# liangyuanpeng/kwok

Measured on AMD Instinct MI355X. Metric: stage transitions/sec (whole node), 1M nodes/100M pods; achieved HBM GB/s, higher is better.
Workload: dtype u8/i64

## Files before the change

### kwok_amd/csrc/engine.hip

```cpp
#include <hip/hip_runtime.h>

#include <cstdio>
#include <cstdlib>
#include <algorithm>
#include <cmath>
#include <cstring>
#include <mutex>
#include <set>
#include <string>
#include <type_traits>
#include <utility>
#include <vector>

#include "../../include/kwok_engine.h"
#include "id8_compose.hpp"
#include "errscope.hpp"
#include "devmem.hpp"
#include "usage_rows.hpp"

namespace {

constexpr int kBlock = 256;
constexpr int kMinObjPerThread = 8;
constexpr int kMaxObjPerThread = 32;
constexpr int kWavesPerBlock = kBlock / 64;
constexpr int kStatWords = 4 + KWK_MAX_STAGES;
constexpr int kStatLine = 3 + KWK_MAX_STAGES;

__device__ __forceinline__ void philox10(uint32_t& c0, uint32_t& c1, uint32_t& c2, uint32_t& c3, uint32_t k0,
                                         uint32_t k1) {
  k0 = (uint32_t)__builtin_amdgcn_readfirstlane((int)k0);
  k1 = (uint32_t)__builtin_amdgcn_readfirstlane((int)k1);
  asm volatile("" : "+s"(k0), "+s"(k1));
#pragma unroll
  for (int r = 0; r < 10; ++r) {
    const uint64_t p0 = (uint64_t)0xD2511F53u * c0, p1 = (uint64_t)0xCD9E8D57u * c2;
    const uint32_t lo0 = (uint32_t)p0, hi0 = (uint32_t)(p0 >> 32);
    const uint32_t lo1 = (uint32_t)p1, hi1 = (uint32_t)(p1 >> 32);
    const uint32_t n0 = hi1 ^ c1 ^ k0;
    const uint32_t n2 = hi0 ^ c3 ^ k1;
    c0 = n0;
    c1 = lo1;
    c2 = n2;
    c3 = lo0;
    k0 += 0x9E3779B9u;
    k1 += 0xBB67AE85u;
  }
}

__device__ __forceinline__ uint64_t philox_u64(uint64_t gslot, uint64_t step, uint32_t site, uint64_t key) {
  uint32_t c0 = (uint32_t)gslot, c1 = (uint32_t)step, c2 = (uint32_t)(step >> 32), c3 = site;
  philox10(c0, c1, c2, c3, (uint32_t)key, (uint32_t)(key >> 32));
  return (uint64_t)c0 | ((uint64_t)c1 << 32);
}

__device__ __forceinline__ int64_t below_u64(uint64_t u, int64_t n) { return (int64_t)__umul64hi(u, (uint64_t)n); }

__device__ __forceinline__ double rng_float64(uint64_t gslot, uint64_t step, uint32_t site, uint64_t key) {
  return (double)(philox_u64(gslot, step, site, key) >> 11) * 0x1.0p-53;
}

constexpr uint32_t kSitePick = 1, kSiteLeaseJitter = 3, kSiteRetryJitter = 4;

__device__ __forceinline__ int64_t sat_add(int64_t a, int64_t b) {
  int64_t r;
  if (__builtin_add_overflow(a, b, &r)) return b > 0 ? INT64_MAX : INT64_MIN;
  return r;
}

__device__ __forceinline__ int64_t abs_time_sub(int64_t sec, int32_t nsec, int64_t now) {
  int64_t now_sec = now / 1000000000;
  int64_t now_ns = now % 1000000000;
  if (now_ns < 0) { now_ns += 1000000000; now_sec -= 1; }
  int64_t ds = sec - now_sec;
  int64_t dn = (int64_t)nsec - now_ns;
  if (ds == 0) return dn;
  if (ds > 0) { ds -= 1; dn += 1000000000; } else { ds += 1; dn -= 1000000000; }
  if (ds > 9223372036ll || ds < -9223372036ll) return ds > 0 ? INT64_MAX : INT64_MIN;
  const int64_t p = ds * 1000000000ll;
  int64_t d;
  if (__builtin_add_overflow(p, dn, &d)) return dn > 0 ? INT64_MAX : INT64_MIN;
  return d;
}

struct Getter {
  int64_t v;
  bool ok;
};

__device__ __forceinline__ Getter eval_getter(int32_t slot, int64_t def, bool def_ok, uint32_t sched,
                                              const kwk_value* __restrict__ rec, int64_t del_s, int64_t now,
                                              bool is_duration) {
  if (slot == KWK_SLOT_NONE) return {def, def_ok};
  if (slot == KWK_SLOT_DELETION) {
    if (del_s == KWK_DEL_ABSENT) return {def, def_ok};
    return {abs_time_sub(del_s, 0, now), true};
  }
  if (!(sched & KWK_F_HASREC)) return {def, def_ok};
  const kwk_value e = rec[slot];
  switch (e.kind) {
    case KWK_V_OK: return {e.value, true};
    case KWK_V_NOTOK: return {0, false};
    case KWK_V_ABSTIME: return {is_duration ? abs_time_sub(e.value, e.nsec, now) : 0, is_duration};
    default: return {def, def_ok};
  }
}

struct StateFmt {
  uint32_t narrow;
  uint32_t half;
  uint32_t byte;
  uint32_t dw;
  int64_t epoch;
  uint32_t pmask;
  uint32_t cshift, cmask;
  uint32_t sshift, smask, none_code;
  uint32_t fshift;
  const uint16_t* id2w;
  const uint8_t* w2id;
};

__host__ __device__ __forceinline__ uint2 fmt_unpack(uint32_t w, const StateFmt& f) {
  const uint32_t cls = (w >> f.cshift) & f.cmask;
  const uint32_t sc = (w >> f.sshift) & f.smask;
  const uint32_t stage = sc == f.none_code ? KWK_STAGE_NONE : sc;
  const uint32_t fl = (w >> f.fshift) & 0x1Fu;
  return make_uint2(w & f.pmask, stage | (fl << 8) | (cls << KWK_CLASS_SHIFT));
}

__host__ __device__ __forceinline__ uint32_t fmt_pack(uint32_t pred, uint32_t sched, const StateFmt& f) {
  const uint32_t stage = sched & 0xFFu;
  const uint32_t sc = stage == KWK_STAGE_NONE ? f.none_code : stage;
  return (pred & f.pmask) | (((sched >> KWK_CLASS_SHIFT) & f.cmask) << f.cshift) | ((sc & f.smask) << f.sshift) |
         (((sched >> 8) & 0x1Fu) << f.fshift);
}

constexpr uint32_t kDwShift = 28;
constexpr uint32_t kDwWordMask = (1u << kDwShift) - 1u;
constexpr uint64_t kDwFar = (1ull << 36) - 1ull;
constexpr uint64_t kDwRebase = 1ull << 34;
__host__ __device__ __forceinline__ uint64_t dw_get(uint2 r) {
  return ((uint64_t)(r.x >> kDwShift) << 32) | r.y;
}
__host__ __device__ __forceinline__ uint2 dw_put(uint2 r, uint64_t d) {
  return make_uint2((r.x & kDwWordMask) | ((uint32_t)(d >> 32) << kDwShift), (uint32_t)d);
}
__host__ __device__ __forceinline__ uint64_t dw_enc(int64_t due, int64_t epoch) {
  if (due < epoch) return kDwFar;
  const uint64_t d = (uint64_t)due - (uint64_t)epoch;
  return d < kDwFar ? d : kDwFar;
}
__host__ __device__ __forceinline__ int64_t dw_abs(uint64_t d, int64_t epoch) {
  return (int64_t)((uint64_t)epoch + d);
}

__device__ __forceinline__ uint2 load_state(const void* st, uint64_t i, const StateFmt& f) {
  if (f.byte) return fmt_unpack(f.id2w[reinterpret_cast<const uint8_t*>(st)[i]], f);
  if (f.half) return fmt_unpack(reinterpret_cast<const uint16_t*>(st)[i], f);
  if (f.dw) return fmt_unpack(reinterpret_cast<const uint32_t*>(st)[2 * i], f);
  return f.narrow ? fmt_unpack(reinterpret_cast<const uint32_t*>(st)[i], f) : reinterpret_cast<const uint2*>(st)[i];
}
__device__ __forceinline__ void store_state(void* st, uint64_t i, uint2 v, const StateFmt& f) {
  if (f.byte) {
    reinterpret_cast<uint8_t*>(st)[i] = f.w2id[fmt_pack(v.x, v.y, f) & 0xFFFFu];
  } else if (f.half) {
    reinterpret_cast<uint16_t*>(st)[i] = (uint16_t)fmt_pack(v.x, v.y, f);
  } else if (f.dw) {
    uint32_t* p = reinterpret_cast<uint32_t*>(st) + 2 * i;
    *p = (*p & ~kDwWordMask) | fmt_pack(v.x, v.y, f);
  } else if (f.narrow) {
    reinterpret_cast<uint32_t*>(st)[i] = fmt_pack(v.x, v.y, f);
  } else {
    reinterpret_cast<uint2*>(st)[i] = v;
  }
}
__device__ __forceinline__ void store_state_due(void* st, int64_t* due_col, uint64_t i, uint2 v, int64_t due,
                                                const StateFmt& f) {
  if (f.dw) {
    const uint64_t d = dw_enc(due, f.epoch);
    reinterpret_cast<uint2*>(st)[i] = dw_put(make_uint2(fmt_pack(v.x, v.y, f), 0u), d);
    if (d == kDwFar) due_col[i] = due;
  } else {
    store_state(st, i, v, f);
    due_col[i] = due;
  }
}

__device__ __forceinline__ uint2 sw_decode(uint2 w, const StateFmt&) { return w; }
__device__ __forceinline__ uint2 sw_decode(uint32_t w, const StateFmt& f) { return fmt_unpack(w, f); }
__device__ __forceinline__ void sw_encode(uint2& out, uint2 v, const StateFmt&) { out = v; }
__device__ __forceinline__ void sw_encode(uint32_t& out, uint2 v, const StateFmt& f) { out = fmt_pack(v.x, v.y, f); }

struct RawTest {
  uint32_t managed, dirty, alive;
  uint32_t sshift, smask, none_code;
  uint32_t term, del;
};

constexpr uint32_t kMaxFuseSteps = 4;
constexpr uint32_t kHbMin = kMaxFuseSteps;
constexpr uint32_t kHbMax = 64;
struct SweepArgs {
  void* __restrict__ st;
  int64_t* __restrict__ due;
  int64_t* __restrict__ del_s;
  const uint32_t* __restrict__ rec_idx;
  const kwk_value* __restrict__ values;
  const kwk_stage_table* __restrict__ table;
  const kwk_delta* __restrict__ deltas;
  const uint32_t* __restrict__ lut;
  kwk_fired_rec* __restrict__ fired;
  uint32_t* __restrict__ wave_counts;
  unsigned long long* __restrict__ cum;
  uint32_t n;
  uint32_t lut_n;
  uint32_t lut_bytes;
  uint32_t lut_rest;
  uint32_t value_slots;
  uint64_t slot_base;
  uint64_t key;
  uint64_t step;
  int64_t now;
  uint32_t fire;
  StateFmt fmt;
  RawTest raw;
  kwk_harness harness;
  const uint32_t* __restrict__ fsm;
  const int64_t* __restrict__ fsm_due;
  uint32_t fsm_bits;
  const uint4* __restrict__ comp;
  int64_t dw_epoch_old;
  uint32_t dw_rebase;
  kwk_fired_rec* __restrict__ firedx[kMaxFuseSteps - 1];
  uint32_t* __restrict__ countsx[kMaxFuseSteps - 1];
  int64_t nowx[kMaxFuseSteps - 1];
  struct TailHb {
    void* out;
    uint32_t* offsets;
    uint32_t* host_len;
    unsigned long long* status;
    uint32_t seq;
    uint32_t packed;
  } tail;
};

__host__ __device__ __forceinline__ bool stage_matches(const kwk_stage_desc& s, uint32_t pred) {
  bool ok = ((pred ^ s.eq_val) & s.eq_mask) == 0;
  for (uint32_t k = 0; k < s.n_any; ++k) ok &= ((pred & s.any_mask[k]) != 0) == (((s.any_want >> k) & 1u) != 0);
  return ok;
}

__device__ __forceinline__ Getter stage_weight(const kwk_stage_desc& s, uint32_t sched,
                                               const kwk_value* __restrict__ rec) {
  return eval_getter(s.weight_slot, s.weight_default, true, sched, rec, KWK_DEL_ABSENT, 0, false);
}

__device__ __forceinline__ int nth_bit(uint32_t m, int64_t n) {
  for (int64_t i = 0; i < n; ++i) m &= m - 1;
  return __ffs(m) - 1;
}

struct Fire {
  bool fire;
  uint32_t stage;
  uint32_t flags;
  uint32_t bytes;
};

__device__ __forceinline__ uint32_t match_mask(const kwk_stage_table* __restrict__ T, uint32_t n_stages,
                                               uint32_t pred, const uint32_t* lut, uint32_t lut_n,
                                               uint32_t lut_bytes, uint32_t lut_rest) {
  uint32_t m = 0;
  if (lut_n) {
    m = lut[pred & 0xFFu];
    if (lut_bytes > 1) m &= lut[256u | ((pred >> 8) & 0xFFu)];
    if (lut_bytes > 2) m &= lut[512u | ((pred >> 16) & 0xFFu)];
    if (lut_bytes > 3) m &= lut[768u | (pred >> 24)];
    for (uint32_t r = lut_rest; r; r &= r - 1) {
      const uint32_t s = (uint32_t)__ffs(r) - 1u;
      m |= (stage_matches(T->stages[s], pred) ? 1u : 0u) << s;
    }
  } else {
    for (uint32_t s = 0; s < n_stages; ++s) m |= (stage_matches(T->stages[s], pred) ? 1u : 0u) << s;
  }
  return m;
}

template <bool kProbe = false>
__device__ __forceinline__ bool match_object(const SweepArgs& a, const kwk_stage_table* __restrict__ T,
                                             uint32_t n_stages, uint64_t i, uint32_t pred, uint32_t& sched,
                                             int64_t& due, uint32_t& bytes, const uint32_t* lut, uint32_t lut_n,
                                             uint32_t& gen) {
  const uint32_t m = match_mask(T, n_stages, pred, lut, lut_n, a.lut_bytes, a.lut_rest);
  sched &= ~(KWK_F_DIRTY | KWK_F_MATCHERR);
  if (m == 0) return false;
  const kwk_value* __restrict__ rec = nullptr;
  if (sched & KWK_F_HASREC) {
    if constexpr (kProbe) { gen = 1; return false; }
    rec = a.values + (uint64_t)a.rec_idx[i] * a.value_slots;
    bytes += 4 + 16 * 3;
  }
  const uint64_t gslot = a.slot_base + i;
  int pick;
  const int cnt = __popc(m);
  uint64_t u_pick = 0, u_jit = 0;
  if (!kProbe && (cnt > 1 || (m & T->reserved[0]))) {
    uint32_t c0 = (uint32_t)gslot, c1 = (uint32_t)a.step, c2 = (uint32_t)(a.step >> 32), c3 = kSitePick;
    philox10(c0, c1, c2, c3, (uint32_t)a.key, (uint32_t)(a.key >> 32));
    u_pick = (uint64_t)c0 | ((uint64_t)c1 << 32);
    u_jit = (uint64_t)c2 | ((uint64_t)c3 << 32);
  }
  if (cnt == 1) {
    pick = __ffs(m) - 1;
  } else {
    if constexpr (kProbe) { gen = 1; return false; }
    int64_t total = 0;
    int nerr = 0, nge0 = 0;
    for (uint32_t mm = m; mm; mm &= mm - 1) {
      const Getter w = stage_weight(T->stages[__ffs(mm) - 1], sched, rec);
      if (w.ok) {
        total = (int64_t)((uint64_t)total + (uint64_t)w.v);
        nge0 += w.v >= 0;
      } else {
        ++nerr;
      }
    }
    if (nerr == cnt || (total == 0 && nerr == 0)) {
      pick = nth_bit(m, below_u64(u_pick, cnt));
    } else if (total == 0) {
      int64_t want = below_u64(u_pick, nge0);
      pick = -1;
      for (uint32_t mm = m; mm; mm &= mm - 1) {
        const int s = __ffs(mm) - 1;
        const Getter w = stage_weight(T->stages[s], sched, rec);
        if (w.ok && w.v >= 0) {
          if (want == 0) { pick = s; break; }
          --want;
        }
      }
    } else if (total < 0) {
      sched |= KWK_F_MATCHERR;
      return false;
    } else {
      int64_t off = below_u64(u_pick, total);
      pick = 31 - __clz(m);
      for (uint32_t mm = m; mm; mm &= mm - 1) {
        const int s = __ffs(mm) - 1;
        const Getter w = stage_weight(T->stages[s], sched, rec);
        const int64_t wv = w.ok ? w.v : -1;
        if (wv <= 0) continue;
        off -= wv;
        if (off < 0) { pick = s; break; }
      }
    }
  }
  const kwk_stage_desc& S = T->stages[pick];
  int64_t delay = 0;
  if (S.has_delay) {
    const bool need_del = S.delay_slot == KWK_SLOT_DELETION || S.jitter_slot == KWK_SLOT_DELETION;
    if constexpr (kProbe) {
      if (need_del) { gen = 1; return false; }
    }
    const int64_t dels = need_del ? a.del_s[i] : KWK_DEL_ABSENT;
    if (need_del) bytes += 8;
    const Getter d = eval_getter(S.delay_slot, S.delay_default, true, sched, rec, dels, a.now, true);
    if (d.ok) {
      delay = d.v;
      if (S.has_jitter) {
        const Getter j = eval_getter(S.jitter_slot, S.jitter_default, S.jitter_default_ok != 0, sched, rec, dels,
                                     a.now, true);
        if (j.ok) {
          if (j.v < delay) {
            delay = j.v;
          } else {
            const int64_t jit = (int64_t)((uint64_t)j.v - (uint64_t)delay);
            if constexpr (kProbe) {
              if (jit > 0) { gen = 1; return false; }
            }
            if (jit > 0)
              delay = (int64_t)((uint64_t)delay + (uint64_t)below_u64(u_jit, jit));
          }
        }
      }
    }
  }
  sched = (sched & ~0xFFu) | (uint32_t)pick;
  due = sat_add(a.now, delay);
  return true;
}

__device__ __forceinline__ void fire_object(const SweepArgs& a, const kwk_stage_table* __restrict__ T,
                                            const kwk_delta* __restrict__ deltas, uint32_t n_stages,
                                            uint32_t fin_group, uint32_t cls, uint32_t st, uint32_t& pred,
                                            uint32_t& sched, Fire& f) {
  const kwk_stage_desc& S = T->stages[st];
  f.fire = true;
  f.stage = st;
  const uint32_t pre = pred;
  bool rematch = (S.flags & KWK_NEXT_PATCHES) && (!(S.flags & KWK_NEXT_PATCH_STATIC) || !(pre & S.applied_mask));
  if (S.flags & KWK_NEXT_FIN) {
    const uint32_t F = pre & fin_group;
    uint32_t F2;
    if ((S.flags & KWK_NEXT_FIN_EMPTY) || ((S.flags & KWK_NEXT_FIN_REMOVE) && (F & ~S.fin_remove) == 0))
      F2 = S.fin_add;
    else
      F2 = (F & ~S.fin_remove) | (S.fin_add & ~F);
    rematch |= F2 != F;
    pred = (pred & ~fin_group) | F2;
  }
  if (S.flags & KWK_NEXT_DELETE) {
    sched &= ~KWK_F_ALIVE;
    f.flags |= KWK_FIRED_DELETED;
    rematch = false;
  } else if (S.flags & KWK_NEXT_PATCHES) {
    const kwk_delta d = deltas[cls * n_stages + st];
    f.bytes += 2;
    if (d.and_mask == KWK_DELTA_UNKNOWN_AND && d.or_mask == KWK_DELTA_UNKNOWN_OR)
      f.flags |= KWK_FIRED_DELTA_UNKNOWN;
    else
      pred = (((pred & d.and_mask) | d.or_mask) & ~fin_group) | (pred & fin_group);
  }
  if (rematch) {
    sched |= KWK_F_DIRTY;
    f.flags |= KWK_FIRED_REMATCH;
  }
  sched |= KWK_STAGE_NONE;
}

template <bool kHarness, uint32_t kWordBytes, bool kProbe = false, bool kDueOut = false>
__device__ __forceinline__ uint2 process_object(const SweepArgs& a, const kwk_stage_table* __restrict__ T,
                                               const kwk_delta* __restrict__ deltas, uint32_t n_stages,
                                               uint32_t fin_group, uint64_t i, uint32_t pred, uint32_t sched,
                                               int64_t due, Fire& f, uint32_t& n_matched, const uint32_t* lut,
                                               uint32_t lut_n, uint32_t& gen, int64_t& due_w) {
  if (kHarness) {
    if (!(sched & KWK_F_ALIVE)) {
      pred &= a.harness.keep_mask;
      sched = (sched & (KWK_F_MANAGED | KWK_F_HASREC | KWK_CLASS_MASK)) | KWK_F_ALIVE | KWK_F_DIRTY | KWK_STAGE_NONE;
      if (a.harness.track_deletion) {
        if constexpr (kProbe) gen = 1;
        else a.del_s[i] = KWK_DEL_ABSENT;
        f.bytes += 8;
      }
    } else if ((pred & a.harness.terminal_mask) && !(pred & a.harness.deletion_bit)) {
      pred |= a.harness.deletion_bit;
      int64_t sec = a.now / 1000000000;
      if (a.now % 1000000000 < 0) sec -= 1;
      if (a.harness.track_deletion) {
        if constexpr (kProbe) gen = 1;
        else a.del_s[i] = sec;
        f.bytes += 8;
      }
      sched |= KWK_F_DIRTY;
    }
  }
  bool scheduled = false;
  if (sched & KWK_F_ALIVE) {
    if (sched & KWK_F_DIRTY) {
      if (pred & T->disregard_mask) {
        sched &= ~KWK_F_DIRTY;
      } else {
        scheduled = match_object<kProbe>(a, T, n_stages, i, pred, sched, due, f.bytes, lut, lut_n, gen);
        n_matched += scheduled ? 1 : 0;
      }
    }
    const uint32_t st = sched & 0xFFu;
    if (a.fire && st < n_stages && due <= a.now) fire_object(a, T, deltas, n_stages, fin_group, sched >> KWK_CLASS_SHIFT, st,
                                                   pred, sched, f);
  }
  if (scheduled && (sched & 0xFFu) < n_stages) {
    if constexpr (kProbe) {
      due_w = due;
    } else if constexpr (kDueOut) {
      due_w = due;
      gen = 1;
    } else {
      a.due[i] = due;
    }
    if constexpr (!kDueOut) f.bytes += 8;
  }
  f.bytes += kWordBytes;
  return make_uint2(pred, sched);
}

template <bool kPacked = false>
__device__ __forceinline__ void emit_fired(const Fire& f, uint64_t i, uint32_t lane, kwk_fired_rec* __restrict__ seg,
                                           uint32_t& seg_n, unsigned int* s_stat, uint32_t& n_bytes) {
  const unsigned long long bal = __ballot(f.fire);
  if (!bal) return;
  if (f.fire) {
    const uint32_t pos = seg_n + (uint32_t)__popcll(bal & ((1ull << lane) - 1ull));
    if constexpr (kPacked) {
      reinterpret_cast<uint32_t*>(seg)[pos] = (uint32_t)i | f.stage << 13 | f.flags << 18;
      n_bytes += 4;
    } else {
      seg[pos] = kwk_fired_rec{(uint32_t)i, (uint16_t)f.stage, (uint16_t)f.flags};
      n_bytes += 8;
    }
  }
  seg_n += (uint32_t)__popcll(bal);
  unsigned long long rest = bal;
  while (rest) {
    const uint32_t s = __shfl(f.stage, __ffsll((long long)rest) - 1);
    const unsigned long long same = __ballot(f.fire && f.stage == s);
    if (lane == 0) atomicAdd(&s_stat[3 + s], (unsigned)__popcll(same));
    rest &= ~same;
  }
}

constexpr uint32_t kLutMax = 256;
constexpr uint32_t kLutTables = 1024;
constexpr uint32_t kLutLdsW = 512;

constexpr uint32_t kOOB = 0xFFFFFFF0u;
__device__ __forceinline__ __amdgpu_buffer_rsrc_t make_rsrc(const void* p, uint32_t bytes) {
  return __builtin_amdgcn_make_buffer_rsrc(const_cast<void*>(p), (short)0, (int)bytes, 0x00020000);
}
__device__ __forceinline__ int64_t buf_load_i64(__amdgpu_buffer_rsrc_t r, uint32_t off) {
  const auto t = __builtin_amdgcn_raw_buffer_load_b64(r, off, 0, 0);
  return (int64_t)(((uint64_t)t[1] << 32) | t[0]);
}

__device__ __forceinline__ void store_chunk_nt(void* p, const uint4& v) {
  typedef uint32_t u32x4 __attribute__((ext_vector_type(4)));
  __builtin_nontemporal_store(u32x4{v.x, v.y, v.z, v.w}, reinterpret_cast<u32x4*>(p));
}

constexpr uint32_t kFsmDue = 1u << 30, kFsmGeneral = 1u << 31;

template <bool kHarness>
__global__ void fsm_build_kernel(SweepArgs a, uint32_t* __restrict__ tab, int64_t* __restrict__ dtab) {
  const uint32_t bits = a.fsm_bits;
  const uint32_t idx = blockIdx.x * blockDim.x + threadIdx.x;
  if (idx >= (2u << bits)) return;
  const uint32_t w = idx & ((1u << bits) - 1u), rdy = idx >> bits;
  const uint2 s = fmt_unpack(w, a.fmt);
  const kwk_stage_table* __restrict__ T = a.table;
  const int64_t due = ((s.y & 0xFFu) != KWK_STAGE_NONE) ? (rdy ? 0 : 1) : 0;
  Fire f{false, 0, 0, 0};
  uint32_t nm = 0, gen = 0;
  int64_t dw = INT64_MIN;
  const uint2 nv = process_object<kHarness, 2, true>(a, T, a.deltas, T->n_stages, T->fin_group_mask, 0, s.x, s.y, due,
                                                     f, nm, a.lut, a.lut_n, gen, dw);
  uint32_t e = fmt_pack(nv.x, nv.y, a.fmt) & 0xFFFFu;
  e |= (f.stage & 31u) << 16 | (f.fire ? 1u : 0u) << 21 | (f.flags & 7u) << 22 | (nm & 1u) << 25;
  e |= ((f.bytes >> 1) & 15u) << 26;
  if (dw != INT64_MIN) e |= kFsmDue;
  if (gen || f.bytes > 30 || (f.bytes & 1u)) e = kFsmGeneral;
  tab[idx] = e;
  dtab[idx] = dw;
}

constexpr uint32_t kQ16 = 4;
constexpr int kWpe16 = 6;
constexpr int kWpe16Q4 = 4;
constexpr int kLdsDeltas16 = 64;
constexpr uint32_t kStoreLanes = 8;
__device__ __forceinline__ constexpr uint32_t bit_word(const uint32_t b) {
  return ((b & 15u) >> 2) * 512u + 2u * (b & 3u) + (b >> 4);
}
template <int Q>
constexpr uint32_t seg16_words() { return 64u * 8u * Q + 32u; }
#define kSeg16 seg16_words<Q>()
template <bool kHarness, int Q, bool kPersist>
__global__ __launch_bounds__(kBlock) __attribute__((amdgpu_waves_per_eu(Q >= 4 ? kWpe16Q4 : kWpe16))) void sweep16_kernel(SweepArgs a) {
  constexpr int K = 8 * Q;
  constexpr uint32_t kWave = 64u * K;
  constexpr uint32_t kTile = kBlock * K;
  __shared__ unsigned int s_stat[kStatWords];
  __shared__ kwk_delta s_delta[kLdsDeltas16];
  __shared__ uint16_t s_work[kWavesPerBlock][kWave];
  __shared__ uint4 s_tile[kWavesPerBlock][64 * Q];
  __shared__ uint32_t s_lut[kLutMax];
  __shared__ kwk_stage_table s_tab;
  const uint32_t lane = threadIdx.x & 63;
  const uint32_t wave = threadIdx.x >> 6;
  const uint32_t n_tiles = (uint32_t)(((uint64_t)a.n + kTile - 1) / kTile);
  const __amdgpu_buffer_rsrc_t st_rs = make_rsrc(a.st, ((a.n * 2u) + 15u) & ~15u);
  uint4 va[Q];
  auto issue_tile = [&](uint4 (&dst)[Q], const uint32_t t) {
    if (t >= n_tiles) return;
    const uint32_t wb = t * kTile + wave * kWave;
#pragma unroll
    for (int q = 0; q < Q; ++q) {
      const auto c = __builtin_amdgcn_raw_buffer_load_b128(st_rs, (wb + (uint32_t)q * 512u + lane * 8u) * 2u, 0, 0);
      dst[q] = make_uint4(c[0], c[1], c[2], c[3]);
    }
  };
  uint32_t tile = blockIdx.x;
  issue_tile(va, tile);
  {
    const uint32_t nw = (offsetof(kwk_stage_table, stages) + a.table->n_stages * sizeof(kwk_stage_desc)) / 4;
    const uint32_t* src = reinterpret_cast<const uint32_t*>(a.table);
    uint32_t* dst = reinterpret_cast<uint32_t*>(&s_tab);
    for (uint32_t j = threadIdx.x; j < nw; j += kBlock) dst[j] = src[j];
  }
  const kwk_stage_table* __restrict__ T = &s_tab;
  const uint32_t n_stages = a.table->n_stages;
  const uint32_t fin_group = a.table->fin_group_mask;
  const uint32_t n_deltas = a.table->n_classes * n_stages;
  const uint32_t lut_n = a.lut_n;
  const uint32_t* __restrict__ lutp = lut_n <= kLutMax ? s_lut : a.lut;
  if (lut_n <= kLutMax)
    for (uint32_t j = threadIdx.x; j < lut_n; j += kBlock) s_lut[j] = a.lut[j];
  if (threadIdx.x < kStatWords) s_stat[threadIdx.x] = 0;
  const kwk_delta* __restrict__ deltas = a.deltas;
  if (n_deltas <= kLdsDeltas16) {
    for (uint32_t j = threadIdx.x; j < n_deltas; j += kBlock) s_delta[j] = a.deltas[j];
    deltas = s_delta;
  }
  __syncthreads();

  const StateFmt fmt = a.fmt;
  const RawTest R = a.raw;
  struct {
    uint32_t m2, d2, a2, t2, l2, s2, n2;
    uint32_t sm, sd, sa, sl;
  } X;
  X.m2 = R.managed * 0x10001u; X.d2 = R.dirty * 0x10001u; X.a2 = R.alive * 0x10001u;
  X.t2 = R.term * 0x10001u; X.l2 = R.del * 0x10001u;
  X.s2 = (R.smask << R.sshift) * 0x10001u; X.n2 = (R.none_code << R.sshift) * 0x10001u;
  X.sm = (uint32_t)(16 - __ffs(R.managed)) & 31u; X.sd = (uint32_t)(16 - __ffs(R.dirty)) & 31u;
  X.sa = (uint32_t)(16 - __ffs(R.alive)) & 31u; X.sl = (uint32_t)(16 - __ffs(R.del)) & 31u;
  uint32_t n_matched = 0, n_bytes = 0;
  uint32_t n_line = 0;
  uint32_t wave_fired = 0;
  uint16_t* __restrict__ wl = s_work[wave];
  uint4* __restrict__ tq = s_tile[wave];
  uint16_t* __restrict__ tw = reinterpret_cast<uint16_t*>(tq);
  uint4* __restrict__ gq = reinterpret_cast<uint4*>(a.st);

  auto tile_body = [&](uint4 (&v)[Q], const uint32_t tile) {
    const uint32_t wbase = tile * kTile + wave * kWave;
    const bool full = (uint64_t)(tile + 1) * kTile <= a.n;
    uint32_t seg_n = 0;
    const uint64_t seg_id = (uint64_t)tile * kWavesPerBlock + wave;
    uint32_t* __restrict__ seg32 = reinterpret_cast<uint32_t*>(a.fired) + seg_id * kSeg16;
    kwk_fired_rec* __restrict__ seg = reinterpret_cast<kwk_fired_rec*>(seg32 + 1);

    uint4 cur[Q];
#pragma unroll
    for (int q = 0; q < Q; ++q) cur[q] = v[q];
    if (kPersist) issue_tile(v, tile + gridDim.x);
    constexpr uint32_t kHalfMask = (1u << (4 * Q)) - 1u;
    uint32_t in_range = kHalfMask | kHalfMask << 16;
    if (!full) {
      in_range = 0;
#pragma unroll
      for (int t = 0; t < K; ++t) {
        const int b = t < 4 * Q ? t : 16 + t - 4 * Q;
        in_range |= (wbase + bit_word((uint32_t)b) + lane * 8u < a.n ? 1u : 0u) << b;
      }
    }
    uint32_t pend = 0, need = 0, ready = 0;
#pragma unroll
    for (int q = 0; q < Q; ++q) {
      const uint32_t dw[4] = {cur[q].x, cur[q].y, cur[q].z, cur[q].w};
#pragma unroll
      for (int j = 0; j < 4; ++j) {
        const uint32_t d = dw[j];
        const uint32_t mg = (d & X.m2) << X.sm;
        const uint32_t pe = (((d & X.s2) ^ X.n2) + 0x7FFF7FFFu) & 0x80008000u;
        uint32_t nb = (d & X.d2) << X.sd;
        if (kHarness) {
          nb |= (~d & X.a2) << X.sa;
          nb |= (((d & X.t2) + 0x7FFF7FFFu) & 0x80008000u) & ~((d & X.l2) << X.sl);
        }
        const uint32_t n2 = mg & nb, p2 = mg & pe;
        const int jj = q * 4 + j;
        need |= n2 >> (15 - jj);
        pend |= p2 >> (15 - jj);
      }
    }
    pend &= in_range;
    need &= in_range;
    if (__ballot(pend != 0)) {
      const __amdgpu_buffer_rsrc_t due_rs = make_rsrc(a.due, a.n * 8u);
#pragma unroll 8
      for (int t = 0; t < K; ++t) {
        const int k = t < 4 * Q ? t : 16 + t - 4 * Q;
        const uint32_t p = (pend >> k) & 1u;
        const int64_t d = buf_load_i64(due_rs, p ? (wbase + bit_word((uint32_t)k) + lane * 8u) * 8u : kOOB);
        ready |= (p & (uint32_t)(d <= a.now)) << k;
      }
      need |= ready;
    }
    n_bytes += 2u * (uint32_t)__popc(in_range) + 8u * (uint32_t)__popc(pend);
    uint32_t n_work = 0, pos = 0;
    {
      const uint32_t cnt = (uint32_t)__popc(need);
      const unsigned long long lt = (1ull << lane) - 1ull;
#pragma unroll
      for (int b = 0; b < 6; ++b) {
        const unsigned long long bal = __ballot((cnt >> b) & 1u);
        pos += (uint32_t)__popcll(bal & lt) << b;
        n_work += (uint32_t)__popcll(bal) << b;
      }
      for (uint32_t m = need; m; m &= m - 1u) {
        const uint32_t k = (uint32_t)__ffs(m) - 1u;
        wl[pos++] = (uint16_t)(bit_word(k) + lane * 8u + (((ready >> k) & 1u) << 15));
      }
    }

    if (n_work) {
#pragma unroll
      for (int q = 0; q < Q; ++q) tq[q * 64 + lane] = cur[q];
      __builtin_amdgcn_fence(__ATOMIC_SEQ_CST, "wavefront");
      auto fetch = [&](const uint32_t c, uint32_t& we, uint32_t& raw, uint32_t& ent) {
        we = (c + lane < n_work) ? (uint32_t)wl[c + lane] : 0xFFFFFFFFu;
        raw = we != 0xFFFFFFFFu ? (uint32_t)tw[we & 0x7FFFu] : 0u;
        ent = (we != 0xFFFFFFFFu && a.fsm) ? a.fsm[((we >> 15) << a.fsm_bits) | raw] : kFsmGeneral;
      };
      uint32_t we, raw, ent;
      fetch(0, we, raw, ent);
      for (uint32_t c = 0; c < n_work; c += 64u) {
        const uint32_t cwe = we, craw = raw, e = ent;
        if (c + 64u < n_work) fetch(c + 64u, we, raw, ent);
        Fire f{false, 0, 0, 0};
        uint64_t i = 0;
        if (cwe != 0xFFFFFFFFu) {
          const uint32_t w = cwe & 0x7FFFu, rdy = cwe >> 15;
          i = wbase + w;
          if (!(e & kFsmGeneral)) {
            tw[w] = (uint16_t)e;
            if (e & kFsmDue) a.due[i] = sat_add(a.now, a.fsm_due[(rdy << a.fsm_bits) | craw]);
            f.fire = (e >> 21) & 1u;
            f.stage = (e >> 16) & 31u;
            f.flags = (e >> 22) & 7u;
            f.bytes = ((e >> 26) & 15u) * 2u;
            n_matched += (e >> 25) & 1u;
          } else {
            const uint2 s = fmt_unpack(craw, fmt);
            const int64_t due = ((s.y & 0xFFu) != KWK_STAGE_NONE) ? a.due[i] : 0;
            uint32_t gen_unused = 0;
            int64_t due_unused = 0;
            const uint2 nv = process_object<kHarness, 2>(a, T, deltas, n_stages, fin_group, i, s.x, s.y, due, f,
                                                         n_matched, lutp, lut_n, gen_unused, due_unused);
            tw[w] = (uint16_t)fmt_pack(nv.x, nv.y, fmt);
          }
          n_line -= 2u;
        }
        n_bytes += f.bytes;
        emit_fired<true>(f, i - wbase, lane, seg, seg_n, s_stat, n_bytes);
      }
      __builtin_amdgcn_fence(__ATOMIC_SEQ_CST, "wavefront");
#pragma unroll
      for (int q = 0; q < Q; ++q) {
        const uint4 nv = tq[q * 64 + lane];
        const bool ch = (nv.x ^ cur[q].x) | (nv.y ^ cur[q].y) | (nv.z ^ cur[q].z) | (nv.w ^ cur[q].w);
        const unsigned long long bal = __ballot(ch);
        if ((bal >> (lane & ~(kStoreLanes - 1u))) & ((1ull << kStoreLanes) - 1ull)) {
          store_chunk_nt(&gq[(wbase + (uint32_t)q * 512u + lane * 8u) / 8u], nv);
          n_line += 16u;
        }
      }
      __builtin_amdgcn_fence(__ATOMIC_SEQ_CST, "wavefront");
    }
    {
      const uint32_t used = 1u + seg_n, end = (used + 31u) & ~31u;
      for (uint32_t x = used + lane; x < end; x += 64) seg32[x] = 0u;
      if (lane == 0) {
        seg32[0] = seg_n;
        a.wave_counts[seg_id] = seg_n;
      }
      n_line += 4u * (uint32_t)__popc((uint32_t)(lane < end - used));
    }
    wave_fired += seg_n;
    n_bytes += lane == 0 ? 4u : 0u;
  };
  if constexpr (!kPersist) {
    if (tile < n_tiles) tile_body(va, tile);
  } else {
    for (; tile < n_tiles; tile += gridDim.x) tile_body(va, tile);
  }

  for (int off = 32; off > 0; off >>= 1) {
    n_matched += __shfl_xor(n_matched, off);
    n_bytes += __shfl_xor(n_bytes, off);
    n_line += __shfl_xor(n_line, off);
  }
  if (lane == 0) {
    atomicAdd(&s_stat[0], n_matched);
    atomicAdd(&s_stat[1], wave_fired);
    atomicAdd(&s_stat[2], n_bytes);
    atomicAdd(&s_stat[kStatLine], n_bytes + n_line);
  }
  __syncthreads();
  if (threadIdx.x < 3 + n_stages || threadIdx.x == kStatLine) {
    const unsigned int val = s_stat[threadIdx.x];
    if (val) atomicAdd(&a.cum[(uint64_t)blockIdx.x * kStatWords + threadIdx.x], (unsigned long long)val);
  }
}

template <bool kHarness>
__device__ __forceinline__ uint2 general16(uint32_t i, uint32_t raw) {
  uint64_t ka = (uint64_t)__builtin_amdgcn_kernarg_segment_ptr();
  asm volatile("" : "+v"(ka));
  const SweepArgs& a = *reinterpret_cast<const SweepArgs*>(ka);
  uint64_t tp = (uint64_t)a.table;
  asm volatile("" : "+v"(tp));
  const kwk_stage_table* __restrict__ T = reinterpret_cast<const kwk_stage_table*>(tp);
  const uint2 s = fmt_unpack(raw, a.fmt);
  const int64_t due = ((s.y & 0xFFu) != KWK_STAGE_NONE) ? a.due[i] : 0;
  Fire f{false, 0, 0, 0};
  uint32_t nm = 0, gen_unused = 0;
  int64_t due_unused = 0;
  const uint2 nv = process_object<kHarness, 2>(a, T, a.deltas, T->n_stages, T->fin_group_mask, i, s.x, s.y, due, f, nm,
                                               a.lut, a.lut_n, gen_unused, due_unused);
  uint32_t e = fmt_pack(nv.x, nv.y, a.fmt) & 0xFFFFu;
  e |= (f.stage & 31u) << 16 | (f.fire ? 1u : 0u) << 21 | (f.flags & 7u) << 22 | (nm & 1u) << 25;
  return make_uint2(e, f.bytes);
}

__device__ __forceinline__ uint32_t block_prefix(unsigned long long* status, uint32_t stride, uint32_t b, uint32_t bt,
                                                 uint32_t seq, uint32_t lane) {
  if (lane == 0)
    __hip_atomic_store(&status[(uint64_t)b * stride], (unsigned long long)seq << 32 | bt, __ATOMIC_RELAXED,
                       __HIP_MEMORY_SCOPE_AGENT);
  constexpr uint32_t kIn = 16;
  uint32_t pre = 0;
  for (uint32_t j0 = lane; j0 < b; j0 += 64u * kIn) {
    unsigned long long v[kIn];
#pragma unroll
    for (uint32_t k = 0; k < kIn; ++k) {
      const uint32_t j = j0 + 64u * k;
      v[k] = j < b ? __hip_atomic_load(&status[(uint64_t)j * stride], __ATOMIC_RELAXED, __HIP_MEMORY_SCOPE_AGENT)
                   : (unsigned long long)seq << 32;
    }
#pragma unroll
    for (uint32_t k = 0; k < kIn; ++k) {
      const uint32_t j = j0 + 64u * k;
      while ((uint32_t)(v[k] >> 32) != seq) {
        __builtin_amdgcn_s_sleep(2);
        v[k] = __hip_atomic_load(&status[(uint64_t)j * stride], __ATOMIC_RELAXED, __HIP_MEMORY_SCOPE_AGENT);
      }
      pre += (uint32_t)v[k];
    }
  }
  for (int o = 32; o > 0; o >>= 1) pre += __shfl_xor(pre, o);
  return pre;
}

template <uint32_t kWaveSlots, uint32_t kSegWords>
__device__ __forceinline__ void tail_handback(const SweepArgs& a, uint32_t wave_n, uint32_t lane, uint32_t wave) {
  __shared__ uint32_t s_wn[kWavesPerBlock];
  __shared__ uint32_t s_pre;
  const SweepArgs::TailHb& t = a.tail;
  __builtin_amdgcn_fence(__ATOMIC_RELEASE, "workgroup");
  if (lane == 0) s_wn[wave] = wave_n;
  __syncthreads();
  const uint32_t bt = s_wn[0] + s_wn[1] + s_wn[2] + s_wn[3];
  if (wave == 0) {
    const uint32_t pre = block_prefix(t.status, 1u, blockIdx.x, bt, t.seq, lane);
    if (lane == 0) s_pre = pre;
  }
  __syncthreads();
  uint32_t off = s_pre;
  for (uint32_t w = 0; w < wave; ++w) off += s_wn[w];
  const uint64_t seg_id = (uint64_t)blockIdx.x * kWavesPerBlock + wave;
  const uint32_t* __restrict__ sp = reinterpret_cast<const uint32_t*>(a.fired) + seg_id * kSegWords;
  const uint32_t base = (uint32_t)seg_id * kWaveSlots;
  for (uint32_t j = lane; j < wave_n; j += 64u) {
    const uint32_t x = sp[1u + j];
    const uint32_t slot = base + (x & 0x1FFFu);
    if (t.packed) {
      __builtin_nontemporal_store(((x >> 13) & 31u) << 27 | slot, reinterpret_cast<uint32_t*>(t.out) + off + j);
    } else {
      typedef uint32_t u32x2 __attribute__((ext_vector_type(2)));
      __builtin_nontemporal_store(u32x2{slot, ((x >> 13) & 31u) | ((x >> 18) & 7u) << 16},
                                  reinterpret_cast<u32x2*>(reinterpret_cast<kwk_fired_rec*>(t.out) + off + j));
    }
  }
  if (blockIdx.x == gridDim.x - 1 && threadIdx.x == 0) {
    t.offsets[0] = s_pre + bt;
    if (t.host_len) t.host_len[0] = s_pre + bt;
  }
}

constexpr int kFsmBatch = 4;
constexpr uint32_t kFsmKernelDefault = 2;
template <bool kHarness, int Q, bool kPersist, int kDepth>
__global__ __launch_bounds__(kBlock) __attribute__((amdgpu_waves_per_eu(Q >= 4 ? 4 : 5))) void sweep16_fsm_kernel(SweepArgs a) {
  constexpr int K = 8 * Q;
  constexpr uint32_t kWave = 64u * K;
  constexpr uint32_t kTile = kBlock * K;
  constexpr int B = kFsmBatch;
  static_assert(kDepth >= 1 && kDepth <= 2 && (kPersist || kDepth == 1), "prefetch depth");
  __shared__ unsigned int s_stat[kStatWords];
  __shared__ uint16_t s_work[kWavesPerBlock][kWave];
  __shared__ uint4 s_tile[kWavesPerBlock][64 * Q];
  const uint32_t lane = threadIdx.x & 63;
  const uint32_t wave = __builtin_amdgcn_readfirstlane(threadIdx.x >> 6);
  const uint32_t n_tiles = (uint32_t)(((uint64_t)a.n + kTile - 1) / kTile);
  const __amdgpu_buffer_rsrc_t st_rs = make_rsrc(a.st, ((a.n * 2u) + 15u) & ~15u);
  const __amdgpu_buffer_rsrc_t due_rs = make_rsrc(a.due, a.n * 8u);
  const uint32_t fbits = a.fsm_bits;
  const __amdgpu_buffer_rsrc_t fsm_rs = make_rsrc(a.fsm, 4u << (fbits + 1));
  const __amdgpu_buffer_rsrc_t fdue_rs = make_rsrc(a.fsm_due, 8u << (fbits + 1));
  uint4 va[kDepth][Q];
  auto issue_tile = [&](uint4 (&dst)[Q], const uint32_t t) __attribute__((always_inline)) {
    const uint32_t off = t < n_tiles ? (t * kTile + wave * kWave + lane * 8u) * 2u : kOOB - 4u * 1024u;
#pragma unroll
    for (int q = 0; q < Q; ++q) {
      const auto c = __builtin_amdgcn_raw_buffer_load_b128(st_rs, off + (uint32_t)q * 1024u, 0, 0);
      dst[q] = make_uint4(c[0], c[1], c[2], c[3]);
    }
  };
  uint32_t tile = blockIdx.x;
  issue_tile(va[0], tile);
  if (kDepth > 1) issue_tile(va[1], tile + gridDim.x);
  const uint32_t n_stages = a.table->n_stages;
  if (threadIdx.x < kStatWords) s_stat[threadIdx.x] = 0;
  __syncthreads();

  const RawTest R = a.raw;
  struct {
    uint32_t m2, d2, a2, t2, l2, s2, n2;
    uint32_t sm, sd, sa, sl;
  } X;
  X.m2 = R.managed * 0x10001u; X.d2 = R.dirty * 0x10001u; X.a2 = R.alive * 0x10001u;
  X.t2 = R.term * 0x10001u; X.l2 = R.del * 0x10001u;
  X.s2 = (R.smask << R.sshift) * 0x10001u; X.n2 = (R.none_code << R.sshift) * 0x10001u;
  X.sm = (uint32_t)(16 - __ffs(R.managed)) & 31u; X.sd = (uint32_t)(16 - __ffs(R.dirty)) & 31u;
  X.sa = (uint32_t)(16 - __ffs(R.alive)) & 31u; X.sl = (uint32_t)(16 - __ffs(R.del)) & 31u;
  uint32_t stc01 = 0, stc23 = 0;
  uint32_t n_matched = 0, n_bytes = 0;
  uint32_t n_lline = 0;
  uint32_t w_bytes = 0, w_line = 0;
  uint32_t wave_fired = 0;
  uint16_t* __restrict__ wl = s_work[wave];
  uint4* __restrict__ tq = s_tile[wave];
  uint16_t* __restrict__ tw = reinterpret_cast<uint16_t*>(tq);
  uint4* __restrict__ gq = reinterpret_cast<uint4*>(a.st);

  auto tile_body = [&](uint4 (&v)[Q], const uint32_t tile) __attribute__((always_inline)) {
    const uint32_t wbase = tile * kTile + wave * kWave;
    const bool full = (uint64_t)(tile + 1) * kTile <= a.n;
    uint32_t seg_n = 0;
    const uint64_t seg_id = (uint64_t)tile * kWavesPerBlock + wave;
    uint32_t* __restrict__ seg32 = reinterpret_cast<uint32_t*>(a.fired) + seg_id * kSeg16;
    const __amdgpu_buffer_rsrc_t seg_rs = make_rsrc(seg32, kSeg16 * 4u);
    uint4 cur_copy[Q];
    if (kDepth == 1) {
#pragma unroll
      for (int q = 0; q < Q; ++q) cur_copy[q] = v[q];
    }
    uint4 (&cur)[Q] = kDepth == 1 ? cur_copy : v;
    constexpr uint32_t kHalfMask = (1u << (4 * Q)) - 1u;
    uint32_t in_range = kHalfMask | kHalfMask << 16;
    if (!full) {
      in_range = 0;
#pragma unroll
      for (int q = 0; q < Q; ++q) {
        const int64_t left = (int64_t)a.n - (int64_t)(wbase + (uint32_t)q * 512u + lane * 8u);
        const uint32_t c = left <= 0 ? 0u : left >= 8 ? 8u : (uint32_t)left;
        in_range |= (((1u << ((c + 1u) >> 1)) - 1u) << (4 * q)) | (((1u << (c >> 1)) - 1u) << (16 + 4 * q));
      }
    }
    uint32_t pend = 0, need = 0, ready = 0;
#pragma unroll
    for (int q = 0; q < Q; ++q) {
      const uint32_t dw[4] = {cur[q].x, cur[q].y, cur[q].z, cur[q].w};
#pragma unroll
      for (int j = 0; j < 4; ++j) {
        const uint32_t d = dw[j];
        const uint32_t mg = (d & X.m2) << X.sm;
        const uint32_t pe = (((d & X.s2) ^ X.n2) + 0x7FFF7FFFu) & 0x80008000u;
        uint32_t nb = (d & X.d2) << X.sd;
        if (kHarness) {
          nb |= (~d & X.a2) << X.sa;
          nb |= (((d & X.t2) + 0x7FFF7FFFu) & 0x80008000u) & ~((d & X.l2) << X.sl);
        }
        const uint32_t n2 = mg & nb, p2 = mg & pe;
        const int jj = q * 4 + j;
        need |= n2 >> (15 - jj);
        pend |= p2 >> (15 - jj);
      }
    }
    pend &= in_range;
    need &= in_range;
    if (__ballot(pend != 0)) {
#pragma unroll 8
      for (int t = 0; t < K; ++t) {
        const int k = t < 4 * Q ? t : 16 + t - 4 * Q;
        const uint32_t p = (pend >> k) & 1u;
        const int64_t d = buf_load_i64(due_rs, p ? (wbase + bit_word((uint32_t)k) + lane * 8u) * 8u : kOOB);
        ready |= (p & (uint32_t)(d <= a.now)) << k;
      }
      need |= ready;
    }
    n_bytes += 2u * (uint32_t)__popc(in_range) + 8u * (uint32_t)__popc(pend);
    uint32_t n_work = 0, pos = 0;
    {
      const uint32_t cnt = (uint32_t)__popc(need);
      const unsigned long long lt = (1ull << lane) - 1ull;
#pragma unroll
      for (int b = 0; b < 6; ++b) {
        const unsigned long long bal = __ballot((cnt >> b) & 1u);
        pos += (uint32_t)__popcll(bal & lt) << b;
        n_work += (uint32_t)__popcll(bal) << b;
      }
      for (uint32_t m = need; m; m &= m - 1u) {
        const uint32_t k = (uint32_t)__ffs(m) - 1u;
        wl[pos++] = (uint16_t)(bit_word(k) + lane * 8u + (((ready >> k) & 1u) << 15));
      }
    }
    uint32_t we[B], raw[B], ent[B];
    auto fetch = [&](const uint32_t c0) __attribute__((always_inline)) {
#pragma unroll
      for (int b = 0; b < B; ++b) {
        const uint32_t c = c0 + 64u * b + lane;
        const bool in = c < n_work;
        const uint32_t x0 = (uint32_t)wl[c & (kWave - 1u)];
        const uint32_t x = in ? x0 : 0u;
        we[b] = in ? x : 0xFFFFFFFFu;
        raw[b] = (uint32_t)tw[x & 0x7FFFu];
        ent[b] = __builtin_amdgcn_raw_buffer_load_b32(fsm_rs, in ? ((((x >> 15) << fbits) | raw[b]) * 4u) : kOOB, 0, 0);
      }
    };
    auto emit = [&](const bool fire, const uint32_t w, const uint32_t e) __attribute__((always_inline)) {
      const unsigned long long bal = __ballot(fire);
      if (bal) {
        const uint32_t pos = seg_n + __builtin_amdgcn_mbcnt_hi((uint32_t)(bal >> 32), __builtin_amdgcn_mbcnt_lo((uint32_t)bal, 0u));
        const uint32_t rec = w | ((e >> 16) & 31u) << 13 | ((e >> 22) & 7u) << 18;
        __builtin_amdgcn_raw_buffer_store_b32(rec, seg_rs, fire ? (1u + pos) * 4u : kOOB, 0, 0);
        const uint32_t nf = (uint32_t)__popcll(bal);
        seg_n += nf;
        w_bytes += 4u * nf;
        const uint32_t code = fire ? ((e >> 16) & 31u) : 31u;
        if (n_stages <= 4) {
          const uint32_t inc = 1u << (16u * (code & 1u));
          stc01 += code < 2u ? inc : 0u;
          stc23 += (code - 2u) < 2u ? inc : 0u;
        } else {
          for (uint32_t st = 0; st < n_stages; ++st) {
            const unsigned long long same = __ballot(code == st);
            if (same && lane == 0) atomicAdd(&s_stat[3 + st], (unsigned)__popcll(same));
          }
        }
      }
    };
    uint32_t n_gen = 0;
    auto pass = [&](const int b) __attribute__((always_inline)) {
      const uint32_t cwe = we[b], e = ent[b];
      const bool act = cwe != 0xFFFFFFFFu;
      const uint32_t w = cwe & 0x7FFFu;
      const bool gen = act && (e & kFsmGeneral);
      const unsigned long long gb = __ballot(gen);
      if (gb) {
        if (gen) wl[n_gen + __builtin_amdgcn_mbcnt_hi((uint32_t)(gb >> 32), __builtin_amdgcn_mbcnt_lo((uint32_t)gb, 0u))] = (uint16_t)w;
        n_gen += (uint32_t)__popcll(gb);
      }
      const bool tab = act && !gen;
      if (tab) {
        tw[w] = (uint16_t)e;
        n_matched += (e >> 25) & 1u;
        n_bytes += ((e >> 26) & 15u) * 2u;
      }
      const bool dw = tab && (e & kFsmDue);
      if (__ballot(dw)) {
        const int64_t dd = buf_load_i64(fdue_rs, dw ? ((((cwe >> 15) << fbits) | raw[b]) * 8u) : kOOB);
        const int64_t v = sat_add(a.now, dd);
        const uint32_t off = dw ? (wbase + w) * 8u : kOOB;
        __builtin_amdgcn_raw_buffer_store_b32((uint32_t)v, due_rs, off, 0, 0);
        __builtin_amdgcn_raw_buffer_store_b32((uint32_t)((uint64_t)v >> 32), due_rs, off + 4u, 0, 0);
      }
      emit(tab && ((e >> 21) & 1u), w, e);
    };
    if (n_work) {
#pragma unroll
      for (int q = 0; q < Q; ++q) tq[q * 64 + lane] = cur[q];
      __builtin_amdgcn_fence(__ATOMIC_SEQ_CST, "wavefront");
      fetch(0);
    }
    if (kPersist && kDepth == 1) issue_tile(v, tile + gridDim.x);
    if (n_work) {
#pragma unroll
      for (int b = 0; b < B; ++b)
        if (64u * b < n_work) pass(b);
      for (uint32_t c0 = 64u * B; c0 < n_work; c0 += 64u * B) {
        fetch(c0);
#pragma unroll
        for (int b = 0; b < B; ++b)
          if (c0 + 64u * b < n_work) pass(b);
      }
      for (uint32_t j = 0; j < n_gen; j += 64u) {
        const bool in = j + lane < n_gen;
        const uint32_t w = in ? (uint32_t)wl[j + lane] : 0u;
        uint32_t e = 0;
        if (in) {
          const uint2 r = general16<kHarness>(wbase + w, (uint32_t)tw[w]);
          e = r.x;
          tw[w] = (uint16_t)e;
          n_matched += (e >> 25) & 1u;
          n_bytes += r.y;
        }
        emit(in && ((e >> 21) & 1u), w, e);
      }
      w_line -= 2u * n_work;
      __builtin_amdgcn_fence(__ATOMIC_SEQ_CST, "wavefront");
#pragma unroll
      for (int q = 0; q < Q; ++q) {
        const uint4 nv = tq[q * 64 + lane];
        const bool ch = (nv.x ^ cur[q].x) | (nv.y ^ cur[q].y) | (nv.z ^ cur[q].z) | (nv.w ^ cur[q].w);
        const unsigned long long bal = __ballot(ch);
        if ((bal >> (lane & ~(kStoreLanes - 1u))) & ((1ull << kStoreLanes) - 1ull)) {
          store_chunk_nt(&gq[(wbase + (uint32_t)q * 512u + lane * 8u) / 8u], nv);
          n_lline += 16u;
        }
      }
      __builtin_amdgcn_fence(__ATOMIC_SEQ_CST, "wavefront");
    }
    {
      const uint32_t used = 1u + seg_n, end = (used + 31u) & ~31u;
      for (uint32_t x = used + lane; x < end; x += 64) seg32[x] = 0u;
      if (lane == 0) {
        seg32[0] = seg_n;
        a.wave_counts[seg_id] = seg_n;
      }
      w_line += 4u * (end - used);
    }
    wave_fired += seg_n;
    w_bytes += 4u;
    if (kPersist && kDepth == 2) issue_tile(v, tile + 2u * gridDim.x);
  };
  if constexpr (!kPersist) {
    if (tile < n_tiles) tile_body(va[0], tile);
  } else if constexpr (kDepth == 1) {
    for (; tile < n_tiles; tile += gridDim.x) tile_body(va[0], tile);
  } else {
    for (; tile < n_tiles; tile += 2u * gridDim.x) {
      tile_body(va[0], tile);
      if (tile + gridDim.x >= n_tiles) break;
      tile_body(va[1], tile + gridDim.x);
    }
  }

  for (int off = 32; off > 0; off >>= 1) {
    n_matched += __shfl_xor(n_matched, off);
    n_bytes += __shfl_xor(n_bytes, off);
    n_lline += __shfl_xor(n_lline, off);
  }
  uint32_t stn[4] = {stc01 & 0xFFFFu, stc01 >> 16, stc23 & 0xFFFFu, stc23 >> 16};
#pragma unroll
  for (int st = 0; st < 4; ++st)
    for (int off = 32; off > 0; off >>= 1) stn[st] += __shfl_xor(stn[st], off);
  if (lane == 0) {
#pragma unroll
    for (int st = 0; st < 4; ++st)
      if (stn[st]) atomicAdd(&s_stat[3 + st], stn[st]);
    atomicAdd(&s_stat[0], n_matched);
    atomicAdd(&s_stat[1], wave_fired);
    atomicAdd(&s_stat[2], n_bytes + w_bytes);
    atomicAdd(&s_stat[kStatLine], n_bytes + w_bytes + n_lline + w_line);
  }
  __syncthreads();
  if (threadIdx.x < 3 + n_stages || threadIdx.x == kStatLine) {
    const unsigned int val = s_stat[threadIdx.x];
    if (val) atomicAdd(&a.cum[(uint64_t)blockIdx.x * kStatWords + threadIdx.x], (unsigned long long)val);
  }
  if constexpr (!kPersist) {
    if (a.tail.out) tail_handback<kWave, kSeg16>(a, tile < n_tiles ? wave_fired : 0u, lane, wave);
  }
}

constexpr int kQ8 = 2;
constexpr uint32_t kId8AnyDue = 1u;
constexpr uint32_t kRec16Header = 16;

__device__ __forceinline__ uint32_t lds_id8(const uint32_t k, const uint32_t lane4) {
  const uint32_t jj = k & 7u;
  return jj << 8 | (lane4 ^ jj << 2) | k >> 3;
}
__device__ __forceinline__ uint32_t lds_col8(const uint32_t jj, const uint32_t lane) { return jj * 64u + (lane ^ jj); }
__host__ __device__ __forceinline__ uint32_t id8_slot(const uint32_t x) {
  const uint32_t jj = x >> 8, lane = ((x >> 2) & 63u) ^ jj, b = x & 3u;
  return (jj >> 2) * 1024u + lane * 16u + (jj & 3u) * 4u + b;
}
__device__ __forceinline__ unsigned long long ballot(const bool b) { return __builtin_amdgcn_ballot_w64(b); }

template <int C, int RM>
__device__ __forceinline__ uint32_t dpp_u32(uint32_t v) {
  return (uint32_t)__builtin_amdgcn_update_dpp(0, (int)v, C, RM, 0xF, false);
}
__device__ __forceinline__ uint32_t wave_incl_scan(uint32_t v) {
  v += dpp_u32<0x111, 0xF>(v);
  v += dpp_u32<0x112, 0xF>(v);
  v += dpp_u32<0x114, 0xF>(v);
  v += dpp_u32<0x118, 0xF>(v);
  v += dpp_u32<0x142, 0xA>(v);
  v += dpp_u32<0x143, 0xC>(v);
  return v;
}

typedef __attribute__((address_space(3))) uint8_t lds_u8;
typedef __attribute__((address_space(3))) uint16_t lds_u16;
__device__ __forceinline__ uint32_t lds_addr(const void* p) {
  return (uint32_t)(size_t)(const __attribute__((address_space(3))) uint8_t*)p;
}

template <bool kStages4>
__device__ __forceinline__ void id8_fire(const uint32_t addr, const uint32_t e, uint16_t* __restrict__ wl,
                                         const __amdgpu_buffer_rsrc_t seg_rs, uint32_t& seg_n, uint32_t (&stc)[4],
                                         unsigned int* s_stat, uint32_t n_stages, uint32_t lane);

template <bool kSlow, bool kStages4>
__device__ __forceinline__ void id8_pass(const uint32_t we, const uint32_t* __restrict__ s_fsm, uint16_t* __restrict__ wl,
                                         const __amdgpu_buffer_rsrc_t seg_rs, uint32_t& seg_n, uint32_t& n_bytes,
                                         uint32_t& n_matched, uint32_t (&stc)[4], unsigned int* s_stat, uint32_t n_stages,
                                         uint32_t lane, bool any_due, const __amdgpu_buffer_rsrc_t fdue_rs,
                                         const __amdgpu_buffer_rsrc_t due_rs, uint32_t wbase, int64_t now) {
  const uint32_t addr = kSlow ? (we & 0x7FFFu) : we;
  const uint32_t r = kSlow ? (we >> 7) & 0x100u : 0u;
  lds_u8* p = (lds_u8*)(size_t)addr;
  const uint32_t key = r | (uint32_t)*p;
  const uint32_t e = s_fsm[key];
  *p = (uint8_t)e;
  n_bytes += (e >> 24) & 31u;
  n_matched += (e >> 30) & 1u;
  if (kSlow && any_due && (e & kId8Due)) {
    const int64_t dd = buf_load_i64(fdue_rs, key * 8u);
    const int64_t t = sat_add(now, dd);
    const uint32_t off = (wbase + id8_slot(addr & 0x7FFu)) * 8u;
    __builtin_amdgcn_raw_buffer_store_b32((uint32_t)t, due_rs, off, 0, 0);
    __builtin_amdgcn_raw_buffer_store_b32((uint32_t)((uint64_t)t >> 32), due_rs, off + 4u, 0, 0);
  }
  id8_fire<kStages4>(addr, e, wl, seg_rs, seg_n, stc, s_stat, n_stages, lane);
}

constexpr uint32_t kId8Batch = 4;
template <bool kStages4, uint32_t kN>
__device__ __forceinline__ void id8_passn(const uint32_t (&we)[kN], const uint32_t* __restrict__ s_fsm,
                                          uint16_t* __restrict__ wl, const __amdgpu_buffer_rsrc_t seg_rs, uint32_t& seg_n,
                                          uint32_t& n_bytes, uint32_t& n_matched, uint32_t (&stc)[4],
                                          unsigned int* s_stat, uint32_t n_stages, uint32_t lane) {
  uint32_t k[kN], e[kN];
#pragma unroll
  for (uint32_t j = 0; j < kN; ++j) k[j] = (uint32_t)*(lds_u8*)(size_t)we[j];
#pragma unroll
  for (uint32_t j = 0; j < kN; ++j) e[j] = s_fsm[k[j]];
#pragma unroll
  for (uint32_t j = 0; j < kN; ++j) *(lds_u8*)(size_t)we[j] = (uint8_t)e[j];
#pragma unroll
  for (uint32_t j = 0; j < kN; ++j) {
    n_bytes += (e[j] >> 24) & 31u;
    n_matched += (e[j] >> 30) & 1u;
    id8_fire<kStages4>(we[j], e[j], wl, seg_rs, seg_n, stc, s_stat, n_stages, lane);
  }
}

template <int kSteps, uint32_t kN>
__device__ __forceinline__ void id8_carryn(const uint32_t (&we)[kN], const uint32_t* __restrict__ s_fsm,
                                           uint16_t* __restrict__ wl, const __amdgpu_buffer_rsrc_t seg_rs,
                                           uint32_t (&segs)[kSteps], uint32_t& n_bytes, uint32_t& n_matched,
                                           uint32_t (&stc)[4], uint32_t& live, unsigned int* s_stat, uint32_t n_stages,
                                           uint32_t lane) {
  constexpr uint32_t kRegion = 2048u / (uint32_t)kSteps;
  uint32_t key[kN], fin[kN], e[kN];
#pragma unroll
  for (uint32_t j = 0; j < kN; ++j) {
    key[j] = (uint32_t)*(lds_u8*)(size_t)we[j];
    fin[j] = kIdInvalid;
  }
#pragma unroll
  for (int s = 0; s < kSteps; ++s) {
    if (s > 0) {
#pragma unroll
      for (uint32_t j = 0; j < kN; ++j) live += (uint32_t)__popcll(ballot(key[j] != kIdInvalid));
    }
#pragma unroll
    for (uint32_t j = 0; j < kN; ++j) e[j] = s_fsm[key[j]];
#pragma unroll
    for (uint32_t j = 0; j < kN; ++j) {
      n_bytes += (e[j] >> 24) & 31u;
      n_matched += (e[j] >> 30) & 1u;
      id8_fire<true>(we[j], e[j], wl + (uint32_t)s * kRegion, seg_rs, segs[s], stc, s_stat, n_stages, lane);
    }
#pragma unroll
    for (uint32_t j = 0; j < kN; ++j) {
      const uint32_t nid = e[j] & 0xFFu;
      if (s + 1 < kSteps) {
        const bool on = (nid & kIdNeed) != 0;
        key[j] = on ? nid : kIdInvalid;
        fin[j] = on ? fin[j] : nid;
      } else {
        fin[j] &= nid;
      }
    }
  }
#pragma unroll
  for (uint32_t j = 0; j < kN; ++j) *(lds_u8*)(size_t)we[j] = (uint8_t)fin[j];
}

template <int kSteps, uint32_t kN>
__device__ __forceinline__ void id8_carryc(const uint32_t (&we)[kN], const uint4* __restrict__ s_comp,
                                           uint16_t* __restrict__ wl, uint32_t (&segs)[kSteps], uint32_t& stat,
                                           uint32_t& n_lline, uint32_t (&stc)[4]) {
  constexpr uint32_t kRegion = 2048u / (uint32_t)kSteps;
  static_assert(kSteps <= kId8cMaxSteps && 2048u / (uint32_t)kSteps / 64u <= 16u, "row words, statistics fields");
  uint32_t key[kN];
  uint4 r[kN];
#pragma unroll
  for (uint32_t j = 0; j < kN; ++j) key[j] = (uint32_t)*(lds_u8*)(size_t)we[j];
#pragma unroll
  for (uint32_t j = 0; j < kN; ++j) r[j] = s_comp[key[j]];
#pragma unroll
  for (uint32_t j = 0; j < kN; ++j) *(lds_u8*)(size_t)we[j] = (uint8_t)r[j].x;
#pragma unroll
  for (uint32_t j = 0; j < kN; ++j) {
    stat += r[j].y & kId8cStat;
    n_lline -= r[j].z & kId8cLive;
    stc[0] += r[j].w & kId8cStages;
  }
#pragma unroll
  for (int s = 0; s < kSteps; ++s) {
#pragma unroll
    for (uint32_t j = 0; j < kN; ++j) {
      const uint32_t w = s == 0 ? r[j].x : s == 1 ? r[j].y : s == 2 ? r[j].z : r[j].w;
      const bool fire = (int32_t)w < 0;
      const unsigned long long bal = ballot(fire);
      if (bal) {
        const uint32_t pos =
            __builtin_amdgcn_mbcnt_hi((uint32_t)(bal >> 32), __builtin_amdgcn_mbcnt_lo((uint32_t)bal, segs[s]));
        if (fire) wl[(uint32_t)s * kRegion + pos] = (uint16_t)((we[j] & 0x7FFu) | (w & kId8Rec16));
        segs[s] += (uint32_t)__popcll(bal);
      }
    }
  }
}

template <bool kStages4>
__device__ __forceinline__ void id8_fire(const uint32_t addr, const uint32_t e, uint16_t* __restrict__ wl,
                                         const __amdgpu_buffer_rsrc_t seg_rs, uint32_t& seg_n, uint32_t (&stc)[4],
                                         unsigned int* s_stat, uint32_t n_stages, uint32_t lane) {
  const bool fire = (int32_t)e < 0;
  const unsigned long long bal = ballot(fire);
  if (bal) {
    const uint32_t pos = __builtin_amdgcn_mbcnt_hi((uint32_t)(bal >> 32), __builtin_amdgcn_mbcnt_lo((uint32_t)bal, seg_n));
    if constexpr (kStages4) {
      if (fire) wl[pos] = (uint16_t)((addr & 0x7FFu) | (e & kId8Rec16));
      stc[0] += (e >> 31) << ((e >> 8) & 0x18u);
    } else {
      __builtin_amdgcn_raw_buffer_store_b32((addr & 0x7FFu) | ((e >> 3) & 0x1FE000u), seg_rs, fire ? (1u + pos) * 4u : kOOB,
                                            0, 0);
      const uint32_t code = (e >> 16) & 31u;
      for (uint32_t st = 0; st < n_stages; ++st) {
        const unsigned long long same = ballot(code == st) & bal;
        if (same && lane == 0) atomicAdd(&s_stat[3 + st], (unsigned)__popcll(same));
      }
    }
    seg_n += (uint32_t)__popcll(bal);
  }
}

template <bool kPersist, int kDepth, bool kStages4, int kSteps = 1>
__global__ __launch_bounds__(kBlock) __attribute__((amdgpu_waves_per_eu(kPersist ? 1 : 6))) void sweep8_kernel(SweepArgs a) {
  constexpr int Q = kQ8;
  constexpr int K = 16 * Q;
  constexpr uint32_t kWave = 64u * K;
  constexpr uint32_t kTile = kBlock * K;
  constexpr uint32_t kSeg8 = 64u * K + 32u;
  static_assert(kDepth >= 1 && kDepth <= 2 && (kPersist || kDepth == 1), "prefetch depth");
  static_assert(kWave == 2048 && K == 32, "11-bit record offsets, 32-bit lane masks");
  static_assert((kSteps == 1 || kStages4) && kSteps >= 1 && kSteps <= (int)kMaxFuseSteps,
                "fused steps hand back 2-byte records");
  __shared__ __attribute__((aligned(2048))) uint32_t s_tile[kWavesPerBlock][4 * Q][64];
  __shared__ __attribute__((aligned(16))) uint16_t s_work[kWavesPerBlock][kWave];
  __shared__ uint32_t s_inv[64];
  __shared__ uint32_t s_fsm[512];
  constexpr bool kCompose = kSteps > 1 && kPersist;
  __shared__ __attribute__((aligned(16))) uint4 s_comp[kCompose ? 256 : 1];
  __shared__ unsigned int s_stat[kStatWords];
  const uint32_t lane = threadIdx.x & 63;
  const uint32_t wave = __builtin_amdgcn_readfirstlane(threadIdx.x >> 6);
  const uint32_t n_tiles = (uint32_t)(((uint64_t)a.n + kTile - 1) / kTile);
  const __amdgpu_buffer_rsrc_t st_rs = make_rsrc(a.st, (a.n + 15u) & ~15u);
  const __amdgpu_buffer_rsrc_t due_rs = make_rsrc(a.due, a.n * 8u);
  const __amdgpu_buffer_rsrc_t fdue_rs = make_rsrc(a.fsm_due, 8u * 512u);
  const __amdgpu_buffer_rsrc_t cnt_rs = make_rsrc(a.wave_counts, n_tiles * kWavesPerBlock * 4u);
  uint4 va[kDepth][Q];
  auto issue_tile = [&](uint4 (&dst)[Q], const uint32_t t) __attribute__((always_inline)) {
    const uint32_t off = t < n_tiles ? t * kTile + wave * kWave + lane * 16u : kOOB - 2048u;
#pragma unroll
    for (int q = 0; q < Q; ++q) {
      const auto c = __builtin_amdgcn_raw_buffer_load_b128(st_rs, off + (uint32_t)q * 1024u, 0, 0);
      dst[q] = make_uint4(c[0], c[1], c[2], c[3]);
    }
  };
  uint32_t tile = blockIdx.x;
  issue_tile(va[0], tile);
  if (kDepth > 1) issue_tile(va[kDepth - 1], tile + gridDim.x);
  const uint32_t n_stages = a.table->n_stages;
  const bool any_due = (a.fsm_bits & kId8AnyDue) != 0;
  static_assert(kBlock * 2 == 512, "id table staging");
  {
    const uint32_t t0 = a.fsm[threadIdx.x], t1 = a.fsm[threadIdx.x + kBlock];
    s_fsm[threadIdx.x] = t0;
    s_fsm[threadIdx.x + kBlock] = t1;
  }
  if constexpr (kCompose) {
    static_assert(kBlock == 256, "composite table staging");
    s_comp[threadIdx.x] = a.comp[threadIdx.x];
  }
  if (threadIdx.x < kStatWords) s_stat[threadIdx.x] = 0;
  if (wave == 0) s_inv[lane] = 0xFFFFFFFFu;
  __syncthreads();

  uint32_t stc[4] = {0u, 0u, 0u, 0u};
  uint32_t n_matched = 0, n_bytes = 0;
  uint32_t n_lline = 0;
  uint32_t w_bytes = 0, w_line = 0;
  uint32_t wave_fired = 0;
  uint32_t* __restrict__ tw = &s_tile[wave][0][0];
  uint16_t* __restrict__ wl = s_work[wave];
  const __amdgpu_buffer_rsrc_t gq_rs = make_rsrc(a.st, (a.n + 2047u) & ~2047u);
  const uint32_t tile_lds = lds_addr(tw);
  const uint32_t lane4 = lane * 4u;
  const uint32_t inv_ent = lds_addr(&s_inv[lane]);

  auto tile_body = [&](uint4 (&v)[Q], const uint32_t tile) __attribute__((always_inline)) {
    const bool real = tile < n_tiles;
    const uint32_t wbase = tile * kTile + wave * kWave;
    const bool full = (uint64_t)(tile + 1) * kTile <= a.n;
    const uint32_t seg_id = tile * kWavesPerBlock + wave;
    uint32_t* __restrict__ seg32 = reinterpret_cast<uint32_t*>(a.fired) + (uint64_t)seg_id * kSeg8;
    const __amdgpu_buffer_rsrc_t seg_rs = make_rsrc(seg32, kSeg8 * 4u);
    uint4 cur_copy[Q];
    if (kDepth == 1) {
#pragma unroll
      for (int q = 0; q < Q; ++q) cur_copy[q] = v[q];
    }
    uint4 (&cur)[Q] = kDepth == 1 ? cur_copy : v;
    if (kPersist && kDepth == 1) issue_tile(v, tile + gridDim.x);
    uint32_t in_range = 0xFFFFFFFFu;
    if (!full) {
      in_range = 0;
#pragma unroll
      for (int q = 0; q < Q; ++q) {
        const int64_t left = (int64_t)a.n - (int64_t)(wbase + (uint32_t)q * 1024u + lane * 16u);
        const uint32_t c = left <= 0 ? 0u : left >= 16 ? 16u : (uint32_t)left;
#pragma unroll
        for (uint32_t j = 0; j < 4; ++j)
#pragma unroll
          for (uint32_t b = 0; b < 4; ++b) in_range |= (j * 4u + b < c ? 1u : 0u) << (b * 8u + (uint32_t)q * 4u + j);
      }
    }
    constexpr uint32_t kCarry = kWave / (uint32_t)kSteps;
    uint32_t segs[kSteps] = {};
    bool carry = false;
    uint32_t cstat = 0;
    auto phase12 = [&](const uint4 (&ids)[Q], const int64_t now, const auto first_t, const bool in_lds, uint32_t& seg_n)
                       __attribute__((always_inline)) -> uint32_t {
      constexpr bool first = decltype(first_t)::value;
      uint32_t need = 0, pend = 0, ready = 0;
  #pragma unroll
      for (int q = 0; q < Q; ++q) {
        const uint32_t dw[4] = {ids[q].x, ids[q].y, ids[q].z, ids[q].w};
  #pragma unroll
        for (int j = 0; j < 4; ++j) {
          const uint32_t jj = (uint32_t)(q * 4 + j);
          need |= (dw[j] & 0x80808080u) >> (7u - jj);
          pend |= ((dw[j] << 1) & 0x80808080u) >> (7u - jj);
        }
      }
// ... 637 lines not shown
}

constexpr uint32_t kCompactSpw = 4;
constexpr uint32_t kCompact16Spw = 8;
template <int kRec, bool kPacked = false, uint32_t kSpw = 1>
__global__ __launch_bounds__(kBlock) void compact_kernel(CompactArgs a) {
  constexpr int kPre = 4;
  static_assert(kScanGroup % (kSpw * kWavesPerBlock) == 0, "a wave's segments lie in one scan group");
  const uint32_t lane = threadIdx.x & 63, wave = threadIdx.x >> 6;
  const uint32_t seg0 = (blockIdx.x * kWavesPerBlock + wave) * kSpw;
  if (seg0 >= a.n_segs) return;
  uint2 r[kSpw][kPre];
  uint32_t c[kSpw], o1[kSpw];
#pragma unroll
  for (uint32_t s = 0; s < kSpw; ++s) {
    const uint32_t seg = seg0 + s < a.n_segs ? seg0 + s : seg0;
    const uint32_t* __restrict__ sp = a.fired32 + (uint64_t)seg * a.stride;
#pragma unroll
    for (int k = 0; k < kPre; ++k) r[s][k] = rec_at<kRec>(sp, lane + 64u * k);
    c[s] = seg0 + s < a.n_segs ? a.counts[seg] : 0u;
    o1[s] = a.offsets[1 + seg];
  }
  uint32_t gp = 0;
  for (uint32_t g = lane; g < seg0 / kScanGroup; g += 64) gp += a.group_tot[g];
  for (int o = 32; o > 0; o >>= 1) gp += __shfl_xor(gp, o);
#pragma unroll
  for (uint32_t s = 0; s < kSpw; ++s) {
    const uint32_t seg = seg0 + s;
    if (seg >= a.n_segs) break;
    const uint32_t off = gp + o1[s];
    if (seg == a.n_segs - 1 && lane == 0) {
      a.offsets[0] = off + c[s];
      if (a.host_len) a.host_len[0] = off + c[s];
    }
    const uint32_t base = (seg >> a.seg_region_shift) * a.region_slots;
#pragma unroll
    for (int k = 0; k < kPre; ++k) {
      const uint32_t j = lane + 64u * k;
      if (j < c[s]) store_out<kPacked>(a, off + j, base + r[s][k].x, r[s][k].y);
    }
    const uint32_t* __restrict__ sp = a.fired32 + (uint64_t)seg * a.stride;
    for (uint32_t j = lane + 64u * kPre; j < c[s]; j += 64) {
      const uint2 x = rec_at<kRec>(sp, j);
      store_out<kPacked>(a, off + j, base + x.x, x.y);
    }
  }
}

template <uint32_t kSpw>
__device__ __forceinline__ void compact16_block(const CompactArgs& a, const uint32_t block) {
  static_assert(kScanGroup % (kSpw * kWavesPerBlock) == 0, "a wave's segments lie in one scan group");
  const uint32_t lane = threadIdx.x & 63, wave = threadIdx.x >> 6;
  const uint32_t seg0 = (block * kWavesPerBlock + wave) * kSpw;
  if (seg0 >= a.n_segs) return;
  uint32_t c[kSpw], o1[kSpw];
  uint16_t r[kSpw][4];
#pragma unroll
  for (uint32_t s = 0; s < kSpw; ++s) {
    const uint32_t seg = seg0 + s < a.n_segs ? seg0 + s : seg0;
    const uint16_t* sp = reinterpret_cast<const uint16_t*>(a.fired32 + (uint64_t)seg * a.stride + kRec16Header / 4u);
#pragma unroll
    for (uint32_t k = 0; k < 4; ++k) r[s][k] = sp[lane + 64u * k];
    c[s] = seg0 + s < a.n_segs ? a.counts[seg] : 0u;
    o1[s] = a.offsets[1 + seg];
  }
  if (a.counts_out) {
#pragma unroll
    for (uint32_t s = 0; s < kSpw; ++s)
      if (lane == s && seg0 + s < a.n_segs) a.counts_out[seg0 + s] = c[s];
  }
  uint32_t gp = 0;
  for (uint32_t g = lane; g < seg0 / kScanGroup; g += 64) gp += a.group_tot[g];
  for (int o = 32; o > 0; o >>= 1) gp += __shfl_xor(gp, o);
  uint16_t* out = reinterpret_cast<uint16_t*>(a.out);
#pragma unroll
  for (uint32_t s = 0; s < kSpw; ++s) {
    const uint32_t seg = seg0 + s;
    if (seg >= a.n_segs) break;
    const uint32_t off = gp + o1[s];
    if (seg == a.n_segs - 1 && lane == 0) {
      a.offsets[0] = off + c[s];
      if (a.host_len) a.host_len[0] = off + c[s];
    }
#pragma unroll
    for (uint32_t k = 0; k < 4; ++k)
      if (lane + 64u * k < c[s]) __builtin_nontemporal_store(r[s][k], out + off + lane + 64u * k);
    const uint16_t* sp = reinterpret_cast<const uint16_t*>(a.fired32 + (uint64_t)seg * a.stride + kRec16Header / 4u);
    for (uint32_t j = lane + 256u; j < c[s]; j += 64) __builtin_nontemporal_store(sp[j], out + off + j);
  }
}
template <uint32_t kSpw>
__global__ __launch_bounds__(kBlock) void compact16_kernel(CompactArgs a) {
  compact16_block<kSpw>(a, blockIdx.x);
}
template <uint32_t kSpw>
__global__ __launch_bounds__(kBlock) void compact16_multi_kernel(CompactArgs4 m) {
  compact16_block<kSpw>(m.a[blockIdx.y], blockIdx.x);
}

constexpr uint32_t kSmall16Spw = 4;
constexpr uint32_t kSmall16Spb = kSmall16Spw * kWavesPerBlock;
template <uint32_t kSpw>
__device__ __forceinline__ void compact16_small_block(const CompactArgs& a, const uint32_t block) {
  constexpr uint32_t kSpb = kSpw * kWavesPerBlock;
  static_assert(kSpb % 4 == 0, "prefix loads assume whole uint4s before the block");
  __shared__ uint32_t s_part[kWavesPerBlock];
  __shared__ uint32_t s_seg[kSpb];
  const uint32_t lane = threadIdx.x & 63, wave = threadIdx.x >> 6;
  const uint32_t first = block * kSpb;
  const uint4* __restrict__ c4 = reinterpret_cast<const uint4*>(a.counts);
  uint32_t sum = 0;
#pragma unroll 8
  for (uint32_t q = threadIdx.x; q < first / 4u; q += kBlock) {
    const uint4 v = c4[q];
    sum += (v.x + v.y) + (v.z + v.w);
  }
  for (int o = 32; o > 0; o >>= 1) sum += __shfl_xor(sum, o);
  if (lane == 0) s_part[wave] = sum;
  if (threadIdx.x < kSpb) {
    const uint32_t c = first + threadIdx.x < a.n_segs ? a.counts[first + threadIdx.x] : 0u;
    s_seg[threadIdx.x] = c;
    if (a.counts_out && first + threadIdx.x < a.n_segs) a.counts_out[first + threadIdx.x] = c;
  }
  __syncthreads();
  const uint32_t seg0 = first + wave * kSpw;
  if (seg0 >= a.n_segs) return;
  uint32_t off = s_part[0] + s_part[1] + s_part[2] + s_part[3];
  for (uint32_t w = 0; w < wave * kSpw; ++w) off += s_seg[w];
  uint32_t c[kSpw];
  uint16_t r[kSpw][4];
#pragma unroll
  for (uint32_t s = 0; s < kSpw; ++s) {
    const uint32_t seg = seg0 + s < a.n_segs ? seg0 + s : seg0;
    const uint16_t* sp = reinterpret_cast<const uint16_t*>(a.fired32 + (uint64_t)seg * a.stride + kRec16Header / 4u);
#pragma unroll
    for (uint32_t k = 0; k < 4; ++k) r[s][k] = sp[lane + 64u * k];
    c[s] = seg0 + s < a.n_segs ? s_seg[wave * kSpw + s] : 0u;
  }
  uint16_t* out = reinterpret_cast<uint16_t*>(a.out);
#pragma unroll
  for (uint32_t s = 0; s < kSpw; ++s) {
    const uint32_t seg = seg0 + s;
    if (seg >= a.n_segs) break;
    if (seg == a.n_segs - 1 && lane == 0) {
      a.offsets[0] = off + c[s];
      if (a.host_len) a.host_len[0] = off + c[s];
    }
#pragma unroll
    for (uint32_t k = 0; k < 4; ++k)
      if (lane + 64u * k < c[s]) __builtin_nontemporal_store(r[s][k], out + off + lane + 64u * k);
    const uint16_t* sp = reinterpret_cast<const uint16_t*>(a.fired32 + (uint64_t)seg * a.stride + kRec16Header / 4u);
    for (uint32_t j = lane + 256u; j < c[s]; j += 64) __builtin_nontemporal_store(sp[j], out + off + j);
    off += c[s];
  }
}
__global__ __launch_bounds__(kBlock) void compact16_small_kernel(CompactArgs a) {
  compact16_small_block<kSmall16Spw>(a, blockIdx.x);
}
__global__ __launch_bounds__(kBlock) void compact16_small_multi_kernel(CompactArgs4 m) {
  compact16_small_block<kSmall16Spw>(m.a[blockIdx.y], blockIdx.x);
}

__device__ __forceinline__ void bits_map(const CompactArgs& a, uint32_t seg, uint32_t c, uint32_t* __restrict__ map,
                                         uint32_t lane) {
  const uint16_t* __restrict__ rp =
      reinterpret_cast<const uint16_t*>(a.fired32 + (uint64_t)seg * a.stride + kRec16Header / 4u);
  map[lane] = 0u;
  __builtin_amdgcn_fence(__ATOMIC_SEQ_CST, "wavefront");
  __builtin_amdgcn_wave_barrier();
  for (uint32_t j = lane; j < c; j += 64u) {
    const uint32_t x = rp[j] & 0x7FFu, jj = x >> 8;
    atomicOr(&map[((x >> 2) & 63u) ^ jj], 1u << ((x & 3u) * 8u + jj));
  }
  __builtin_amdgcn_fence(__ATOMIC_SEQ_CST, "wavefront");
  __builtin_amdgcn_wave_barrier();
}

__device__ __forceinline__ uint32_t nz_bytes(uint32_t d) {
  return (uint32_t)((d & 0xFFu) != 0) + (uint32_t)((d & 0xFF00u) != 0) + (uint32_t)((d & 0xFF0000u) != 0) +
         (uint32_t)((d >> 24) != 0);
}

__global__ __launch_bounds__(kBlock) void bits_size_kernel(CompactArgs a, uint32_t* __restrict__ wc,
                                                           uint32_t* __restrict__ bsum) {
  __shared__ uint32_t s_map[kWavesPerBlock][64];
  __shared__ uint32_t s_c[kWavesPerBlock];
  const uint32_t lane = threadIdx.x & 63, wave = threadIdx.x >> 6;
  const uint32_t seg = blockIdx.x * kSegsPerBlock + wave;
  uint32_t c = 0;
  if (seg < a.n_segs) {
    c = a.counts[seg];
    bits_map(a, seg, c, s_map[wave], lane);
    uint32_t z = nz_bytes(s_map[wave][lane]);
    for (int o = 32; o > 0; o >>= 1) z += __shfl_xor(z, o);
    if (lane == 0) {
      reinterpret_cast<uint32_t*>(a.out)[seg] = c | z << 16;
      wc[seg] = 8u + ((z + 3u) >> 2) + ((c + 15u) >> 4);
    }
  }
  if (lane == 0) s_c[wave] = c;
  __syncthreads();
  if (threadIdx.x == 0) bsum[blockIdx.x] = s_c[0] + s_c[1] + s_c[2] + s_c[3];
}

template <bool kSmall>
__global__ __launch_bounds__(kBlock) void bits_write_kernel(CompactArgs a, const uint32_t* __restrict__ wc,
                                                            const uint32_t* __restrict__ bsum, uint32_t* __restrict__ tot) {
  __shared__ uint32_t s_map[kWavesPerBlock][64];
  __shared__ uint32_t s_stage[kWavesPerBlock][64];
  __shared__ uint32_t s_sum[kWavesPerBlock][8];
  __shared__ uint32_t s_part[kWavesPerBlock];
  __shared__ uint32_t s_seg[kWavesPerBlock];
  const uint32_t lane = threadIdx.x & 63, wave = threadIdx.x >> 6;
  const uint32_t first = blockIdx.x * kSegsPerBlock;
  const uint32_t seg = first + wave;
  const uint32_t n = a.n_segs;
  uint32_t pre = 0;
  if constexpr (kSmall) {
    const uint4* __restrict__ w4 = reinterpret_cast<const uint4*>(wc);
    uint32_t ws = 0;
#pragma unroll 8
    for (uint32_t q = threadIdx.x; q < first / 4u; q += kBlock) {
      const uint4 v = w4[q];
      ws += (v.x + v.y) + (v.z + v.w);
    }
    for (int o = 32; o > 0; o >>= 1) ws += __shfl_xor(ws, o);
    if (lane == 0) s_part[wave] = ws;
    if (threadIdx.x < kSegsPerBlock) s_seg[threadIdx.x] = first + threadIdx.x < n ? wc[first + threadIdx.x] : 0u;
    __syncthreads();
    if (seg >= n) return;
    pre = s_part[0] + s_part[1] + s_part[2] + s_part[3];
    for (uint32_t w = 0; w < wave; ++w) pre += s_seg[w];
  } else {
    if (seg >= n) return;
    for (uint32_t x = lane; x < seg / kScanGroup; x += 64) pre += a.group_tot[x];
    for (int o = 32; o > 0; o >>= 1) pre += __shfl_xor(pre, o);
    pre += a.offsets[1 + seg];
  }
  uint32_t* __restrict__ out = reinterpret_cast<uint32_t*>(a.out);
  const uint32_t cz = out[seg];
  const uint32_t c = cz & 0xFFFFu, z = cz >> 16;
  uint32_t* __restrict__ map = s_map[wave];
  bits_map(a, seg, c, map, lane);
  uint32_t* __restrict__ dst = out + n + pre;
  const uint32_t d = map[lane];
  const uint32_t f4 = (uint32_t)((d & 0xFFu) != 0) | (uint32_t)((d & 0xFF00u) != 0) << 1 |
                      (uint32_t)((d & 0xFF0000u) != 0) << 2 | (uint32_t)((d >> 24) != 0) << 3;
  uint32_t* __restrict__ sm = s_sum[wave];
  uint32_t* __restrict__ st = s_stage[wave];
  if (lane < 8) sm[lane] = 0u;
  st[lane] = 0u;
  __builtin_amdgcn_fence(__ATOMIC_SEQ_CST, "wavefront");
  __builtin_amdgcn_wave_barrier();
  if (f4) atomicOr(&sm[lane >> 3], f4 << (4u * (lane & 7u)));
  const uint32_t cnt = (uint32_t)__popc(f4);
  const uint32_t incl = wave_incl_scan(cnt);
  uint32_t pb = incl - cnt;
  uint8_t* __restrict__ sb = reinterpret_cast<uint8_t*>(st);
#pragma unroll
  for (uint32_t j = 0; j < 4; ++j)
    if ((f4 >> j) & 1u) sb[pb++] = (uint8_t)(d >> (8u * j));
  __builtin_amdgcn_fence(__ATOMIC_SEQ_CST, "wavefront");
  __builtin_amdgcn_wave_barrier();
  if (lane < 8) __builtin_nontemporal_store(sm[lane], dst + lane);
  const uint32_t zw = (z + 3u) >> 2;
  if (lane < zw) __builtin_nontemporal_store(st[lane], dst + 8u + lane);
  uint32_t* __restrict__ codes = dst + 8u + zw;
  const uint16_t* __restrict__ rp =
      reinterpret_cast<const uint16_t*>(a.fired32 + (uint64_t)seg * a.stride + kRec16Header / 4u);
  for (uint32_t base = 0; base < c; base += 1024u) {
    const uint32_t i = base + 16u * lane;
    if (i < c) {
      const uint4* q = reinterpret_cast<const uint4*>(rp + i);
      const uint4 r0 = q[0], r1 = q[1];
      const uint32_t dd[8] = {r0.x, r0.y, r0.z, r0.w, r1.x, r1.y, r1.z, r1.w};
      uint32_t w = 0;
#pragma unroll
      for (uint32_t t = 0; t < 8; ++t) {
        w |= ((dd[t] >> 11) & 3u) << (4u * t);
        w |= ((dd[t] >> 27) & 3u) << (4u * t + 2u);
      }
      const uint32_t left = c - i;
      if (left < 16u) w &= (1u << (2u * left)) - 1u;
      __builtin_nontemporal_store(w, codes + i / 16u);
    }
  }
  if (seg == n - 1) {
    const uint32_t nb = (n + kSegsPerBlock - 1) / kSegsPerBlock;
    uint32_t r = 0;
    for (uint32_t x = lane; x < nb; x += 64) r += bsum[x];
    for (int o = 32; o > 0; o >>= 1) r += __shfl_xor(r, o);
    if (lane == 0) {
      tot[0] = n + pre + 8u + zw + ((c + 15u) >> 4);
      tot[1] = r;
      a.offsets[0] = tot[0];
      if (a.host_len) {
        a.host_len[0] = tot[0];
        a.host_len[1] = r;
      }
    }
  }
}

template <int kRec, bool kPacked = false>
__global__ __launch_bounds__(kBlock) void compact_small_kernel(CompactArgs a) {
  __shared__ uint32_t s_part[kWavesPerBlock];
  __shared__ uint32_t s_seg[kWavesPerBlock];
  const uint32_t lane = threadIdx.x & 63, wave = threadIdx.x >> 6;
  const uint32_t first = blockIdx.x * kSegsPerBlock;
  static_assert(kSegsPerBlock % 4 == 0, "prefix loads assume whole uint4s before the block");
  const uint4* __restrict__ c4 = reinterpret_cast<const uint4*>(a.counts);
  const uint32_t nq = first / 4u;
  uint32_t sum = 0;
#pragma unroll 8
  for (uint32_t q = threadIdx.x; q < nq; q += kBlock) {
    const uint4 v = c4[q];
    sum += (v.x + v.y) + (v.z + v.w);
  }
  for (int o = 32; o > 0; o >>= 1) sum += __shfl_xor(sum, o);
  if (lane == 0) s_part[wave] = sum;
  if (threadIdx.x < kSegsPerBlock) s_seg[threadIdx.x] = first + threadIdx.x < a.n_segs ? a.counts[first + threadIdx.x] : 0u;
  __syncthreads();
  const uint32_t seg = first + wave;
  if (seg >= a.n_segs) return;
  uint32_t off = s_part[0] + s_part[1] + s_part[2] + s_part[3];
  for (uint32_t w = 0; w < wave; ++w) off += s_seg[w];
  const uint32_t c = s_seg[wave];
  if (seg == a.n_segs - 1 && lane == 0) {
    a.offsets[0] = off + c;
    if (a.host_len) a.host_len[0] = off + c;
  }
  const uint32_t* __restrict__ sp = a.fired32 + (uint64_t)seg * a.stride;
  const uint32_t base = (seg >> a.seg_region_shift) * a.region_slots;
  for (uint32_t j = lane; j < c; j += 64) {
    const uint2 x = rec_at<kRec>(sp, j);
    store_out<kPacked>(a, off + j, base + x.x, x.y);
  }
}

__global__ void reduce_stats_kernel(const unsigned long long* __restrict__ cum, uint32_t n_blocks,
                                    unsigned long long* __restrict__ out) {
  const uint32_t word = blockIdx.x;
  unsigned long long s = 0;
  for (uint32_t b = threadIdx.x; b < n_blocks; b += blockDim.x) s += cum[(uint64_t)b * kStatWords + word];
  for (int off = 32; off > 0; off >>= 1) s += __shfl_xor(s, off);
  __shared__ unsigned long long part[kBlock / 64];
  if ((threadIdx.x & 63) == 0) part[threadIdx.x >> 6] = s;
  __syncthreads();
  if (threadIdx.x == 0) {
    unsigned long long t = 0;
    for (int i = 0; i < kBlock / 64; ++i) t += part[i];
    out[word] = t;
  }
}

struct ScatterArgs {
  void* st;
  StateFmt fmt;
  int64_t* due;
  int64_t* del_s;
  uint32_t* rec_idx;
  const uint32_t* slots;
  const kwk_hot* s_hot;
  const int64_t* s_del;
  const uint32_t* s_rec;
  const uint16_t* s_cls;
  uint32_t n;
  uint32_t mark_dirty;
};

__global__ void scatter_kernel(ScatterArgs a) {
  const uint32_t j = blockIdx.x * blockDim.x + threadIdx.x;
  if (j >= a.n) return;
  const uint32_t i = a.slots[j];
  kwk_hot h = a.s_hot[j];
  h.sched = (h.sched & ~KWK_CLASS_MASK) | ((uint32_t)a.s_cls[j] << KWK_CLASS_SHIFT);
  if (a.mark_dirty) h.sched |= KWK_F_DIRTY;
  store_state_due(a.st, a.due, i, make_uint2(h.pred, h.sched), h.due, a.fmt);
  a.del_s[i] = a.s_del[j];
  a.rec_idx[i] = a.s_rec[j];
}

__device__ __forceinline__ double go_pow_int(double x, uint64_t n) {
  if (n == 0 || x == 1.0) return 1.0;
  if (n == 1) return x;
  if (x == 0.0 || isinf(x) || isnan(x)) return pow(x, (double)n);
  double a1 = 1.0;
  int ae = 0;
  int xe;
  double x1 = frexp(x, &xe);
  for (uint64_t i = n; i != 0; i >>= 1) {
    if (xe < -(1 << 12) || (1 << 12) < xe) {
      ae += xe;
      break;
    }
    if (i & 1) {
      a1 *= x1;
      ae += xe;
    }
    x1 *= x1;
    xe <<= 1;
    if (x1 < 0.5) {
      x1 += x1;
      xe--;
    }
  }
  return ldexp(a1, ae);
}

__device__ __forceinline__ int64_t go_duration(double d) {
  if (!(d > -9223372036854775808.0 && d < 9223372036854775808.0)) return INT64_MIN;
  return (int64_t)d;
}

struct RetryArgs {
  void* st;
  StateFmt fmt;
  int64_t* due;
  const uint32_t* slots;
  const kwk_hot* hot;
  const uint16_t* cls;
  const uint16_t* stages;
  const uint32_t* retry_count;
  kwk_backoff b;
  uint32_t n;
  uint64_t slot_base;
  uint64_t key;
  uint64_t step;
  int64_t now;
};

__global__ void retry_kernel(RetryArgs a) {
  const uint32_t j = blockIdx.x * blockDim.x + threadIdx.x;
  if (j >= a.n) return;
  const uint32_t i = a.slots[j];
  const double d = fmin((double)a.b.duration_ns * go_pow_int(a.b.factor, a.retry_count[j]), (double)a.b.cap_ns);
  const int64_t base = go_duration(d);
  const double mf = a.b.jitter <= 0.0 ? 1.0 : a.b.jitter;
  const double u = rng_float64(a.slot_base + i, a.step, kSiteRetryJitter, a.key);
  const int64_t delay = base + go_duration(u * mf * (double)base);
  const uint32_t sched = (a.hot[j].sched & ~(KWK_CLASS_MASK | 0xFFu | KWK_F_DIRTY)) |
                         ((uint32_t)a.cls[j] << KWK_CLASS_SHIFT) | (uint32_t)a.stages[j];
  store_state_due(a.st, a.due, i, make_uint2(a.hot[j].pred, sched), sat_add(a.now, delay), a.fmt);
}

__global__ void delete_kernel(void* st, StateFmt fmt, const uint32_t* slots, uint32_t n) {
  const uint32_t j = blockIdx.x * blockDim.x + threadIdx.x;
  if (j >= n) return;
  const uint32_t i = slots[j];
  uint2 v = load_state(st, i, fmt);
  v.y = (v.y & ~(KWK_F_ALIVE | KWK_F_DIRTY | 0xFFu)) | KWK_STAGE_NONE;
  store_state(st, i, v, fmt);
}

__global__ void dw_fold_kernel(uint2* __restrict__ st, const int64_t* __restrict__ due, uint32_t first, uint32_t n,
                               int64_t epoch) {
  for (uint32_t j = blockIdx.x * blockDim.x + threadIdx.x; j < n; j += gridDim.x * blockDim.x) {
    const uint32_t i = first + j;
    st[i] = dw_put(st[i], dw_enc(due[i], epoch));
  }
}
__global__ void dw_unfold_kernel(const uint2* __restrict__ st, int64_t* __restrict__ due, uint32_t first, uint32_t n,
                                 int64_t epoch) {
  for (uint32_t j = blockIdx.x * blockDim.x + threadIdx.x; j < n; j += gridDim.x * blockDim.x) {
    const uint32_t i = first + j;
    const uint64_t d = dw_get(st[i]);
    if (d != kDwFar) due[i] = dw_abs(d, epoch);
  }
}

constexpr uint32_t kURun = 16;
constexpr uint32_t kURow = 64u * kURun;
constexpr uint32_t kUChunkRows = 4;
constexpr uint32_t kUChunkPods = kURow - 8u;
constexpr uint32_t kUChunkNodes = 128;
constexpr uint32_t kULdsValues = 512;
constexpr int kMaxCountMasks = 16;
struct UsageArgs {
  const void* __restrict__ st;
  StateFmt fmt;
  const uint32_t* __restrict__ node_ptr;
  const uint32_t* __restrict__ ukey;
  const double* __restrict__ cpu_v;
  const double* __restrict__ mem_v;
  uint32_t n_cpu, n_mem;
  const uint4* __restrict__ chunks;
  uint32_t n_chunks;
  uint32_t n_pods;
  double* __restrict__ node_out;
  double* __restrict__ cum;
  int64_t* __restrict__ last_t;
  int64_t now;
  double* __restrict__ block_part;
  double* __restrict__ pod_out;
  double* __restrict__ pod_cum;
  int64_t* __restrict__ pod_last;
  const uint2* __restrict__ mixed;
  const uint32_t* __restrict__ ckeys;
  const uint32_t* __restrict__ mbase;
  double* __restrict__ ccum;
  const double* __restrict__ podv;
  uint32_t podv_n;
  const uint8_t* __restrict__ ukey8;
  const double2* __restrict__ kv;
  uint32_t kv_n;
  const uint32_t* __restrict__ cmasks;
  uint32_t n_cmasks;
  uint32_t* __restrict__ cpart;
};
struct UsageDynArgs {
  const uint2* __restrict__ progs;
  uint32_t n_cpu_progs, n_mem_progs;
  const kwk_metric_op* __restrict__ uops;
  uint32_t n_uops;
  const int64_t* __restrict__ pod_created;
  const int64_t* __restrict__ node_created;
  double zero_time_unix_s;
  double* __restrict__ unit_val;
  double* __restrict__ cval;
};
constexpr uint32_t kUKeyDict = 256;
constexpr uint32_t kUKeyZero = 255;
constexpr uint32_t kUSeqKeys = 16;

constexpr uint32_t kUKeyMixedIndex = 0x0FFFFFFFu;

__device__ __forceinline__ double dur_seconds(int64_t d) {
  return (double)(d / 1000000000) + (double)(d % 1000000000) / 1e9;
}

__device__ __forceinline__ double since_seconds(int64_t now, int64_t created) {
  if (created == INT64_MIN) return 9223372036.854775807;
  int64_t d;
  if (__builtin_sub_overflow(now, created, &d)) d = now > created ? INT64_MAX : INT64_MIN;
  return dur_seconds(d);
}

constexpr uint32_t kULdsOps = 256;
constexpr uint32_t kULdsProgs = 256;
constexpr uint32_t kUStack = 8;

__device__ __forceinline__ double qfloat_approx(double v) {
  const double x = v * 10e9;
  const int64_t n = (x >= -9223372036854775808.0 && x < 9223372036854775808.0) ? (int64_t)x : INT64_MIN;
  return (double)n * 1e-9;
}

__device__ __noinline__ double run_usage_program(const kwk_metric_op* ops, uint32_t n_ops, int64_t now,
                                                 int64_t pod_created, int64_t node_created, double zero_time_unix_s) {
  double s[kUStack] = {0.0, 0.0, 0.0, 0.0, 0.0, 0.0, 0.0, 0.0};
  auto push = [&](double v) {
#pragma unroll
    for (int i = kUStack - 1; i > 0; --i) s[i] = s[i - 1];
    s[0] = v;
  };
  auto drop = [&](int from) {
#pragma unroll
    for (int i = 1; i < (int)kUStack - 1; ++i)
      if (i >= from) s[i] = s[i + 1];
  };
  for (uint32_t i = 0; i < n_ops; ++i) {
    const kwk_metric_op op = ops[i];
    switch (op.op) {
      case KWK_MOP_CONST: push(op.value); break;
      case KWK_MOP_LOAD: {
        double v;
        if (op.arg == KWK_MIN_NOW_S) v = (double)now / 1e9;
        else if (op.arg == KWK_MIN_POD_SINCE) v = since_seconds(now, pod_created);
        else if (op.arg == KWK_MIN_NODE_SINCE) v = since_seconds(now, node_created);
        else {
          const int64_t c = op.arg == KWK_MIN_POD_CREATED ? pod_created : node_created;
          v = c == INT64_MIN ? zero_time_unix_s : (double)c / 1e9;
        }
        push(v);
        break;
      }
      case KWK_MOP_ADD: s[0] = s[1] + s[0]; drop(1); break;
      case KWK_MOP_SUB: s[0] = s[1] - s[0]; drop(1); break;
      case KWK_MOP_MUL: s[0] = s[1] * s[0]; drop(1); break;
      case KWK_MOP_DIV: s[0] = s[1] / s[0]; drop(1); break;
      case KWK_MOP_NEG: s[0] = -s[0]; break;
      case KWK_MOP_QFLOAT: s[0] = qfloat_approx(s[0]); break;
      case KWK_MOP_LT: s[0] = s[1] < s[0] ? 1.0 : 0.0; drop(1); break;
      case KWK_MOP_LE: s[0] = s[1] <= s[0] ? 1.0 : 0.0; drop(1); break;
      case KWK_MOP_GT: s[0] = s[1] > s[0] ? 1.0 : 0.0; drop(1); break;
      case KWK_MOP_GE: s[0] = s[1] >= s[0] ? 1.0 : 0.0; drop(1); break;
      case KWK_MOP_SELECT: s[0] = s[2] != 0.0 ? s[1] : s[0]; drop(1); drop(1); break;
      default: break;
    }
  }
  return s[0];
}

template <uint32_t WB>
__device__ __forceinline__ bool run_alive(const uint4 (&sv)[WB], int j, uint32_t abit, bool px) {
  if constexpr (WB == 1) {
    const uint4 c = sv[0];
    const int d = j >> 2;
    const uint32_t w = d == 0 ? c.x : d == 1 ? c.y : d == 2 ? c.z : c.w;
    return ((w >> (8 * (j & 3))) & abit) != 0;
  } else if constexpr (WB == 2) {
    const uint4 c = sv[j >> 3];
    const int d = (j >> 1) & 3;
    const uint32_t w = d == 0 ? c.x : d == 1 ? c.y : d == 2 ? c.z : c.w;
    return ((w >> (16 * (j & 1))) & abit) != 0;
  } else if constexpr (WB == 4) {
    const uint4 c = sv[j >> 2];
    const int d = j & 3;
    return ((d == 0 ? c.x : d == 1 ? c.y : d == 2 ? c.z : c.w) & abit) != 0;
  } else {
    const uint4 c = sv[j >> 1];
    return ((px ? ((j & 1) ? c.z : c.x) : ((j & 1) ? c.w : c.y)) & abit) != 0;
  }
}

__device__ __forceinline__ uint32_t alive16_ids(const uint4 c) {
  const uint32_t dw[4] = {c.x, c.y, c.z, c.w};
  uint32_t m = 0;
#pragma unroll
  for (int d = 0; d < 4; ++d) {
    const uint32_t a = (dw[d] >> 5) & 0x01010101u;
    m |= (((a * 0x204081u) >> 21) & 15u) << (4 * d);
  }
  return m;
}

template <int C, int RM>
__device__ __forceinline__ double dpp_f64(double v) {
  const uint64_t b = (uint64_t)__double_as_longlong(v);
  const uint32_t lo = (uint32_t)__builtin_amdgcn_update_dpp(0, (int)(uint32_t)b, C, RM, 0xF, false);
  const uint32_t hi = (uint32_t)__builtin_amdgcn_update_dpp(0, (int)(uint32_t)(b >> 32), C, RM, 0xF, false);
  return __longlong_as_double((long long)(((uint64_t)hi << 32) | lo));
}
template <int C, int RM>
__device__ __forceinline__ uint32_t dpp_key(uint32_t v) {
  return (uint32_t)__builtin_amdgcn_update_dpp((int)0xFFFFFFFFu, (int)v, C, RM, 0xF, false);
}
template <int C, int RM>
__device__ __forceinline__ void dpp_seg_step(double& sc, double& sm, const uint32_t key) {
  const double uc = dpp_f64<C, RM>(sc), um = dpp_f64<C, RM>(sm);
// ... 2186 lines not shown

kwk_status kwk_load(kwk_engine* e, uint32_t n, const kwk_hot* hot, const int64_t* del, const uint32_t* rec,
                    const uint16_t* cls, uint32_t n_records, const kwk_value* records) {
  ErrScope es_(e ? &e->err : nullptr);
  if (!e || (n && (!hot || !del || !rec || !cls))) return fail(KWK_EINVAL, "null argument");
  if (n > e->capacity) return fail(KWK_ECAP, "n exceeds capacity");
  if (n_records > e->max_records) return fail(KWK_ECAP, "n_records exceeds max_records");
  for (uint32_t i = 0; i < n; ++i) {
    if ((hot[i].sched & KWK_F_HASREC) && rec[i] >= n_records)
      return fail(KWK_EINVAL, "object " + std::to_string(i) + ": record index out of range");
    if (e->loaded_table && cls[i] >= e->n_classes)
      return fail(KWK_EINVAL, "object " + std::to_string(i) + ": class out of range");
  }
  if (kwk_status st = set_dev(e)) return st;
  HIP_TRY(hipStreamSynchronize(e->stream));
  {
    std::vector<uint2> st(n);
    std::vector<int64_t> due(n);
    for (uint32_t i = 0; i < n; ++i) {
      st[i] = make_uint2(hot[i].pred, (hot[i].sched & ~KWK_CLASS_MASK) | ((uint32_t)cls[i] << KWK_CLASS_SHIFT));
      if (!fits_fmt(e->fmt, e->n_stages, st[i].x, st[i].y))
        return fail(KWK_EINVAL, "object " + std::to_string(i) + ": pred bits / stage beyond the loaded stage table");
      due[i] = hot[i].due;
    }
    StateFmt nf;
    if (kwk_status s2 = pick_format(e, st, nf)) return s2;
    e->fmt = nf;
    const std::vector<uint8_t> raw = pack_words(e, st, e->fmt);
    HIP_TRY(hipMemcpyAsync(e->d_st, raw.data(), raw.size(), hipMemcpyHostToDevice, e->stream));
    HIP_TRY(hipMemcpyAsync(e->d_due, due.data(), sizeof(int64_t) * n, hipMemcpyHostToDevice, e->stream));
    if (kwk_status s2 = dw_fold(e, 0, n)) return s2;
    HIP_TRY(hipStreamSynchronize(e->stream));
  }
  HIP_TRY(upload(e, e->d_del, del, sizeof(int64_t) * n));
  HIP_TRY(upload(e, e->d_rec, rec, sizeof(uint32_t) * n));
  if (n_records)
    HIP_TRY(upload(e, e->d_values, records, sizeof(kwk_value) * (size_t)n_records * e->value_slots));
  if (n < e->n_active)
    HIP_TRY(hipMemsetAsync((char*)e->d_st.get() + word_bytes(e->fmt) * n, 0, word_bytes(e->fmt) * (size_t)(e->n_active - n), e->stream));
  e->n_active = n;
  return KWK_OK;
}

kwk_status kwk_set_records(kwk_engine* e, uint32_t first, uint32_t n, const kwk_value* records) {
  ErrScope es_(e ? &e->err : nullptr);
  if (!e || (n && !records)) return fail(KWK_EINVAL, "null argument");
  if ((uint64_t)first + n > e->max_records) return fail(KWK_ECAP, "records exceed max_records");
  if (kwk_status st = set_dev(e)) return st;
  HIP_TRY(upload(e, e->d_values + (size_t)first * e->value_slots, records, sizeof(kwk_value) * (size_t)n * e->value_slots));
  return KWK_OK;
}

static kwk_status scatter_rows(kwk_engine* e, uint32_t n, const uint32_t* slots, const kwk_hot* hot, const int64_t* del,
                               const uint32_t* rec, const uint16_t* cls, uint32_t mark_dirty);

kwk_status kwk_upsert(kwk_engine* e, uint32_t n, const uint32_t* slots, const kwk_hot* hot, const int64_t* del,
                      const uint32_t* rec, const uint16_t* cls) {
  ErrScope es_(e ? &e->err : nullptr);
  return scatter_rows(e, n, slots, hot, del, rec, cls, 1u);
}

kwk_status kwk_replace(kwk_engine* e, uint32_t n, const uint32_t* slots, const kwk_hot* hot, const int64_t* del,
                       const uint32_t* rec, const uint16_t* cls) {
  ErrScope es_(e ? &e->err : nullptr);
  return scatter_rows(e, n, slots, hot, del, rec, cls, 0u);
}

static kwk_status scatter_rows(kwk_engine* e, uint32_t n, const uint32_t* slots, const kwk_hot* hot, const int64_t* del,
                               const uint32_t* rec, const uint16_t* cls, uint32_t mark_dirty) {
  if (!e || (n && (!slots || !hot || !del || !rec || !cls))) return fail(KWK_EINVAL, "null argument");
  if (n == 0) return KWK_OK;
  uint32_t max_slot = 0;
  for (uint32_t j = 0; j < n; ++j) {
    if (slots[j] >= e->capacity) return fail(KWK_ECAP, "slot beyond capacity");
    if (e->loaded_table && cls[j] >= e->n_classes) return fail(KWK_EINVAL, "class out of range");
    if ((hot[j].sched & KWK_F_HASREC) && rec[j] >= e->max_records) return fail(KWK_EINVAL, "record out of range");
    if (!fits_fmt(e->fmt, e->n_stages, hot[j].pred, hot[j].sched))
      return fail(KWK_EINVAL, "pred bits / stage beyond the loaded stage table");
    max_slot = slots[j] > max_slot ? slots[j] : max_slot;
  }
  if (kwk_status st = set_dev(e)) return st;
  {
    std::vector<uint2> rows(n);
    for (uint32_t j = 0; j < n; ++j)
      rows[j] = make_uint2(hot[j].pred, (hot[j].sched & ~KWK_CLASS_MASK) | ((uint32_t)cls[j] << KWK_CLASS_SHIFT) |
                                            (mark_dirty ? KWK_F_DIRTY : 0u));
    if (kwk_status st = admit_rows(e, rows)) return st;
  }
  const size_t bytes = (size_t)n * (4 + sizeof(kwk_hot) + 8 + 4 + 2) + 64;
  if (kwk_status st = ensure_stage_buf(e, bytes)) return st;
  HIP_TRY(hipStreamSynchronize(e->stream));
  char* p = (char*)e->d_stage_buf.get();
  kwk_hot* s_hot = (kwk_hot*)p; p += sizeof(kwk_hot) * n;
  int64_t* s_del = (int64_t*)p; p += 8 * (size_t)n;
  uint32_t* s_slots = (uint32_t*)p; p += 4 * (size_t)n;
  uint32_t* s_rec = (uint32_t*)p; p += 4 * (size_t)n;
  uint16_t* s_cls = (uint16_t*)p;
  HIP_TRY(upload(e, s_hot, hot, sizeof(kwk_hot) * n));
  HIP_TRY(upload(e, s_del, del, 8 * (size_t)n));
  HIP_TRY(upload(e, s_slots, slots, 4 * (size_t)n));
  HIP_TRY(upload(e, s_rec, rec, 4 * (size_t)n));
  HIP_TRY(upload(e, s_cls, cls, 2 * (size_t)n));
  if (max_slot + 1 > e->n_active) {
    HIP_TRY(hipMemsetAsync((char*)e->d_st.get() + word_bytes(e->fmt) * e->n_active, 0,
                           word_bytes(e->fmt) * (size_t)(max_slot + 1 - e->n_active), e->stream));
    e->n_active = max_slot + 1;
  }
  ScatterArgs a{e->d_st, e->fmt, e->d_due, e->d_del, e->d_rec, s_slots, s_hot, s_del, s_rec, s_cls, n, mark_dirty};
  hipLaunchKernelGGL(scatter_kernel, dim3((n + kBlock - 1) / kBlock), dim3(kBlock), 0, e->stream, a);
  HIP_TRY(hipGetLastError());
  HIP_TRY(hipStreamSynchronize(e->stream));
  return KWK_OK;
}

kwk_status kwk_delete(kwk_engine* e, uint32_t n, const uint32_t* slots) {
  ErrScope es_(e ? &e->err : nullptr);
  if (!e || (n && !slots)) return fail(KWK_EINVAL, "null argument");
  if (n == 0) return KWK_OK;
  for (uint32_t j = 0; j < n; ++j)
    if (slots[j] >= e->n_active) return fail(KWK_EINVAL, "slot not active");
  if (kwk_status st = set_dev(e)) return st;
  if (kwk_status st = ensure_stage_buf(e, 4 * (size_t)n)) return st;
  HIP_TRY(hipStreamSynchronize(e->stream));
  HIP_TRY(upload(e, e->d_stage_buf, slots, 4 * (size_t)n));
  hipLaunchKernelGGL(delete_kernel, dim3((n + kBlock - 1) / kBlock), dim3(kBlock), 0, e->stream, e->d_st,
                     e->fmt, (const uint32_t*)e->d_stage_buf.get(), n);
  HIP_TRY(hipGetLastError());
  HIP_TRY(hipStreamSynchronize(e->stream));
  return KWK_OK;
}

kwk_status kwk_retry(kwk_engine* e, int64_t now_ns, uint64_t seed, uint64_t step, uint32_t n, const uint32_t* slots,
                     const kwk_hot* hot, const uint16_t* cls, const uint16_t* stages, const uint32_t* retry_count,
                     const kwk_backoff* backoff) {
  ErrScope es_(e ? &e->err : nullptr);
  if (!e || !backoff || (n && (!slots || !hot || !cls || !stages || !retry_count)))
    return fail(KWK_EINVAL, "null argument");
  if (n == 0) return KWK_OK;
  for (uint32_t j = 0; j < n; ++j) {
    if (slots[j] >= e->n_active) return fail(KWK_EINVAL, "slot not active");
    if (stages[j] >= e->n_stages) return fail(KWK_EINVAL, "stage out of range");
    if (e->loaded_table && cls[j] >= e->n_classes) return fail(KWK_EINVAL, "class out of range");
    if (!(hot[j].sched & KWK_F_ALIVE)) return fail(KWK_EINVAL, "retried object must be alive");
    if (!fits_fmt(e->fmt, e->n_stages, hot[j].pred, stages[j])) return fail(KWK_EINVAL, "pred bits beyond the stage table");
  }
  if (kwk_status st = set_dev(e)) return st;
  {
    std::vector<uint2> rows(n);
    for (uint32_t j = 0; j < n; ++j)
      rows[j] = make_uint2(hot[j].pred, (hot[j].sched & ~(KWK_CLASS_MASK | 0xFFu | KWK_F_DIRTY)) |
                                            ((uint32_t)cls[j] << KWK_CLASS_SHIFT) | (uint32_t)stages[j]);
    if (kwk_status st = admit_rows(e, rows)) return st;
  }
  const size_t bytes = (size_t)n * (4 + sizeof(kwk_hot) + 2 + 2 + 4) + 64;
  if (kwk_status st = ensure_stage_buf(e, bytes)) return st;
  HIP_TRY(hipStreamSynchronize(e->stream));
  char* p = (char*)e->d_stage_buf.get();
  kwk_hot* s_hot = (kwk_hot*)p; p += sizeof(kwk_hot) * n;
  uint32_t* s_slots = (uint32_t*)p; p += 4 * (size_t)n;
  uint32_t* s_rc = (uint32_t*)p; p += 4 * (size_t)n;
  uint16_t* s_cls = (uint16_t*)p; p += 2 * (size_t)n;
  uint16_t* s_stg = (uint16_t*)p;
  HIP_TRY(upload(e, s_hot, hot, sizeof(kwk_hot) * n));
  HIP_TRY(upload(e, s_slots, slots, 4 * (size_t)n));
  HIP_TRY(upload(e, s_rc, retry_count, 4 * (size_t)n));
  HIP_TRY(upload(e, s_cls, cls, 2 * (size_t)n));
  HIP_TRY(upload(e, s_stg, stages, 2 * (size_t)n));
  RetryArgs a{e->d_st, e->fmt, e->d_due, s_slots, s_hot, s_cls, s_stg, s_rc, *backoff, n, e->slot_base,
              seed ^ ((uint64_t)e->kind_salt << 32), step, now_ns};
  hipLaunchKernelGGL(retry_kernel, dim3((n + kBlock - 1) / kBlock), dim3(kBlock), 0, e->stream, a);
  HIP_TRY(hipGetLastError());
  HIP_TRY(hipStreamSynchronize(e->stream));
  return KWK_OK;
}

static uint32_t persist_grid(kwk_engine* e, const void* kernel, uint32_t tiles) {
  int per_cu = 0;
  for (const auto& kv : e->occupancy)
    if (kv.first == kernel) per_cu = kv.second;
  if (per_cu == 0) {
    if (hipOccupancyMaxActiveBlocksPerMultiprocessor(&per_cu, kernel, kBlock, 0) != hipSuccess || per_cu <= 0) per_cu = 1;
    e->occupancy.emplace_back(kernel, per_cu);
  }
  const uint32_t g = (uint32_t)e->n_cus * (uint32_t)per_cu;
  return tiles < g ? tiles : g;
}

static SweepArgs sweep_args(kwk_engine* e, int64_t now_ns, uint64_t seed, uint64_t step, bool fire) {
  SweepArgs a;
  a.st = e->d_st;
  a.due = e->d_due;
  a.del_s = e->d_del;
  a.rec_idx = e->d_rec;
  a.values = e->d_values;
  a.table = e->d_table;
  a.deltas = e->d_deltas;
  a.lut = e->d_lut;
  a.lut_n = e->lut_n;
  a.lut_bytes = e->lut_bytes;
  a.lut_rest = e->lut_rest;
  a.fired = e->d_fired;
  a.wave_counts = e->d_wave_counts;
  a.cum = e->d_cum;
  a.n = e->n_active;
  a.value_slots = e->value_slots;
  a.slot_base = e->slot_base;
  a.key = seed ^ ((uint64_t)e->kind_salt << 32);
  a.step = step;
  a.now = now_ns;
  a.fire = fire ? 1u : 0u;
  a.fmt = e->fmt;
  if (e->fmt.narrow) {
    const uint32_t fs = e->fmt.fshift;
    a.raw = RawTest{(KWK_F_MANAGED >> 8) << fs, (KWK_F_DIRTY >> 8) << fs, (KWK_F_ALIVE >> 8) << fs, e->fmt.sshift,
                    e->fmt.smask, e->fmt.none_code, e->harness.terminal_mask & e->fmt.pmask,
                    e->harness.deletion_bit & e->fmt.pmask};
  } else {
    a.raw = RawTest{KWK_F_MANAGED, KWK_F_DIRTY, KWK_F_ALIVE, 0, 0xFFu, KWK_STAGE_NONE, e->harness.terminal_mask,
                    e->harness.deletion_bit};
  }
  a.harness = e->harness;
  if (!fire) a.harness.enable = 0;
  a.fsm = nullptr;
  a.fsm_due = nullptr;
  a.fsm_bits = 0;
  a.comp = nullptr;
  a.dw_epoch_old = e->fmt.epoch;
  a.dw_rebase = 0;
  a.tail = SweepArgs::TailHb{nullptr, nullptr, nullptr, nullptr, 0u, 0u};
  return a;
}

static kwk_status build_fsm(kwk_engine* e) {
  e->fsm_harness = -1;
  e->byte_ok = false;
  if (!e->fmt.half || !e->loaded_table || !e->use_fsm) return KWK_OK;
  const uint32_t bits = e->fmt.fshift + 5;
  if (bits > 16) return KWK_OK;
  if (e->fsm_bits != bits || !e->d_fsm) {
    e->d_fsm.reset();
    HIP_TRY(e->d_fsm_due.alloc(2u << bits));
    HIP_TRY(e->d_fsm.alloc(2u << bits));
    e->fsm_bits = bits;
  }
  SweepArgs a = sweep_args(e, 0, 0, 0, true);
  a.fsm_bits = bits;
  const uint32_t n = 2u << bits;
  if (a.harness.enable)
    hipLaunchKernelGGL(fsm_build_kernel<true>, dim3((n + kBlock - 1) / kBlock), dim3(kBlock), 0, e->stream, a, e->d_fsm,
                       e->d_fsm_due);
  else
    hipLaunchKernelGGL(fsm_build_kernel<false>, dim3((n + kBlock - 1) / kBlock), dim3(kBlock), 0, e->stream, a, e->d_fsm,
                       e->d_fsm_due);
  HIP_TRY(hipGetLastError());
  HIP_TRY(hipStreamSynchronize(e->stream));
  e->fsm_harness = a.harness.enable ? 1 : 0;
  e->h_fsm.resize(n);
  e->h_fsm_due.resize(n);
  HIP_TRY(hipMemcpy(e->h_fsm.data(), e->d_fsm, sizeof(uint32_t) * n, hipMemcpyDeviceToHost));
  HIP_TRY(hipMemcpy(e->h_fsm_due.data(), e->d_fsm_due, sizeof(int64_t) * n, hipMemcpyDeviceToHost));
  e->byte_ok = true;
  return KWK_OK;
}

struct TailReq {
  uint32_t slot;
  HbFmt mode;
  bool done;
};
static void hb_tail_args(kwk_engine* e, const TailReq& t, SweepArgs& a);


using SweepKernel = void (*)(SweepArgs);

static const void* sweep8_pick(bool persistent, uint32_t depth, bool stages4, uint32_t steps) {
  static const SweepKernel k[3][4] = {
      {sweep8_kernel<true, 2, true, 4>, sweep8_kernel<true, 2, true, 2>, sweep8_kernel<true, 2, true>,
       sweep8_kernel<true, 2, false>},
      {sweep8_kernel<true, 1, true, 4>, sweep8_kernel<true, 1, true, 2>, sweep8_kernel<true, 1, true>,
       sweep8_kernel<true, 1, false>},
      {sweep8_kernel<false, 1, true, 4>, sweep8_kernel<false, 1, true, 2>, sweep8_kernel<false, 1, true>,
       sweep8_kernel<false, 1, false>}};
  return (const void*)k[persistent ? (depth == 2 ? 0 : 1) : 2][steps == 4 ? 0 : steps == 2 ? 1 : stages4 ? 2 : 3];
}

static const void* sweep16_pick(bool harness, uint32_t q, bool lean, bool persistent, uint32_t depth) {
  static const SweepKernel k[3][2][5] = {
      {{sweep16_fsm_kernel<true, 4, true, 2>, sweep16_fsm_kernel<true, 4, true, 1>, sweep16_kernel<true, 4, true>,
        sweep16_fsm_kernel<true, 4, false, 1>, sweep16_kernel<true, 4, false>},
       {sweep16_fsm_kernel<false, 4, true, 2>, sweep16_fsm_kernel<false, 4, true, 1>, sweep16_kernel<false, 4, true>,
        sweep16_fsm_kernel<false, 4, false, 1>, sweep16_kernel<false, 4, false>}},
      {{sweep16_fsm_kernel<true, 1, true, 2>, sweep16_fsm_kernel<true, 1, true, 1>, sweep16_kernel<true, 1, true>,
        sweep16_fsm_kernel<true, 1, false, 1>, sweep16_kernel<true, 1, false>},
       {sweep16_fsm_kernel<false, 1, true, 2>, sweep16_fsm_kernel<false, 1, true, 1>, sweep16_kernel<false, 1, true>,
        sweep16_fsm_kernel<false, 1, false, 1>, sweep16_kernel<false, 1, false>}},
      {{sweep16_fsm_kernel<true, 2, true, 2>, sweep16_fsm_kernel<true, 2, true, 1>, sweep16_kernel<true, 2, true>,
        sweep16_fsm_kernel<true, 2, false, 1>, sweep16_kernel<true, 2, false>},
       {sweep16_fsm_kernel<false, 2, true, 2>, sweep16_fsm_kernel<false, 2, true, 1>, sweep16_kernel<false, 2, true>,
        sweep16_fsm_kernel<false, 2, false, 1>, sweep16_kernel<false, 2, false>}}};
  const int v = persistent ? (lean ? (depth == 2 ? 0 : 1) : 2) : (lean ? 3 : 4);
  return (const void*)k[q == 4 ? 0 : q == 1 ? 1 : 2][harness ? 0 : 1][v];
}

static const void* sweepw_pick(bool harness, bool dw, bool narrow) {
  static const SweepKernel k[3][2] = {{sweepw_kernel<true, 8, true>, sweepw_kernel<false, 8, true>},
                                      {sweepw_kernel<true, 4>, sweepw_kernel<false, 4>},
                                      {sweepw_kernel<true, 8>, sweepw_kernel<false, 8>}};
  return (const void*)k[dw ? 0 : narrow ? 1 : 2][harness ? 0 : 1];
}

static kwk_status launch_sweep(kwk_engine* e, int64_t now_ns, uint64_t seed, uint64_t step, bool fire,
                               uint32_t steps = 1, int64_t dt_ns = 0, TailReq* tail = nullptr) {
  const bool fuse = steps > 1;
  if (!e) return fail(KWK_EINVAL, "null engine");
  if (!e->loaded_table) return fail(KWK_ESTATE, "kwk_load_stages must be called before kwk_step");
  e->compacted = false;
  e->last_sweep = kwk_sweep_info{};
  e->last_step_no = step + (steps ? steps - 1 : 0);
  if (e->n_active == 0) { e->last_blocks = 0; e->steps += steps; return KWK_OK; }
  SweepArgs a = sweep_args(e, now_ns, seed, step, fire);
  const bool nar = e->fmt.narrow != 0, dw = e->fmt.dw != 0;
  const bool h = a.harness.enable != 0;
  if (e->fmt.half && fire && e->fsm_harness == (h ? 1 : 0)) {
    a.fsm = e->d_fsm;
    a.fsm_due = e->d_fsm_due;
    a.fsm_bits = e->fsm_bits;
  }

  uint32_t K, region_shift = 0;
  int rec = kRecSlot;
  uint32_t q16 = e->q16;
  bool lean = false, s4 = false;
  if (e->fmt.byte) {
    if (!fire) return fail(KWK_ESTATE, "the 1-byte format sweeps with fire only");
    a.fsm = e->d_fsm8;
    a.fsm_due = e->d_fsm8_due;
    a.fsm_bits = e->fsm8_due_any ? kId8AnyDue : 0u;
    s4 = e->n_stages <= 4;
    if (fuse) {
      if (!s4 || (steps != 2 && steps != 4)) return fail(KWK_ESTATE, "fused steps: 2 or 4, 1-byte sweep with <= 4 stages");
      for (uint32_t i = 0; i + 1 < steps; ++i) {
        if (!e->d_firedx[i]) return fail(KWK_ESTATE, "fused steps: buffers not allocated");
        a.firedx[i] = e->d_firedx[i];
        a.countsx[i] = e->d_countsx[i];
        a.nowx[i] = now_ns + (int64_t)(i + 1) * dt_ns;
      }
      a.comp = e->d_comp8 + (steps == 4 ? 256 : 0);
    }
    K = 16 * kQ8;
    rec = s4 ? kRecId8Half : kRecId8;
  } else if (e->fmt.half) {
    if (q16 > 1 && (e->n_active + kBlock * 8 * q16 - 1) / (kBlock * 8 * q16) < 4u * (uint32_t)e->n_cus) q16 = 1;
    K = 8 * q16;
    lean = a.fsm && e->fsm_kernel;
  } else {
    K = dw ? (uint32_t)kQWD * 2u : (uint32_t)kQW * (nar ? 4u : 2u);
    region_shift = 2;
    static_assert(kWavesPerBlock == 4, "region shift");
  }
  const uint32_t tile = kBlock * K;
  const uint32_t tiles = (e->n_active + tile - 1) / tile;

  const void* kern;
  uint32_t blocks = tiles;
  if (e->fmt.byte || e->fmt.half) {
    const uint32_t depth = e->fmt.byte ? e->fsm_kernel : lean ? e->fsm_kernel : 1;
    const void* pk = e->fmt.byte ? sweep8_pick(true, depth, s4, steps) : sweep16_pick(h, q16, lean, true, depth);
    const uint32_t pg = e->persist16 ? persist_grid(e, pk, tiles) : tiles;
    const uint32_t kind = e->fmt.byte ? KWK_SWEEP_8 : lean ? KWK_SWEEP_16_FSM : KWK_SWEEP_16;
    e->last_sweep = kwk_sweep_info{kind, e->fmt.byte ? (uint32_t)kQ8 : q16, 0, 1, tiles, tiles, h ? 1u : 0u, 0};
    if (2 * pg <= tiles) {
      blocks = pg;
      e->last_sweep.persistent = 1;
      e->last_sweep.grid = pg;
      e->last_sweep.depth = depth;
      kern = pk;
    } else if (e->fmt.byte) {
      kern = sweep8_pick(false, 1, s4, steps);
    } else {
      if (lean && tail && tiles * 4u <= (uint32_t)e->n_cus && tiles * kWavesPerBlock <= e->compact_small) {
        hb_tail_args(e, *tail, a);
        tail->done = true;
      }
      kern = sweep16_pick(h, q16, lean, false, 1);
    }
    if (e->fmt.byte) e->last_sweep.steps = steps;
  } else {
    const uint32_t tpb = e->word_tpb ? e->word_tpb : dw ? 8u : 4u;
    blocks = e->word_tpb ? (tiles + tpb - 1) / tpb
                         : std::min(tiles, std::max((tiles + tpb - 1) / tpb, (uint32_t)e->n_cus * 5u));
    if (dw) {
      const int64_t e0 = e->fmt.epoch;
      if (now_ns < e0 || (uint64_t)now_ns - (uint64_t)e0 > kDwRebase) {
        a.fmt.epoch = now_ns;
        a.dw_rebase = 1;
      }
    }
    kern = sweepw_pick(h, dw, nar);
    e->last_sweep = kwk_sweep_info{dw ? (uint32_t)KWK_SWEEP_WD : nar ? (uint32_t)KWK_SWEEP_W4 : (uint32_t)KWK_SWEEP_W8,
                                   (uint32_t)(dw ? kQWD : kQW), blocks < tiles ? 1u : 0u,
                                   blocks < tiles ? 2u : 1u , blocks, tiles, h ? 1u : 0u, 0};
  }

  void* args[] = {&a};
  HIP_TRY(hipLaunchKernel(kern, dim3(blocks), dim3(kBlock), args, 0, e->stream));
  HIP_TRY(hipGetLastError());

  if (dw) e->fmt.epoch = a.fmt.epoch;
  e->last_objs = K;
  e->last_region_shift = region_shift;
  e->last_rec = rec;
  e->last_blocks = tiles;
  e->last_grid = blocks;
  e->cum_rows = blocks > e->cum_rows ? blocks : e->cum_rows;
  e->steps += steps;
  return KWK_OK;
}

kwk_status kwk_step(kwk_engine* e, int64_t now_ns, uint64_t seed, uint64_t step) {
  ErrScope es_(e ? &e->err : nullptr);
  return launch_sweep(e, now_ns, seed, step, true);
}

kwk_status kwk_match(kwk_engine* e, int64_t now_ns, uint64_t seed, uint64_t step) {
  ErrScope es_(e ? &e->err : nullptr);
  if (!e) return fail(KWK_EINVAL, "null engine");
  if (kwk_status st = set_dev(e)) return st;
  if (kwk_status st = leave_byte(e)) return st;
  return launch_sweep(e, now_ns, seed, step, false);
}

kwk_status kwk_sync(kwk_engine* e) {
  ErrScope es_(e ? &e->err : nullptr);
  if (!e) return fail(KWK_EINVAL, "null engine");
  if (kwk_status st = set_dev(e)) return st;
  HIP_TRY(hipStreamSynchronize(e->stream));
  return KWK_OK;
}


static bool hb_fmt_of(uint32_t code, HbFmt* f) {
  switch (code) {
    case KWK_COMPACT_REC: *f = HbFmt::Rec; return true;
    case KWK_COMPACT_PACKED: *f = HbFmt::Packed; return true;
    case KWK_COMPACT_PACKED16: *f = HbFmt::Packed16; return true;
    case KWK_COMPACT_BITS: *f = HbFmt::Bits; return true;
  }
  return false;
}
static uint32_t hb_code(HbFmt f) {
  switch (f) {
    case HbFmt::Packed: return KWK_COMPACT_PACKED;
    case HbFmt::Packed16: return KWK_COMPACT_PACKED16;
    case HbFmt::Bits: return KWK_COMPACT_BITS;
    case HbFmt::Rec: break;
  }
  return KWK_COMPACT_REC;
}
static HbFmt hb_fmt_of_compact(uint32_t compact) {
  HbFmt f = HbFmt::Rec;
  hb_fmt_of(compact, &f);
  return f;
}
static uint32_t hb_record_bytes(HbFmt f) {
  return f == HbFmt::Packed16 ? 2u : f == HbFmt::Rec ? (uint32_t)sizeof(kwk_fired_rec) : 4u;
}
static bool hb_segmented(HbFmt f) { return f == HbFmt::Packed16 || f == HbFmt::Bits; }
static HbFmt current_fmt(const kwk_engine* e) { return e->hb[e->hb_cur].mode; }

static uint32_t hb_next(const kwk_engine* e, uint32_t k = 1) { return (e->hb_cur + k) % (uint32_t)e->hb.size(); }

static size_t hb_list_bytes(const kwk_engine* e, HbFmt mode) {
  if (mode == HbFmt::Bits) return 4u * ((size_t)e->n_blocks_cap * kWavesPerBlock * 201u + 64u);
  return (size_t)hb_record_bytes(mode) * (size_t)e->capacity + 64u;
}

static kwk_status hb_prepare(kwk_engine* e, uint32_t i, HbFmt mode, hipStream_t stream) {
  kwk_engine::HbSlot& h = e->hb[i];
  if (h.copy_pending) {
    HIP_TRY(hipStreamWaitEvent(stream, h.ev_copied, 0));
    h.copy_pending = false;
  }
  const size_t need = hb_list_bytes(e, mode);
  HIP_TRY(h.list.grow(need));
  if (!h.offsets) {
    const size_t n_waves = (size_t)e->n_blocks_cap * kWavesPerBlock;
    HIP_TRY(h.offsets.alloc(n_waves + 4));
    HIP_TRY(h.groups.alloc(n_waves / kScanGroup + 4));
    HIP_TRY(h.tot.alloc(16));
    HIP_TRY(h.counts.alloc(n_waves + 4));
  }
  if (e->hb_track) HIP_TRY(h.ev_done.create(hipEventDisableTiming));
  return KWK_OK;
}

static kwk_status hb_commit(kwk_engine* e, uint32_t i, uint64_t step, HbFmt mode, uint32_t n_segs, int done_slot,
                            hipStream_t stream, bool record) {
  kwk_engine::HbSlot& h = e->hb[i];
  h.valid = true;
  h.step = step;
  h.mode = mode;
  h.n_segs = n_segs;
  h.region_slots = n_segs ? 64u * e->last_objs << e->last_region_shift : 0u;
  h.done_slot = done_slot;
  e->hb_cur = i;
  e->compacted = true;
  if (e->hb_track && record) HIP_TRY(hipEventRecord(h.ev_done, stream));
  return KWK_OK;
}

static void hb_args(const kwk_engine* e, uint32_t i, HbFmt mode, CompactArgs& a) {
  const kwk_engine::HbSlot& h = e->hb[i];
  a.out = reinterpret_cast<kwk_fired_rec*>(h.list.get());
  a.offsets = h.offsets;
  a.group_tot = h.groups;
  a.counts_out = mode == HbFmt::Packed16 ? h.counts : nullptr;
  a.host_len = e->hb_track ? e->h_len_dev + 2u * i : nullptr;
  a.n_segs = e->last_blocks * kWavesPerBlock;
  a.seg_region_shift = e->last_region_shift;
  a.region_slots = 64u * e->last_objs << e->last_region_shift;
  a.stride = 64u * e->last_objs + 32u;
}

static void hb_tail_args(kwk_engine* e, const TailReq& t, SweepArgs& a) {
  const kwk_engine::HbSlot& h = e->hb[t.slot];
  if (++e->tail_seq == 0) e->tail_seq = 1;
  a.tail = SweepArgs::TailHb{h.list, h.offsets, e->hb_track ? e->h_len_dev + 2u * t.slot : nullptr, e->d_tail_status,
                             e->tail_seq, t.mode == HbFmt::Packed ? 1u : 0u};
}

using BitsWriteKernel = void (*)(CompactArgs, const uint32_t*, const uint32_t*, uint32_t*);
static const void* compact_pick(HbFmt mode, int rec, bool small) {
  constexpr uint32_t W = kCompactSpw;
  static_assert(std::is_same<decltype(&bits_write_kernel<true>), BitsWriteKernel>::value &&
                    std::is_same<decltype(&bits_write_kernel<false>), BitsWriteKernel>::value &&
                    std::is_same<decltype(&compact16_small_kernel), void (*)(CompactArgs)>::value &&
                    std::is_same<decltype(&compact16_kernel<kCompact16Spw>), void (*)(CompactArgs)>::value &&
                    std::is_same<decltype(&compact_small_kernel<kRecSlot>), void (*)(CompactArgs)>::value &&
                    std::is_same<decltype(&compact_kernel<kRecSlot, false, W>), void (*)(CompactArgs)>::value,
                "enqueue_compact's argument array");
  static const void* const k[2][8] = {
      {(const void*)bits_write_kernel<true>, (const void*)compact16_small_kernel,
       (const void*)compact_small_kernel<kRecId8Half, true>, (const void*)compact_small_kernel<kRecId8, true>,
       (const void*)compact_small_kernel<kRecSlot, true>, (const void*)compact_small_kernel<kRecId8Half>,
       (const void*)compact_small_kernel<kRecId8>, (const void*)compact_small_kernel<kRecSlot>},
      {(const void*)bits_write_kernel<false>, (const void*)compact16_kernel<kCompact16Spw>,
       (const void*)compact_kernel<kRecId8Half, true, W>, (const void*)compact_kernel<kRecId8, true, W>,
       (const void*)compact_kernel<kRecSlot, true, W>, (const void*)compact_kernel<kRecId8Half, false, W>,
       (const void*)compact_kernel<kRecId8, false, W>, (const void*)compact_kernel<kRecSlot, false, W>}};
  const int r = rec == kRecId8Half ? 0 : rec == kRecId8 ? 1 : 2;
  const int col = mode == HbFmt::Bits ? 0 : mode == HbFmt::Packed16 ? 1 : mode == HbFmt::Packed ? 2 + r : 5 + r;
  return k[small ? 0 : 1][col];
}

static kwk_status launch_compact16(const kwk_engine* e, hipStream_t stream, uint32_t n_waves, CompactArgs4& c4,
                                   uint32_t m) {
  constexpr uint32_t W16 = kCompact16Spw;
  const bool small = n_waves <= e->compact_small;
  const uint32_t spb = small ? kSmall16Spb : W16 * kWavesPerBlock;
  const dim3 grid((n_waves + spb - 1) / spb, m);
  const dim3 scan_grid((n_waves + kScanGroup - 1) / kScanGroup, m);
  CompactArgs& a = c4.a[0];
  if (m > 1) {
    if (small) {
      hipLaunchKernelGGL(compact16_small_multi_kernel, grid, dim3(kBlock), 0, stream, c4);
    } else {
      hipLaunchKernelGGL(seg_scan_multi_kernel, scan_grid, dim3(kBlock), 0, stream, c4);
      hipLaunchKernelGGL(compact16_multi_kernel<W16>, grid, dim3(kBlock), 0, stream, c4);
    }
  } else {
    if (!small)
      hipLaunchKernelGGL(seg_scan_kernel, scan_grid, dim3(kBlock), 0, stream, a.counts, n_waves, a.offsets,
                         const_cast<uint32_t*>(a.group_tot));
    void* args[] = {&a};
    HIP_TRY(hipLaunchKernel(compact_pick(HbFmt::Packed16, e->last_rec, small), grid, dim3(kBlock), args, 0, stream));
  }
  HIP_TRY(hipGetLastError());
  return KWK_OK;
}

static kwk_status enqueue_compact(kwk_engine* e, HbFmt mode) {
  const hipStream_t stream = e->stream;
  const uint32_t n_waves = e->last_blocks * kWavesPerBlock;
  if (hb_segmented(mode) && e->last_rec != kRecId8Half) mode = HbFmt::Packed;
  const uint32_t i = hb_next(e);
  if (kwk_status st = hb_prepare(e, i, mode, stream)) return st;
  kwk_engine::HbSlot& h = e->hb[i];
  if (n_waves == 0) {
    HIP_TRY(hipMemsetAsync(h.offsets, 0, sizeof(uint32_t), stream));
    HIP_TRY(hipMemsetAsync(h.tot, 0, 2 * sizeof(uint32_t), stream));
    if (e->hb_track) HIP_TRY(hipMemsetAsync(e->h_len_dev + 2u * i, 0, 2 * sizeof(uint32_t), stream));
    return hb_commit(e, i, e->last_step_no, mode, 0, (int)i, stream, true);
  }
  CompactArgs4 c4;
  CompactArgs& a = c4.a[0];
  a.fired32 = reinterpret_cast<const uint32_t*>(e->d_fired.get());
  a.counts = e->d_wave_counts;
  hb_args(e, i, mode, a);
  if (mode == HbFmt::Packed16) {
    if (kwk_status st = launch_compact16(e, stream, n_waves, c4, 1)) return st;
  } else {
    const bool bits = mode == HbFmt::Bits, small = n_waves <= e->compact_small;
    const uint32_t blocks = (n_waves + kSegsPerBlock - 1) / kSegsPerBlock;
    const uint32_t eblocks = (n_waves + kCompactSpw * kWavesPerBlock - 1) / (kCompactSpw * kWavesPerBlock);
    if (bits)
      hipLaunchKernelGGL(bits_size_kernel, dim3(blocks), dim3(kBlock), 0, stream, a, e->d_bits_wc, e->d_bits_bsum);
    if (!small)
      hipLaunchKernelGGL(seg_scan_kernel, dim3((n_waves + kScanGroup - 1) / kScanGroup), dim3(kBlock), 0, stream,
                         bits ? e->d_bits_wc : e->d_wave_counts, n_waves, h.offsets, h.groups);
    const uint32_t* wc = e->d_bits_wc;
    const uint32_t* bsum = e->d_bits_bsum;
    uint32_t* tot = h.tot;
    void* args[] = {&a, &wc, &bsum, &tot};
    HIP_TRY(hipLaunchKernel(compact_pick(mode, e->last_rec, small), dim3(bits || small ? blocks : eblocks), dim3(kBlock),
                            args, 0, stream));
    HIP_TRY(hipGetLastError());
  }
  return hb_commit(e, i, e->last_step_no, mode, n_waves, (int)i, stream, true);
}

static kwk_status packed_ok(const kwk_engine* e) {
  if (e->capacity > kPackedSlots) return fail(KWK_ECAP, "packed fired records hold 27-bit slots: engine capacity > 2^27");
  return KWK_OK;
}

static kwk_status sweep_compact(kwk_engine* e, int64_t now, uint64_t seed, uint64_t step, bool compact, HbFmt mode,
                                int ev_a = -1) {
  TailReq tr{0u, mode == HbFmt::Rec ? HbFmt::Rec : HbFmt::Packed, false};
  const bool try_tail = compact && e->tail_hb && e->fmt.half && !e->fmt.byte && e->loaded_table;
  if (try_tail) {
    tr.slot = hb_next(e);
    if (kwk_status st = hb_prepare(e, tr.slot, tr.mode, e->stream)) return st;
  }
  if (ev_a >= 0)
    if (kwk_status st = kwk_event_record(e, (uint32_t)ev_a)) return st;
  if (kwk_status st = launch_sweep(e, now, seed, step, true, 1, 0, try_tail ? &tr : nullptr)) return st;
  if (ev_a >= 0)
    if (kwk_status st = kwk_event_record(e, (uint32_t)ev_a + 1u)) return st;
  if (!compact) return KWK_OK;
  if (tr.done)
    return hb_commit(e, tr.slot, e->last_step_no, tr.mode, e->last_blocks * kWavesPerBlock, (int)tr.slot, e->stream,
                     true);
  return enqueue_compact(e, mode);
}

static kwk_status step_one(kwk_engine* e, int64_t now, uint64_t seed, uint64_t step, uint32_t compact, int ev_a = -1) {
  return sweep_compact(e, now, seed, step, compact != 0, hb_fmt_of_compact(compact), ev_a);
}

static uint32_t fuse_group(const kwk_engine* e, uint32_t left, uint32_t ev_every) {
  if (e->fuse_steps < 2 || !e->fmt.byte || e->n_stages > 4 || e->fsm8_due_any || !e->loaded_table || ev_every == 1)
    return 1;
  uint32_t m = e->fuse_steps;
  while (ev_every && m > 2 && m > ev_every) m >>= 1;
  while (m > left) m >>= 1;
  return m ? m : 1;
}

static kwk_status step_group(kwk_engine* e, uint32_t m, int64_t now, int64_t dt, uint64_t seed, uint64_t step,
                             uint32_t compact, int ev_a) {
  for (uint32_t i = 0; i + 1 < m; ++i) {
    if (e->d_firedx[i]) continue;
    const size_t n_waves = (size_t)e->n_blocks_cap * kWavesPerBlock;
    HIP_TRY(e->d_firedx[i].alloc((size_t)e->n_blocks_cap * kBlock * kMinObjPerThread + (size_t)kBlock * kMaxObjPerThread));
    HIP_TRY(e->d_countsx[i].alloc(n_waves + 4));
  }
  if (ev_a >= 0)
    if (kwk_status st = kwk_event_record(e, (uint32_t)ev_a)) return st;
  if (kwk_status st = launch_sweep(e, now, seed, step, true, m, dt)) return st;
  if (ev_a >= 0)
    if (kwk_status st = kwk_event_record(e, (uint32_t)ev_a + 1u)) return st;
  const uint32_t n_waves = e->last_blocks * kWavesPerBlock;
  if (compact == KWK_COMPACT_PACKED16 && e->last_rec == kRecId8Half && n_waves) {
    CompactArgs4 c4;
    for (uint32_t i = 0; i < m; ++i)
      if (kwk_status st = hb_prepare(e, hb_next(e, i + 1), HbFmt::Packed16, e->stream)) return st;
    for (uint32_t i = 0; i < m; ++i) {
      CompactArgs& a = c4.a[i];
      a.fired32 = reinterpret_cast<const uint32_t*>((i ? e->d_firedx[i - 1] : e->d_fired).get());
      a.counts = i ? e->d_countsx[i - 1] : e->d_wave_counts;
      hb_args(e, hb_next(e, i + 1), HbFmt::Packed16, a);
    }
    if (kwk_status st = launch_compact16(e, e->stream, n_waves, c4, m)) return st;
    for (uint32_t i = 1; i < m; ++i) {
      std::swap(e->d_fired, e->d_firedx[i - 1]);
      std::swap(e->d_wave_counts, e->d_countsx[i - 1]);
    }
    const uint32_t last = hb_next(e, m);
    for (uint32_t i = 0; i < m; ++i) {
      const uint32_t slot = hb_next(e, 1);
      if (kwk_status st = hb_commit(e, slot, step + i, HbFmt::Packed16, n_waves, (int)last, e->stream, i + 1 == m))
        return st;
    }
    return KWK_OK;
  }
  for (uint32_t i = 0; i < m; ++i) {
    if (i) {
      std::swap(e->d_fired, e->d_firedx[i - 1]);
      std::swap(e->d_wave_counts, e->d_countsx[i - 1]);
      e->compacted = false;
    }
    if (compact) {
      e->last_step_no = step + i;
      if (kwk_status st = enqueue_compact(e, hb_fmt_of_compact(compact))) return st;
    }
  }
  e->last_step_no = step + m - 1;
  return KWK_OK;
}

static int ev_of(uint32_t ev_every, uint32_t j) {
  return ev_every && j % ev_every == 0 ? (int)(2u * (j / ev_every)) : -1;
}
static int ev_of_group(uint32_t ev_every, uint32_t j, uint32_t m) {
  for (uint32_t i = 0; i < m; ++i)
    if (ev_of(ev_every, j + i) >= 0) return ev_of(ev_every, j + i);
  return -1;
}

kwk_status kwk_step_n(kwk_engine* e, uint32_t n, int64_t now0_ns, int64_t dt_ns, uint64_t seed, uint64_t step0,
                      uint32_t compact, uint32_t ev_every, uint32_t ev_j0) {
  ErrScope es_(e ? &e->err : nullptr);
  if (!e) return fail(KWK_EINVAL, "null engine");
  if (compact == KWK_COMPACT_PACKED || compact == KWK_COMPACT_PACKED16)
    if (kwk_status st = packed_ok(e)) return st;
  if (kwk_status st = set_dev(e)) return st;
  for (uint32_t k = 0; k < n;) {
    const uint32_t j = ev_j0 + k;
    const uint32_t m = fuse_group(e, n - k, ev_every);
    if (m > 1) {
      if (kwk_status st = step_group(e, m, now0_ns + (int64_t)k * dt_ns, dt_ns, seed, step0 + k, compact,
                                     ev_of_group(ev_every, j, m)))
        return st;
      k += m;
      continue;
    }
    if (kwk_status st = step_one(e, now0_ns + (int64_t)k * dt_ns, seed, step0 + k, compact, ev_of(ev_every, j)))
      return st;
    ++k;
  }
  return KWK_OK;
}

kwk_status kwk_step_n_pair(kwk_engine* e, kwk_engine* other, uint32_t n, int64_t now0_ns, int64_t dt_ns, uint64_t seed,
                           uint64_t step0, uint32_t compact, uint32_t ev_every, uint32_t ev_j0) {
  ErrScope es_(e ? &e->err : nullptr);
  if (!e || !other) return fail(KWK_EINVAL, "null engine");
  if (e == other) return fail(KWK_EINVAL, "the two engines must differ");
  if (e->device != other->device) return fail(KWK_EINVAL, "the two engines are on different devices");
  if (compact == KWK_COMPACT_PACKED || compact == KWK_COMPACT_PACKED16) {
    if (kwk_status st = packed_ok(e)) return st;
    if (other->capacity > kPackedSlots) return fail(KWK_ECAP, "packed fired records hold 27-bit slots: other engine > 2^27");
  }
  if (kwk_status st = set_dev(e)) return st;
  for (uint32_t k = 0; k < n;) {
    const uint32_t j = ev_j0 + k;
    const int64_t now = now0_ns + (int64_t)k * dt_ns;
    const uint32_t m = fuse_group(e, n - k, ev_every);
    if (m > 1) {
      if (kwk_status st = step_group(e, m, now, dt_ns, seed, step0 + k, compact, ev_of_group(ev_every, j, m))) return st;
    } else if (kwk_status st = step_one(e, now, seed, step0 + k, compact, ev_of(ev_every, j))) {
      return st;
    }
    for (uint32_t i = 0; i < m; ++i)
      if (kwk_status st = step_one(other, now + (int64_t)i * dt_ns, seed, step0 + k + i, compact, -1)) return st;
    k += m;
  }
  return KWK_OK;
}

kwk_status kwk_fired_keep(kwk_engine* e, uint32_t depth) {
  ErrScope es_(e ? &e->err : nullptr);
  if (!e) return fail(KWK_EINVAL, "null engine");
  if (depth > kHbMax) return fail(KWK_EINVAL, "kwk_fired_keep: depth 0.." + std::to_string(kHbMax));
  if (kwk_status st = set_dev(e)) return st;
  HIP_TRY(hipStreamSynchronize(e->stream));
  if (e->copy_stream) HIP_TRY(hipStreamSynchronize(e->copy_stream));
  const uint32_t slots = depth > kHbMin ? depth : kHbMin;
  kwk_engine::HbSlot cur = std::move(e->hb[e->hb_cur]);
  e->hb.clear();
  e->hb.resize(slots);
  cur.copy_pending = false;
  e->hb[0] = std::move(cur);
  e->hb_cur = 0;
  e->hb_track = depth > 0;
  if (e->hb_track && !e->h_len) {
    HIP_TRY(e->h_len.alloc(2 * kHbMax));
    memset(e->h_len, 0, 2 * sizeof(uint32_t) * kHbMax);
    void* dev = nullptr;
    HIP_TRY(hipHostGetDevicePointer(&dev, e->h_len, 0));
    e->h_len_dev = static_cast<uint32_t*>(dev);
  }
  e->hb[0].done_slot = 0;
  if (e->hb_track && e->hb[0].offsets) {
    HIP_TRY(e->hb[0].ev_done.create(hipEventDisableTiming));
    const bool bits = e->hb[0].mode == HbFmt::Bits;
    e->h_len[1] = 0u;
    HIP_TRY(hipMemcpy(e->h_len, bits ? e->hb[0].tot : e->hb[0].offsets, (bits ? 2 : 1) * sizeof(uint32_t),
                      hipMemcpyDeviceToHost));
    HIP_TRY(hipEventRecord(e->hb[0].ev_done, e->stream));
  }
  return KWK_OK;
}

static kwk_status hb_fetch(kwk_engine* e, uint32_t i, void* out, uint64_t cap_bytes, uint32_t* seg_counts,
                           uint32_t seg_cap, kwk_fetch_info* info) {
  kwk_engine::HbSlot& h = e->hb[i];
  if (!e->copy_stream) {
    int prio = 0;
    HIP_TRY(hipStreamGetPriority(e->stream, &prio));
    HIP_TRY(hipStreamCreateWithPriority(&e->copy_stream, hipStreamNonBlocking, prio));
    HIP_TRY(e->ev_count.create(hipEventDisableTiming));
    HIP_TRY(e->h_count.alloc(16));
  }
  HIP_TRY(h.ev_copied.create(hipEventDisableTiming));
  const bool bits = h.mode == HbFmt::Bits, b16 = h.mode == HbFmt::Packed16;
  const uint32_t rb = hb_record_bytes(h.mode);
  const bool segs = b16 && seg_counts && h.n_segs;
  if (segs && h.n_segs > seg_cap) return fail(KWK_ECAP, "segment buffer too small: need " + std::to_string(h.n_segs));
  uint32_t t[2] = {0u, 0u};
  hipEvent_t done = nullptr;
  if (e->hb_track && h.done_slot >= 0 && e->hb[h.done_slot].ev_done) {
    done = e->hb[h.done_slot].ev_done;
    HIP_TRY(hipEventSynchronize(done));
    t[0] = e->h_len[2u * i];
    t[1] = e->h_len[2u * i + 1u];
  } else {
    HIP_TRY(hipMemcpyAsync(e->h_count, bits ? h.tot : h.offsets, 2 * sizeof(uint32_t), hipMemcpyDeviceToHost, e->stream));
    HIP_TRY(hipEventRecord(e->ev_count, e->stream));
    HIP_TRY(hipEventSynchronize(e->ev_count));
    done = e->ev_count;
    t[0] = e->h_count[0];
    t[1] = e->h_count[1];
  }
  if (!h.n_segs) t[0] = t[1] = 0u;
  const uint32_t total = t[0];
  info->n_records = bits ? t[1] : total;
  info->record_bytes = bits ? 0u : rb;
  info->format = hb_code(h.mode);
  info->bytes = (uint64_t)total * rb;
  info->step = h.step;
  if (b16 || bits) {
    info->n_segs = h.n_segs;
    info->region_slots = h.region_slots;
  }
  if (out && (uint64_t)total * rb > cap_bytes)
    return fail(KWK_ECAP, "fired buffer too small: need " + std::to_string((uint64_t)total * rb) + " bytes");
  HIP_TRY(hipStreamWaitEvent(e->copy_stream, done, 0));
  if (out && total) HIP_TRY(hipMemcpyAsync(out, h.list, (size_t)total * rb, hipMemcpyDeviceToHost, e->copy_stream));
  if (segs)
    HIP_TRY(hipMemcpyAsync(seg_counts, h.counts, sizeof(uint32_t) * h.n_segs, hipMemcpyDeviceToHost, e->copy_stream));
  HIP_TRY(hipEventRecord(h.ev_copied, e->copy_stream));
  h.copy_pending = true;
  e->copy_recorded = true;
  return KWK_OK;
}

static kwk_status fired_prologue(kwk_engine* e, uint32_t format, HbFmt* f) {
  if (!hb_fmt_of(format, f)) return fail(KWK_EINVAL, "format: KWK_COMPACT_REC, _PACKED, _PACKED16 or _BITS");
  if (*f == HbFmt::Packed)
    if (kwk_status st = packed_ok(e)) return st;
  return set_dev(e);
}

kwk_status kwk_fired_compact(kwk_engine* e, uint32_t format) {
  ErrScope es_(e ? &e->err : nullptr);
  if (!e) return fail(KWK_EINVAL, "null engine");
  HbFmt f;
  if (kwk_status st = fired_prologue(e, format, &f)) return st;
  return enqueue_compact(e, f);
}

kwk_status kwk_fired_device(kwk_engine* e, uint32_t format, const void** list, const uint32_t** count) {
  ErrScope es_(e ? &e->err : nullptr);
  if (!e || !list || !count) return fail(KWK_EINVAL, "null argument");
  HbFmt f;
  if (!hb_fmt_of(format, &f)) return fail(KWK_EINVAL, "format: KWK_COMPACT_REC, _PACKED, _PACKED16 or _BITS");
  if (!e->compacted || current_fmt(e) != f)
    return fail(KWK_ESTATE, "kwk_fired_compact in this format must follow kwk_step");
  *list = e->hb[e->hb_cur].list;
  *count = f == HbFmt::Bits ? e->hb[e->hb_cur].tot : e->hb[e->hb_cur].offsets;
  return KWK_OK;
}

kwk_status kwk_fired_read(kwk_engine* e, uint32_t format, void* out, uint64_t cap_bytes, uint32_t* seg_counts,
                          uint32_t seg_cap, kwk_fetch_info* info) {
  ErrScope es_(e ? &e->err : nullptr);
  if (!e || !info) return fail(KWK_EINVAL, "null argument");
  HbFmt f;
  if (kwk_status st = fired_prologue(e, format, &f)) return st;
  const bool bits = f == HbFmt::Bits;
  const uint32_t rb = hb_record_bytes(f);
  const uint32_t n_waves = e->last_blocks * kWavesPerBlock;
  memset(info, 0, sizeof(*info));
  info->format = format;
  info->record_bytes = bits ? 0u : rb;
  info->step = e->last_step_no;
  if (hb_segmented(f)) {
    info->n_segs = n_waves;
    info->region_slots = 64u * e->last_objs << e->last_region_shift;
  }
  if (n_waves == 0) return KWK_OK;
  if (!e->compacted || current_fmt(e) != f) {
    if (hb_segmented(f) && e->last_rec != kRecId8Half)
      return fail(KWK_ESTATE, std::string(bits ? "the bitmap hand-back is" : "2-byte records are") +
                                  " the 1-byte sweep's with at most 4 stages: use KWK_COMPACT_PACKED");
    if (kwk_status st = enqueue_compact(e, f)) return st;
  }
  const kwk_engine::HbSlot& h = e->hb[e->hb_cur];
  uint32_t t[2] = {0u, 0u};
  HIP_TRY(hipMemcpyAsync(t, bits ? h.tot : h.offsets, (bits ? 2 : 1) * sizeof(uint32_t), hipMemcpyDeviceToHost,
                         e->stream));
  HIP_TRY(hipStreamSynchronize(e->stream));
  const uint32_t total = t[0];
  info->n_records = bits ? t[1] : total;
  info->bytes = (uint64_t)total * rb;
  const bool segs = f == HbFmt::Packed16 && seg_counts;
  if (!out && !segs) return KWK_OK;
  if (out && info->bytes > cap_bytes)
    return fail(KWK_ECAP, "fired buffer too small: need " + std::to_string(total) + (bits ? " words" : ""));
  if (segs && n_waves > seg_cap) return fail(KWK_ECAP, "segment buffer too small: need " + std::to_string(n_waves));
  if (out && total) HIP_TRY(hipMemcpyAsync(out, h.list, (size_t)total * rb, hipMemcpyDeviceToHost, e->stream));
  if (segs) HIP_TRY(hipMemcpyAsync(seg_counts, h.counts, sizeof(uint32_t) * n_waves, hipMemcpyDeviceToHost, e->stream));
  HIP_TRY(hipStreamSynchronize(e->stream));
  return KWK_OK;
}

kwk_status kwk_fired_fetch(kwk_engine* e, uint64_t step, void* out, uint64_t cap_bytes, uint32_t* seg_counts,
                           uint32_t seg_cap, kwk_fetch_info* info) {
  ErrScope es_(e ? &e->err : nullptr);
  if (!e || !info) return fail(KWK_EINVAL, "null argument");
  if (kwk_status st = set_dev(e)) return st;
  memset(info, 0, sizeof(*info));
  const uint32_t n = (uint32_t)e->hb.size();
  if (step == KWK_STEP_LAST) {
    if (e->last_blocks == 0) return KWK_OK;
    if (!e->compacted) return fail(KWK_ESTATE, "kwk_fired_fetch needs the step's list compacted (kwk_fired_compact)");
    return hb_fetch(e, e->hb_cur, out, cap_bytes, seg_counts, seg_cap, info);
  }
  for (uint32_t k = 0; k < n; ++k) {
    const uint32_t i = (e->hb_cur + n - k) % n;
    if (e->hb[i].valid && e->hb[i].step == step) return hb_fetch(e, i, out, cap_bytes, seg_counts, seg_cap, info);
  }
  return fail(KWK_ESTATE, "no kept list of step " + std::to_string(step) + " (the ring holds the last " +
                              std::to_string(n) + " compactions: kwk_fired_keep)");
}

static kwk_status hb_view(const kwk_engine* e, uint32_t i, kwk_fired_view* out) {
  const kwk_engine::HbSlot& h = e->hb[i];
  if (!h.list || !h.offsets) return fail(KWK_ESTATE, "the ring slot of step " + std::to_string(h.step) + " holds no list");
  out->list = h.list;
  out->count = h.mode == HbFmt::Bits ? h.tot : h.offsets;
  out->seg_counts = h.mode == HbFmt::Packed16 ? h.counts : nullptr;
  out->format = hb_code(h.mode);
  out->n_segs = h.n_segs;
  out->region_slots = h.region_slots;
  out->step = h.step;
  return KWK_OK;
}

kwk_status kwk_ring_view(kwk_engine* e, uint64_t step, kwk_fired_view* out) {
  ErrScope es_(e ? &e->err : nullptr);
  if (!e || !out) return fail(KWK_EINVAL, "null argument");
  memset(out, 0, sizeof(*out));
  const uint32_t n = (uint32_t)e->hb.size();
  if (step == KWK_STEP_LAST) {
    if (!e->compacted) return fail(KWK_ESTATE, "kwk_ring_view needs the step's list compacted (kwk_fired_compact)");
    return hb_view(e, e->hb_cur, out);
  }
  for (uint32_t k = 0; k < n; ++k) {
    const uint32_t i = (e->hb_cur + n - k) % n;
    if (e->hb[i].valid && e->hb[i].step == step) return hb_view(e, i, out);
  }
  return fail(KWK_ESTATE, "no kept list of step " + std::to_string(step) + " (the ring holds the last " +
                              std::to_string(n) + " compactions: kwk_fired_keep)");
}

kwk_status kwk_fired_fetch_wait(kwk_engine* e) {
  ErrScope es_(e ? &e->err : nullptr);
  if (!e) return fail(KWK_EINVAL, "null engine");
  if (kwk_status st = set_dev(e)) return st;
  if (e->copy_recorded) HIP_TRY(hipStreamSynchronize(e->copy_stream));
  return KWK_OK;
}

kwk_status kwk_alloc_host(uint64_t bytes, void** out) {
  if (!out) return fail(KWK_EINVAL, "null argument");
  *out = nullptr;
  if (bytes == 0) return KWK_OK;
  HIP_TRY(hipHostMalloc(out, bytes, hipHostMallocDefault));
  return KWK_OK;
}

kwk_status kwk_free_host(void* p) {
  if (p) HIP_TRY(hipHostFree(p));
  return KWK_OK;
}

kwk_status kwk_stats(kwk_engine* e, kwk_step_stats* out) {
  ErrScope es_(e ? &e->err : nullptr);
  if (!e || !out) return fail(KWK_EINVAL, "null argument");
  if (kwk_status st = set_dev(e)) return st;
  hipLaunchKernelGGL(reduce_stats_kernel, dim3(kStatWords), dim3(kBlock), 0, e->stream, e->d_cum, e->cum_rows,
                     e->d_stats);
  HIP_TRY(hipGetLastError());
  unsigned long long h[kStatWords];
  HIP_TRY(hipMemcpyAsync(h, e->d_stats, sizeof(h), hipMemcpyDeviceToHost, e->stream));
  HIP_TRY(hipStreamSynchronize(e->stream));
  memset(out, 0, sizeof(*out));
  out->steps = e->steps;
  out->matched = h[0];
  out->fired = h[1];
  out->bytes = h[2];
  for (int s = 0; s < KWK_MAX_STAGES; ++s) out->fired_per_stage[s] = h[3 + s];
  out->line_bytes = h[kStatLine];
  out->state_bytes = word_bytes(e->fmt);
  return KWK_OK;
}

kwk_status kwk_read(kwk_engine* e, uint32_t first, uint32_t n, kwk_hot* hot, int64_t* del) {
  ErrScope es_(e ? &e->err : nullptr);
  if (!e) return fail(KWK_EINVAL, "null engine");
  if ((uint64_t)first + n > e->capacity) return fail(KWK_EINVAL, "range beyond capacity");
  if (kwk_status st = set_dev(e)) return st;
  HIP_TRY(hipStreamSynchronize(e->stream));
  if (hot) {
    std::vector<uint8_t> raw(word_bytes(e->fmt) * (size_t)n);
    std::vector<int64_t> due(n);
    HIP_TRY(hipMemcpy(raw.data(), (const char*)e->d_st.get() + word_bytes(e->fmt) * first, raw.size(), hipMemcpyDeviceToHost));
    HIP_TRY(hipMemcpy(due.data(), e->d_due + first, sizeof(int64_t) * n, hipMemcpyDeviceToHost));
    const std::vector<uint2> st = unpack_words(e, raw, e->fmt, n);
    if (e->fmt.dw) {
      const uint2* r = reinterpret_cast<const uint2*>(raw.data());
      for (uint32_t i = 0; i < n; ++i) {
        const uint64_t d = dw_get(r[i]);
        if (d != kDwFar) due[i] = dw_abs(d, e->fmt.epoch);
      }
    }
    for (uint32_t i = 0; i < n; ++i) hot[i] = kwk_hot{st[i].x, st[i].y, due[i]};
  }
  if (del) HIP_TRY(hipMemcpy(del, e->d_del + first, sizeof(int64_t) * n, hipMemcpyDeviceToHost));
  return KWK_OK;
}

static kwk_status check_usage_program(const kwk_metric_op* ops, kwk_usage_prog pr, uint32_t n_ops) {
  if (pr.n_ops == 0 || pr.n_ops > 64 || (uint64_t)pr.first_op + pr.n_ops > n_ops) return fail(KWK_EINVAL, "usage program ops range");
  int depth = 0;
  for (uint32_t i = pr.first_op; i < pr.first_op + pr.n_ops; ++i) {
    const kwk_metric_op& op = ops[i];
    const std::string at = " (op " + std::to_string(i) + ": " + std::to_string(op.op) + ")";
    if (op.op == KWK_MOP_CONST || op.op == KWK_MOP_LOAD) {
      if (++depth > (int)kUStack) return fail(KWK_EINVAL, "usage program deeper than 8" + at);
      if (op.op == KWK_MOP_LOAD && op.arg != KWK_MIN_NOW_S && op.arg != KWK_MIN_POD_SINCE && op.arg != KWK_MIN_NODE_SINCE &&
          op.arg != KWK_MIN_POD_CREATED && op.arg != KWK_MIN_NODE_CREATED)
        return fail(KWK_EINVAL, "usage program loads input " + std::to_string(op.arg) + at);
    } else if (op.op == KWK_MOP_NEG || op.op == KWK_MOP_QFLOAT) {
      if (depth < 1) return fail(KWK_EINVAL, "usage program underflow" + at);
    } else if ((op.op >= KWK_MOP_ADD && op.op <= KWK_MOP_DIV) || (op.op >= KWK_MOP_LT && op.op <= KWK_MOP_GE)) {
      if (depth < 2) return fail(KWK_EINVAL, "usage program underflow" + at);
      --depth;
    } else if (op.op == KWK_MOP_SELECT) {
      if (depth < 3) return fail(KWK_EINVAL, "usage program underflow" + at);
      depth -= 2;
    } else {
      return fail(KWK_EINVAL, "usage program op" + at);
    }
  }
  if (depth != 1) return fail(KWK_EINVAL, "a usage program leaves one value");
// ... 1426 lines not shown
```

Baseline: 222.0 billion.

## Fuse multiple steps into one 2-byte FSM sweep kernel with multi-step compaction

Extends the 2-byte FSM sweep kernel so one launch can run 2 or 4 simulation steps over a tile kept in registers. Each step writes to its own fired buffer and uses its own timestamp. A multi-step small compaction kernel is added, and the paired-engine loop now groups the other engine's steps too. The aim is to avoid re-reading and re-writing the state words from HBM and to cut per-step launch overhead. In exchange the code gains more template instantiations, higher register pressure, and coherent due loads between fused steps.

```diff
diff --git a/kwok_amd/csrc/engine.hip b/kwok_amd/csrc/engine.hip
--- a/kwok_amd/csrc/engine.hip
+++ b/kwok_amd/csrc/engine.hip
@@ -286,11 +286,23 @@
   return m;
 }
 
-template <bool kProbe = false>
+struct ClockOfArgs {
+  const SweepArgs& a;
+  __device__ __forceinline__ int64_t now() const { return a.now; }
+  __device__ __forceinline__ uint64_t step() const { return a.step; }
+};
+struct ClockAt {
+  int64_t now_ns;
+  uint64_t step_no;
+  __device__ __forceinline__ int64_t now() const { return now_ns; }
+  __device__ __forceinline__ uint64_t step() const { return step_no; }
+};
+
+template <bool kProbe = false, class Clock>
 __device__ __forceinline__ bool match_object(const SweepArgs& a, const kwk_stage_table* __restrict__ T,
                                              uint32_t n_stages, uint64_t i, uint32_t pred, uint32_t& sched,
                                              int64_t& due, uint32_t& bytes, const uint32_t* lut, uint32_t lut_n,
-                                             uint32_t& gen) {
+                                             uint32_t& gen, const Clock& clk) {
   const uint32_t m = match_mask(T, n_stages, pred, lut, lut_n, a.lut_bytes, a.lut_rest);
   sched &= ~(KWK_F_DIRTY | KWK_F_MATCHERR);
   if (m == 0) return false;
@@ -305,7 +317,7 @@
   const int cnt = __popc(m);
   uint64_t u_pick = 0, u_jit = 0;
   if (!kProbe && (cnt > 1 || (m & T->reserved[0]))) {
-    uint32_t c0 = (uint32_t)gslot, c1 = (uint32_t)a.step, c2 = (uint32_t)(a.step >> 32), c3 = kSitePick;
+    uint32_t c0 = (uint32_t)gslot, c1 = (uint32_t)clk.step(), c2 = (uint32_t)(clk.step() >> 32), c3 = kSitePick;
     philox10(c0, c1, c2, c3, (uint32_t)a.key, (uint32_t)(a.key >> 32));
     u_pick = (uint64_t)c0 | ((uint64_t)c1 << 32);
     u_jit = (uint64_t)c2 | ((uint64_t)c3 << 32);
@@ -363,12 +375,12 @@
     }
     const int64_t dels = need_del ? a.del_s[i] : KWK_DEL_ABSENT;
     if (need_del) bytes += 8;
-    const Getter d = eval_getter(S.delay_slot, S.delay_default, true, sched, rec, dels, a.now, true);
+    const Getter d = eval_getter(S.delay_slot, S.delay_default, true, sched, rec, dels, clk.now(), true);
     if (d.ok) {
       delay = d.v;
       if (S.has_jitter) {
         const Getter j = eval_getter(S.jitter_slot, S.jitter_default, S.jitter_default_ok != 0, sched, rec, dels,
-                                     a.now, true);
+                                     clk.now(), true);
         if (j.ok) {
           if (j.v < delay) {
             delay = j.v;
@@ -385,7 +397,7 @@
     }
   }
   sched = (sched & ~0xFFu) | (uint32_t)pick;
-  due = sat_add(a.now, delay);
+  due = sat_add(clk.now(), delay);
   return true;
 }
 
@@ -427,12 +439,12 @@
   sched |= KWK_STAGE_NONE;
 }
 
-template <bool kHarness, uint32_t kWordBytes, bool kProbe = false, bool kDueOut = false>
+template <bool kHarness, uint32_t kWordBytes, bool kProbe = false, bool kDueOut = false, class Clock>
 __device__ __forceinline__ uint2 process_object(const SweepArgs& a, const kwk_stage_table* __restrict__ T,
                                                const kwk_delta* __restrict__ deltas, uint32_t n_stages,
                                                uint32_t fin_group, uint64_t i, uint32_t pred, uint32_t sched,
                                                int64_t due, Fire& f, uint32_t& n_matched, const uint32_t* lut,
-                                               uint32_t lut_n, uint32_t& gen, int64_t& due_w) {
+                                               uint32_t lut_n, uint32_t& gen, int64_t& due_w, const Clock& clk) {
   if (kHarness) {
     if (!(sched & KWK_F_ALIVE)) {
       pred &= a.harness.keep_mask;
@@ -444,8 +456,8 @@
       }
     } else if ((pred & a.harness.terminal_mask) && !(pred & a.harness.deletion_bit)) {
       pred |= a.harness.deletion_bit;
-      int64_t sec = a.now / 1000000000;
-      if (a.now % 1000000000 < 0) sec -= 1;
+      int64_t sec = clk.now() / 1000000000;
+      if (clk.now() % 1000000000 < 0) sec -= 1;
       if (a.harness.track_deletion) {
         if constexpr (kProbe) gen = 1;
         else a.del_s[i] = sec;
@@ -460,12 +472,12 @@
       if (pred & T->disregard_mask) {
         sched &= ~KWK_F_DIRTY;
       } else {
-        scheduled = match_object<kProbe>(a, T, n_stages, i, pred, sched, due, f.bytes, lut, lut_n, gen);
+        scheduled = match_object<kProbe>(a, T, n_stages, i, pred, sched, due, f.bytes, lut, lut_n, gen, clk);
         n_matched += scheduled ? 1 : 0;
       }
     }
     const uint32_t st = sched & 0xFFu;
-    if (a.fire && st < n_stages && due <= a.now) fire_object(a, T, deltas, n_stages, fin_group, sched >> KWK_CLASS_SHIFT, st,
+    if (a.fire && st < n_stages && due <= clk.now()) fire_object(a, T, deltas, n_stages, fin_group, sched >> KWK_CLASS_SHIFT, st,
                                                    pred, sched, f);
   }
   if (scheduled && (sched & 0xFFu) < n_stages) {
@@ -481,6 +493,15 @@
   }
   f.bytes += kWordBytes;
   return make_uint2(pred, sched);
+}
+template <bool kHarness, uint32_t kWordBytes, bool kProbe = false, bool kDueOut = false>
+__device__ __forceinline__ uint2 process_object(const SweepArgs& a, const kwk_stage_table* __restrict__ T,
+                                               const kwk_delta* __restrict__ deltas, uint32_t n_stages,
+                                               uint32_t fin_group, uint64_t i, uint32_t pred, uint32_t sched,
+                                               int64_t due, Fire& f, uint32_t& n_matched, const uint32_t* lut,
+                                               uint32_t lut_n, uint32_t& gen, int64_t& due_w) {
+  return process_object<kHarness, kWordBytes, kProbe, kDueOut>(a, T, deltas, n_stages, fin_group, i, pred, sched, due, f,
+                                                               n_matched, lut, lut_n, gen, due_w, ClockOfArgs{a});
 }
 
 template <bool kPacked = false>
@@ -518,6 +539,10 @@
 }
 __device__ __forceinline__ int64_t buf_load_i64(__amdgpu_buffer_rsrc_t r, uint32_t off) {
   const auto t = __builtin_amdgcn_raw_buffer_load_b64(r, off, 0, 0);
+  return (int64_t)(((uint64_t)t[1] << 32) | t[0]);
+}
+__device__ __forceinline__ int64_t buf_load_i64_sc1(__amdgpu_buffer_rsrc_t r, uint32_t off) {
+  const auto t = __builtin_amdgcn_raw_buffer_load_b64(r, off, 0, 16);
   return (int64_t)(((uint64_t)t[1] << 32) | t[0]);
 }
 
@@ -792,8 +817,8 @@
   }
 }
 
-template <bool kHarness>
-__device__ __forceinline__ uint2 general16(uint32_t i, uint32_t raw) {
+template <bool kHarness, bool kAt = false>
+__device__ __forceinline__ uint2 general16(uint32_t i, uint32_t raw, int64_t now = 0, uint64_t step = 0) {
   uint64_t ka = (uint64_t)__builtin_amdgcn_kernarg_segment_ptr();
   asm volatile("" : "+v"(ka));
   const SweepArgs& a = *reinterpret_cast<const SweepArgs*>(ka);
@@ -801,12 +826,20 @@
   asm volatile("" : "+v"(tp));
   const kwk_stage_table* __restrict__ T = reinterpret_cast<const kwk_stage_table*>(tp);
   const uint2 s = fmt_unpack(raw, a.fmt);
-  const int64_t due = ((s.y & 0xFFu) != KWK_STAGE_NONE) ? a.due[i] : 0;
   Fire f{false, 0, 0, 0};
   uint32_t nm = 0, gen_unused = 0;
   int64_t due_unused = 0;
-  const uint2 nv = process_object<kHarness, 2>(a, T, a.deltas, T->n_stages, T->fin_group_mask, i, s.x, s.y, due, f, nm,
-                                               a.lut, a.lut_n, gen_unused, due_unused);
+  uint2 nv;
+  if constexpr (kAt) {
+    const int64_t due = ((s.y & 0xFFu) != KWK_STAGE_NONE)
+                            ? __hip_atomic_load(&a.due[i], __ATOMIC_RELAXED, __HIP_MEMORY_SCOPE_AGENT) : 0;
+    nv = process_object<kHarness, 2>(a, T, a.deltas, T->n_stages, T->fin_group_mask, i, s.x, s.y, due, f, nm, a.lut,
+                                     a.lut_n, gen_unused, due_unused, ClockAt{now, step});
+  } else {
+    const int64_t due = ((s.y & 0xFFu) != KWK_STAGE_NONE) ? a.due[i] : 0;
+    nv = process_object<kHarness, 2>(a, T, a.deltas, T->n_stages, T->fin_group_mask, i, s.x, s.y, due, f, nm, a.lut,
+                                     a.lut_n, gen_unused, due_unused);
+  }
   uint32_t e = fmt_pack(nv.x, nv.y, a.fmt) & 0xFFFFu;
   e |= (f.stage & 31u) << 16 | (f.fire ? 1u : 0u) << 21 | (f.flags & 7u) << 22 | (nm & 1u) << 25;
   return make_uint2(e, f.bytes);
@@ -879,13 +912,15 @@
 
 constexpr int kFsmBatch = 4;
 constexpr uint32_t kFsmKernelDefault = 2;
-template <bool kHarness, int Q, bool kPersist, int kDepth>
+template <bool kHarness, int Q, bool kPersist, int kDepth, int kSteps = 1>
 __global__ __launch_bounds__(kBlock) __attribute__((amdgpu_waves_per_eu(Q >= 4 ? 4 : 5))) void sweep16_fsm_kernel(SweepArgs a) {
   constexpr int K = 8 * Q;
   constexpr uint32_t kWave = 64u * K;
   constexpr uint32_t kTile = kBlock * K;
   constexpr int B = kFsmBatch;
   static_assert(kDepth >= 1 && kDepth <= 2 && (kPersist || kDepth == 1), "prefetch depth");
+  static_assert(kSteps >= 1 && kSteps <= (int)kMaxFuseSteps && (kSteps == 1 || !kPersist), "fused steps: one tile per block");
+  constexpr bool kFused = kSteps > 1;
   __shared__ unsigned int s_stat[kStatWords];
   __shared__ uint16_t s_work[kWavesPerBlock][kWave];
   __shared__ uint4 s_tile[kWavesPerBlock][64 * Q];
@@ -939,189 +974,232 @@
     uint32_t seg_n = 0;
     const uint64_t seg_id = (uint64_t)tile * kWavesPerBlock + wave;
     uint32_t* __restrict__ seg32 = reinterpret_cast<uint32_t*>(a.fired) + seg_id * kSeg16;
-    const __amdgpu_buffer_rsrc_t seg_rs = make_rsrc(seg32, kSeg16 * 4u);
+    __amdgpu_buffer_rsrc_t seg_rs = make_rsrc(seg32, kSeg16 * 4u);
     uint4 cur_copy[Q];
     if (kDepth == 1) {
 #pragma unroll
       for (int q = 0; q < Q; ++q) cur_copy[q] = v[q];
     }
     uint4 (&cur)[Q] = kDepth == 1 ? cur_copy : v;
-    constexpr uint32_t kHalfMask = (1u << (4 * Q)) - 1u;
-    uint32_t in_range = kHalfMask | kHalfMask << 16;
-    if (!full) {
-      in_range = 0;
+    uint4 mid[kFused ? Q : 1];
+    bool in_lds = false;
+    if constexpr (kFused) {
+#pragma unroll
+      for (int q = 0; q < Q; ++q) mid[q] = cur[q];
+    }
+    auto step_body = [&](uint4 (&ws)[Q], const uint32_t s) __attribute__((always_inline)) {
+      const int64_t now_s = kFused && s ? a.nowx[s - 1] : 0;
+      auto now = [&]() __attribute__((always_inline)) { return kFused && s ? now_s : a.now; };
+      if (kFused && s) {
+        seg_n = 0;
+        seg32 = reinterpret_cast<uint32_t*>(a.firedx[s - 1]) + seg_id * kSeg16;
+        seg_rs = make_rsrc(seg32, kSeg16 * 4u);
+      }
+      constexpr uint32_t kHalfMask = (1u << (4 * Q)) - 1u;
+      uint32_t in_range = kHalfMask | kHalfMask << 16;
+      if (!full) {
+        in_range = 0;
+#pragma unroll
+        for (int q = 0; q < Q; ++q) {
+          const int64_t left = (int64_t)a.n - (int64_t)(wbase + (uint32_t)q * 512u + lane * 8u);
+          const uint32_t c = left <= 0 ? 0u : left >= 8 ? 8u : (uint32_t)left;
+          in_range |= (((1u << ((c + 1u) >> 1)) - 1u) << (4 * q)) | (((1u << (c >> 1)) - 1u) << (16 + 4 * q));
+        }
+      }
+      uint32_t pend = 0, need = 0, ready = 0;
 #pragma unroll
       for (int q = 0; q < Q; ++q) {
-        const int64_t left = (int64_t)a.n - (int64_t)(wbase + (uint32_t)q * 512u + lane * 8u);
-        const uint32_t c = left <= 0 ? 0u : left >= 8 ? 8u : (uint32_t)left;
-        in_range |= (((1u << ((c + 1u) >> 1)) - 1u) << (4 * q)) | (((1u << (c >> 1)) - 1u) << (16 + 4 * q));
-      }
-    }
-    uint32_t pend = 0, need = 0, ready = 0;
-#pragma unroll
-    for (int q = 0; q < Q; ++q) {
-      const uint32_t dw[4] = {cur[q].x, cur[q].y, cur[q].z, cur[q].w};
-#pragma unroll
-      for (int j = 0; j < 4; ++j) {
-        const uint32_t d = dw[j];
-        const uint32_t mg = (d & X.m2) << X.sm;
-        const uint32_t pe = (((d & X.s2) ^ X.n2) + 0x7FFF7FFFu) & 0x80008000u;
-        uint32_t nb = (d & X.d2) << X.sd;
-        if (kHarness) {
-          nb |= (~d & X.a2) << X.sa;
-          nb |= (((d & X.t2) + 0x7FFF7FFFu) & 0x80008000u) & ~((d & X.l2) << X.sl);
+        const uint32_t dw[4] = {ws[q].x, ws[q].y, ws[q].z, ws[q].w};
+#pragma unroll
+        for (int j = 0; j < 4; ++j) {
+          const uint32_t d = dw[j];
+          const uint32_t mg = (d & X.m2) << X.sm;
+          const uint32_t pe = (((d & X.s2) ^ X.n2) + 0x7FFF7FFFu) & 0x80008000u;
+          uint32_t nb = (d & X.d2) << X.sd;
+          if (kHarness) {
+            nb |= (~d & X.a2) << X.sa;
+            nb |= (((d & X.t2) + 0x7FFF7FFFu) & 0x80008000u) & ~((d & X.l2) << X.sl);
+          }
+          const uint32_t n2 = mg & nb, p2 = mg & pe;
+          const int jj = q * 4 + j;
+          need |= n2 >> (15 - jj);
+          pend |= p2 >> (15 - jj);
         }
-        const uint32_t n2 = mg & nb, p2 = mg & pe;
-        const int jj = q * 4 + j;
-        need |= n2 >> (15 - jj);
-        pend |= p2 >> (15 - jj);
-      }
-    }
-    pend &= in_range;
-    need &= in_range;
-    if (__ballot(pend != 0)) {
+      }
+      pend &= in_range;
+      need &= in_range;
+      if (__ballot(pend != 0)) {
 #pragma unroll 8
-      for (int t = 0; t < K; ++t) {
-        const int k = t < 4 * Q ? t : 16 + t - 4 * Q;
-        const uint32_t p = (pend >> k) & 1u;
-        const int64_t d = buf_load_i64(due_rs, p ? (wbase + bit_word((uint32_t)k) + lane * 8u) * 8u : kOOB);
-        ready |= (p & (uint32_t)(d <= a.now)) << k;
-      }
-      need |= ready;
-    }
-    n_bytes += 2u * (uint32_t)__popc(in_range) + 8u * (uint32_t)__popc(pend);
-    uint32_t n_work = 0, pos = 0;
-    {
-      const uint32_t cnt = (uint32_t)__popc(need);
-      const unsigned long long lt = (1ull << lane) - 1ull;
-#pragma unroll
-      for (int b = 0; b < 6; ++b) {
-        const unsigned long long bal = __ballot((cnt >> b) & 1u);
-        pos += (uint32_t)__popcll(bal & lt) << b;
-        n_work += (uint32_t)__popcll(bal) << b;
-      }
-      for (uint32_t m = need; m; m &= m - 1u) {
-        const uint32_t k = (uint32_t)__ffs(m) - 1u;
-        wl[pos++] = (uint16_t)(bit_word(k) + lane * 8u + (((ready >> k) & 1u) << 15));
-      }
-    }
-    uint32_t we[B], raw[B], ent[B];
-    auto fetch = [&](const uint32_t c0) __attribute__((always_inline)) {
-#pragma unroll
-      for (int b = 0; b < B; ++b) {
-        const uint32_t c = c0 + 64u * b + lane;
-        const bool in = c < n_work;
-        const uint32_t x0 = (uint32_t)wl[c & (kWave - 1u)];
-        const uint32_t x = in ? x0 : 0u;
-        we[b] = in ? x : 0xFFFFFFFFu;
-        raw[b] = (uint32_t)tw[x & 0x7FFFu];
-        ent[b] = __builtin_amdgcn_raw_buffer_load_b32(fsm_rs, in ? ((((x >> 15) << fbits) | raw[b]) * 4u) : kOOB, 0, 0);
-      }
-    };
-    auto emit = [&](const bool fire, const uint32_t w, const uint32_t e) __attribute__((always_inline)) {
-      const unsigned long long bal = __ballot(fire);
-      if (bal) {
-        const uint32_t pos = seg_n + __builtin_amdgcn_mbcnt_hi((uint32_t)(bal >> 32), __builtin_amdgcn_mbcnt_lo((uint32_t)bal, 0u));
-        const uint32_t rec = w | ((e >> 16) & 31u) << 13 | ((e >> 22) & 7u) << 18;
-        __builtin_amdgcn_raw_buffer_store_b32(rec, seg_rs, fire ? (1u + pos) * 4u : kOOB, 0, 0);
-        const uint32_t nf = (uint32_t)__popcll(bal);
-        seg_n += nf;
-        w_bytes += 4u * nf;
-        const uint32_t code = fire ? ((e >> 16) & 31u) : 31u;
-        if (n_stages <= 4) {
-          const uint32_t inc = 1u << (16u * (code & 1u));
-          stc01 += code < 2u ? inc : 0u;
-          stc23 += (code - 2u) < 2u ? inc : 0u;
-        } else {
-          for (uint32_t st = 0; st < n_stages; ++st) {
-            const unsigned long long same = __ballot(code == st);
-            if (same && lane == 0) atomicAdd(&s_stat[3 + st], (unsigned)__popcll(same));
+        for (int t = 0; t < K; ++t) {
+          const int k = t < 4 * Q ? t : 16 + t - 4 * Q;
+          const uint32_t p = (pend >> k) & 1u;
+          const int64_t d = kFused ? buf_load_i64_sc1(due_rs, p ? (wbase + bit_word((uint32_t)k) + lane * 8u) * 8u : kOOB)
+                                   : buf_load_i64(due_rs, p ? (wbase + bit_word((uint32_t)k) + lane * 8u) * 8u : kOOB);
+          ready |= (p & (uint32_t)(d <= now())) << k;
+        }
+        need |= ready;
+      }
+      n_bytes += 2u * (uint32_t)__popc(in_range) + 8u * (uint32_t)__popc(pend);
+      uint32_t n_work = 0, pos = 0;
+      {
+        const uint32_t cnt = (uint32_t)__popc(need);
+        const unsigned long long lt = (1ull << lane) - 1ull;
+#pragma unroll
+        for (int b = 0; b < 6; ++b) {
+          const unsigned long long bal = __ballot((cnt >> b) & 1u);
+          pos += (uint32_t)__popcll(bal & lt) << b;
+          n_work += (uint32_t)__popcll(bal) << b;
+        }
+        for (uint32_t m = need; m; m &= m - 1u) {
+          const uint32_t k = (uint32_t)__ffs(m) - 1u;
+          wl[pos++] = (uint16_t)(bit_word(k) + lane * 8u + (((ready >> k) & 1u) << 15));
+        }
+      }
+      uint32_t we[B], raw[B], ent[B];
+      auto fetch = [&](const uint32_t c0) __attribute__((always_inline)) {
+#pragma unroll
+        for (int b = 0; b < B; ++b) {
+          const uint32_t c = c0 + 64u * b + lane;
+          const bool in = c < n_work;
+          const uint32_t x0 = (uint32_t)wl[c & (kWave - 1u)];
+          const uint32_t x = in ? x0 : 0u;
+          we[b] = in ? x : 0xFFFFFFFFu;
+          raw[b] = (uint32_t)tw[x & 0x7FFFu];
+          ent[b] = __builtin_amdgcn_raw_buffer_load_b32(fsm_rs, in ? ((((x >> 15) << fbits) | raw[b]) * 4u) : kOOB, 0, 0);
+        }
+      };
+      auto emit = [&](const bool fire, const uint32_t w, const uint32_t e) __attribute__((always_inline)) {
+        const unsigned long long bal = __ballot(fire);
+        if (bal) {
+          const uint32_t pos = seg_n + __builtin_amdgcn_mbcnt_hi((uint32_t)(bal >> 32), __builtin_amdgcn_mbcnt_lo((uint32_t)bal, 0u));
+          const uint32_t rec = w | ((e >> 16) & 31u) << 13 | ((e >> 22) & 7u) << 18;
+          __builtin_amdgcn_raw_buffer_store_b32(rec, seg_rs, fire ? (1u + pos) * 4u : kOOB, 0, 0);
+          const uint32_t nf = (uint32_t)__popcll(bal);
+          seg_n += nf;
+          w_bytes += 4u * nf;
+          const uint32_t code = fire ? ((e >> 16) & 31u) : 31u;
+          if (n_stages <= 4) {
+            const uint32_t inc = 1u << (16u * (code & 1u));
+            stc01 += code < 2u ? inc : 0u;
+            stc23 += (code - 2u) < 2u ? inc : 0u;
+          } else {
+            for (uint32_t st = 0; st < n_stages; ++st) {
+              const unsigned long long same = __ballot(code == st);
+              if (same && lane == 0) atomicAdd(&s_stat[3 + st], (unsigned)__popcll(same));
+            }
           }
         }
-      }
-    };
-    uint32_t n_gen = 0;
-    auto pass = [&](const int b) __attribute__((always_inline)) {
-      const uint32_t cwe = we[b], e = ent[b];
-      const bool act = cwe != 0xFFFFFFFFu;
-      const uint32_t w = cwe & 0x7FFFu;
-      const bool gen = act && (e & kFsmGeneral);
-      const unsigned long long gb = __ballot(gen);
-      if (gb) {
-        if (gen) wl[n_gen + __builtin_amdgcn_mbcnt_hi((uint32_t)(gb >> 32), __builtin_amdgcn_mbcnt_lo((uint32_t)gb, 0u))] = (uint16_t)w;
-        n_gen += (uint32_t)__popcll(gb);
-      }
-      const bool tab = act && !gen;
-      if (tab) {
-        tw[w] = (uint16_t)e;
-        n_matched += (e >> 25) & 1u;
-        n_bytes += ((e >> 26) & 15u) * 2u;
-      }
-      const bool dw = tab && (e & kFsmDue);
-      if (__ballot(dw)) {
-        const int64_t dd = buf_load_i64(fdue_rs, dw ? ((((cwe >> 15) << fbits) | raw[b]) * 8u) : kOOB);
-        const int64_t v = sat_add(a.now, dd);
-        const uint32_t off = dw ? (wbase + w) * 8u : kOOB;
-        __builtin_amdgcn_raw_buffer_store_b32((uint32_t)v, due_rs, off, 0, 0);
-        __builtin_amdgcn_raw_buffer_store_b32((uint32_t)((uint64_t)v >> 32), due_rs, off + 4u, 0, 0);
-      }
-      emit(tab && ((e >> 21) & 1u), w, e);
-    };
-    if (n_work) {
-#pragma unroll
-      for (int q = 0; q < Q; ++q) tq[q * 64 + lane] = cur[q];
-      __builtin_amdgcn_fence(__ATOMIC_SEQ_CST, "wavefront");
-      fetch(0);
-    }
-    if (kPersist && kDepth == 1) issue_tile(v, tile + gridDim.x);
-    if (n_work) {
-#pragma unroll
-      for (int b = 0; b < B; ++b)
-        if (64u * b < n_work) pass(b);
-      for (uint32_t c0 = 64u * B; c0 < n_work; c0 += 64u * B) {
-        fetch(c0);
-#pragma unroll
-        for (int b = 0; b < B; ++b)
-          if (c0 + 64u * b < n_work) pass(b);
-      }
-      for (uint32_t j = 0; j < n_gen; j += 64u) {
-        const bool in = j + lane < n_gen;
-        const uint32_t w = in ? (uint32_t)wl[j + lane] : 0u;
-        uint32_t e = 0;
-        if (in) {
-          const uint2 r = general16<kHarness>(wbase + w, (uint32_t)tw[w]);
-          e = r.x;
+      };
+      uint32_t n_gen = 0;
+      auto pass = [&](const int b) __attribute__((always_inline)) {
+        const uint32_t cwe = we[b], e = ent[b];
+        const bool act = cwe != 0xFFFFFFFFu;
+        const uint32_t w = cwe & 0x7FFFu;
+        const bool gen = act && (e & kFsmGeneral);
+        const unsigned long long gb = __ballot(gen);
+        if (gb) {
+          if (gen) wl[n_gen + __builtin_amdgcn_mbcnt_hi((uint32_t)(gb >> 32), __builtin_amdgcn_mbcnt_lo((uint32_t)gb, 0u))] = (uint16_t)w;
+          n_gen += (uint32_t)__popcll(gb);
+        }
+        const bool tab = act && !gen;
+        if (tab) {
           tw[w] = (uint16_t)e;
           n_matched += (e >> 25) & 1u;
-          n_bytes += r.y;
+          n_bytes += ((e >> 26) & 15u) * 2u;
         }
-        emit(in && ((e >> 21) & 1u), w, e);
-      }
-      w_line -= 2u * n_work;
-      __builtin_amdgcn_fence(__ATOMIC_SEQ_CST, "wavefront");
-#pragma unroll
-      for (int q = 0; q < Q; ++q) {
-        const uint4 nv = tq[q * 64 + lane];
-        const bool ch = (nv.x ^ cur[q].x) | (nv.y ^ cur[q].y) | (nv.z ^ cur[q].z) | (nv.w ^ cur[q].w);
-        const unsigned long long bal = __ballot(ch);
-        if ((bal >> (lane & ~(kStoreLanes - 1u))) & ((1ull << kStoreLanes) - 1ull)) {
-          store_chunk_nt(&gq[(wbase + (uint32_t)q * 512u + lane * 8u) / 8u], nv);
-          n_lline += 16u;
+        const bool dw = tab && (e & kFsmDue);
+        if (__ballot(dw)) {
+          const int64_t dd = buf_load_i64(fdue_rs, dw ? ((((cwe >> 15) << fbits) | raw[b]) * 8u) : kOOB);
+          const int64_t v = sat_add(now(), dd);
+          const uint32_t off = dw ? (wbase + w) * 8u : kOOB;
+          __builtin_amdgcn_raw_buffer_store_b32((uint32_t)v, due_rs, off, 0, 0);
+          __builtin_amdgcn_raw_buffer_store_b32((uint32_t)((uint64_t)v >> 32), due_rs, off + 4u, 0, 0);
         }
-      }
-      __builtin_amdgcn_fence(__ATOMIC_SEQ_CST, "wavefront");
-    }
-    {
-      const uint32_t used = 1u + seg_n, end = (used + 31u) & ~31u;
-      for (uint32_t x = used + lane; x < end; x += 64) seg32[x] = 0u;
-      if (lane == 0) {
-        seg32[0] = seg_n;
-        a.wave_counts[seg_id] = seg_n;
-      }
-      w_line += 4u * (end - used);
-    }
-    wave_fired += seg_n;
-    w_bytes += 4u;
+        emit(tab && ((e >> 21) & 1u), w, e);
+      };
+      if (n_work) {
+        if (!kFused || !in_lds) {
+#pragma unroll
+          for (int q = 0; q < Q; ++q) tq[q * 64 + lane] = ws[q];
+        }
+        __builtin_amdgcn_fence(__ATOMIC_SEQ_CST, "wavefront");
+        fetch(0);
+      }
+      if (kPersist && kDepth == 1) issue_tile(v, tile + gridDim.x);
+      if (n_work) {
+#pragma unroll
+        for (int b = 0; b < B; ++b)
+          if (64u * b < n_work) pass(b);
+        for (uint32_t c0 = 64u * B; c0 < n_work; c0 += 64u * B) {
+          fetch(c0);
+#pragma unroll
+          for (int b = 0; b < B; ++b)
+            if (c0 + 64u * b < n_work) pass(b);
+        }
+        for (uint32_t j = 0; j < n_gen; j += 64u) {
+          const bool in = j + lane < n_gen;
+          const uint32_t w = in ? (uint32_t)wl[j + lane] : 0u;
+          uint32_t e = 0;
+          if (in) {
+            uint2 r;
+            if constexpr (kFused) r = general16<kHarness, true>(wbase + w, (uint32_t)tw[w], now(), a.step + s);
+            else r = general16<kHarness>(wbase + w, (uint32_t)tw[w]);
+            e = r.x;
+            tw[w] = (uint16_t)e;
+            n_matched += (e >> 25) & 1u;
+            n_bytes += r.y;
+          }
+          emit(in && ((e >> 21) & 1u), w, e);
+        }
+        w_line -= 2u * n_work;
+        __builtin_amdgcn_fence(__ATOMIC_SEQ_CST, "wavefront");
+#pragma unroll
+        for (int q = 0; q < Q; ++q) {
+          const uint4 nv = tq[q * 64 + lane];
+          const bool ch = (nv.x ^ ws[q].x) | (nv.y ^ ws[q].y) | (nv.z ^ ws[q].z) | (nv.w ^ ws[q].w);
+          const unsigned long long bal = __ballot(ch);
+          if ((bal >> (lane & ~(kStoreLanes - 1u))) & ((1ull << kStoreLanes) - 1ull)) {
+            if constexpr (!kFused) store_chunk_nt(&gq[(wbase + (uint32_t)q * 512u + lane * 8u) / 8u], nv);
+            n_lline += 16u;
+          }
+          if constexpr (kFused) ws[q] = nv;
+        }
+        __builtin_amdgcn_fence(__ATOMIC_SEQ_CST, "wavefront");
+        if constexpr (kFused) in_lds = true;
+      }
+      {
+        const uint32_t used = 1u + seg_n, end = (used + 31u) & ~31u;
+        for (uint32_t x = used + lane; x < end; x += 64) seg32[x] = 0u;
+        if (lane == 0) {
+          seg32[0] = seg_n;
+          (kFused && s ? a.countsx[s - 1] : a.wave_counts)[seg_id] = seg_n;
+        }
+        w_line += 4u * (end - used);
+      }
+      wave_fired += seg_n;
+      w_bytes += 4u;
+    };
+    if constexpr (!kFused) {
+      step_body(cur, 0u);
+    } else {
+#pragma nounroll
+      for (uint32_t s = 0; s < (uint32_t)kSteps; ++s) {
+        step_body(mid, s);
+        if (s + 1u < (uint32_t)kSteps) {
+          __builtin_amdgcn_fence(__ATOMIC_RELEASE, "workgroup");
+          asm volatile("s_waitcnt vmcnt(0)" ::: "memory");
+        }
+      }
+      if (in_lds) {
+#pragma unroll
+        for (int q = 0; q < Q; ++q) {
+          const bool ch = (mid[q].x ^ cur[q].x) | (mid[q].y ^ cur[q].y) | (mid[q].z ^ cur[q].z) | (mid[q].w ^ cur[q].w);
+          const unsigned long long bal = __ballot(ch);
+          if ((bal >> (lane & ~(kStoreLanes - 1u))) & ((1ull << kStoreLanes) - 1ull))
+            store_chunk_nt(&gq[(wbase + (uint32_t)q * 512u + lane * 8u) / 8u], mid[q]);
+        }
+      }
+    }
     if (kPersist && kDepth == 2) issue_tile(v, tile + 2u * gridDim.x);
   };
   if constexpr (!kPersist) {
@@ -1159,7 +1237,7 @@
     const unsigned int val = s_stat[threadIdx.x];
     if (val) atomicAdd(&a.cum[(uint64_t)blockIdx.x * kStatWords + threadIdx.x], (unsigned long long)val);
   }
-  if constexpr (!kPersist) {
+  if constexpr (!kPersist && !kFused) {
     if (a.tail.out) tail_handback<kWave, kSeg16>(a, tile < n_tiles ? wave_fired : 0u, lane, wave);
   }
 }
@@ -2403,12 +2481,12 @@
   }
 }
 
-template <int kRec, bool kPacked = false>
-__global__ __launch_bounds__(kBlock) void compact_small_kernel(CompactArgs a) {
+template <int kRec, bool kPacked>
+__device__ __forceinline__ void compact_small_block(const CompactArgs& a, const uint32_t block) {
   __shared__ uint32_t s_part[kWavesPerBlock];
   __shared__ uint32_t s_seg[kWavesPerBlock];
   const uint32_t lane = threadIdx.x & 63, wave = threadIdx.x >> 6;
-  const uint32_t first = blockIdx.x * kSegsPerBlock;
+  const uint32_t first = block * kSegsPerBlock;
   static_assert(kSegsPerBlock % 4 == 0, "prefix loads assume whole uint4s before the block");
   const uint4* __restrict__ c4 = reinterpret_cast<const uint4*>(a.counts);
   const uint32_t nq = first / 4u;
@@ -2437,6 +2515,14 @@
     const uint2 x = rec_at<kRec>(sp, j);
     store_out<kPacked>(a, off + j, base + x.x, x.y);
   }
+}
+template <int kRec, bool kPacked = false>
+__global__ __launch_bounds__(kBlock) void compact_small_kernel(CompactArgs a) {
+  compact_small_block<kRec, kPacked>(a, blockIdx.x);
+}
+template <int kRec, bool kPacked = false>
+__global__ __launch_bounds__(kBlock) void compact_small_multi_kernel(CompactArgs4 m) {
+  compact_small_block<kRec, kPacked>(m.a[blockIdx.y], blockIdx.x);
 }
 
 __global__ void reduce_stats_kernel(const unsigned long long* __restrict__ cum, uint32_t n_blocks,
@@ -5229,6 +5315,17 @@
   return (const void*)k[q == 4 ? 0 : q == 1 ? 1 : 2][harness ? 0 : 1][v];
 }
 
+static const void* sweep16_fused_pick(bool harness, uint32_t q, uint32_t steps) {
+  static const SweepKernel k[3][2][2] = {
+      {{sweep16_fsm_kernel<true, 4, false, 1, 4>, sweep16_fsm_kernel<true, 4, false, 1, 2>},
+       {sweep16_fsm_kernel<false, 4, false, 1, 4>, sweep16_fsm_kernel<false, 4, false, 1, 2>}},
+      {{sweep16_fsm_kernel<true, 1, false, 1, 4>, sweep16_fsm_kernel<true, 1, false, 1, 2>},
+       {sweep16_fsm_kernel<false, 1, false, 1, 4>, sweep16_fsm_kernel<false, 1, false, 1, 2>}},
+      {{sweep16_fsm_kernel<true, 2, false, 1, 4>, sweep16_fsm_kernel<true, 2, false, 1, 2>},
+       {sweep16_fsm_kernel<false, 2, false, 1, 4>, sweep16_fsm_kernel<false, 2, false, 1, 2>}}};
+  return (const void*)k[q == 4 ? 0 : q == 1 ? 1 : 2][harness ? 0 : 1][steps == 4 ? 0 : 1];
+}
+
 static const void* sweepw_pick(bool harness, bool dw, bool narrow) {
   static const SweepKernel k[3][2] = {{sweepw_kernel<true, 8, true>, sweepw_kernel<false, 8, true>},
                                       {sweepw_kernel<true, 4>, sweepw_kernel<false, 4>},
@@ -5280,6 +5377,15 @@
     if (q16 > 1 && (e->n_active + kBlock * 8 * q16 - 1) / (kBlock * 8 * q16) < 4u * (uint32_t)e->n_cus) q16 = 1;
     K = 8 * q16;
     lean = a.fsm && e->fsm_kernel;
+    if (fuse) {
+      if (!lean || (steps != 2 && steps != 4)) return fail(KWK_ESTATE, "fused steps: 2 or 4, table-only 2-byte sweep");
+      for (uint32_t i = 0; i + 1 < steps; ++i) {
+        if (!e->d_firedx[i]) return fail(KWK_ESTATE, "fused steps: buffers not allocated");
+        a.firedx[i] = e->d_firedx[i];
+        a.countsx[i] = e->d_countsx[i];
+        a.nowx[i] = now_ns + (int64_t)(i + 1) * dt_ns;
+      }
+    }
   } else {
     K = dw ? (uint32_t)kQWD * 2u : (uint32_t)kQW * (nar ? 4u : 2u);
     region_shift = 2;
@@ -5296,7 +5402,10 @@
     const uint32_t pg = e->persist16 ? persist_grid(e, pk, tiles) : tiles;
     const uint32_t kind = e->fmt.byte ? KWK_SWEEP_8 : lean ? KWK_SWEEP_16_FSM : KWK_SWEEP_16;
     e->last_sweep = kwk_sweep_info{kind, e->fmt.byte ? (uint32_t)kQ8 : q16, 0, 1, tiles, tiles, h ? 1u : 0u, 0};
-    if (2 * pg <= tiles) {
+    if (fuse && !e->fmt.byte) {
+      if (2 * pg <= tiles) return fail(KWK_ESTATE, "fused steps: the 2-byte sweep's grid is persistent");
+      kern = sweep16_fused_pick(h, q16, steps);
+    } else if (2 * pg <= tiles) {
       blocks = pg;
       e->last_sweep.persistent = 1;
       e->last_sweep.grid = pg;
@@ -5311,7 +5420,7 @@
       }
       kern = sweep16_pick(h, q16, lean, false, 1);
     }
-    if (e->fmt.byte) e->last_sweep.steps = steps;
+    if (e->fmt.byte || fuse) e->last_sweep.steps = steps;
   } else {
     const uint32_t tpb = e->word_tpb ? e->word_tpb : dw ? 8u : 4u;
     blocks = e->word_tpb ? (tiles + tpb - 1) / tpb
@@ -5575,9 +5684,20 @@
   return sweep_compact(e, now, seed, step, compact != 0, hb_fmt_of_compact(compact), ev_a);
 }
 
-static uint32_t fuse_group(const kwk_engine* e, uint32_t left, uint32_t ev_every) {
-  if (e->fuse_steps < 2 || !e->fmt.byte || e->n_stages > 4 || e->fsm8_due_any || !e->loaded_table || ev_every == 1)
-    return 1;
+static bool fuse16_ok(kwk_engine* e) {
+  if (!e->fmt.half || e->fmt.byte || !e->fsm_kernel || e->n_active == 0) return false;
+  const bool h = e->harness.enable != 0;
+  if (e->fsm_harness != (h ? 1 : 0)) return false;
+  uint32_t q = e->q16;
+  if (q > 1 && (e->n_active + kBlock * 8 * q - 1) / (kBlock * 8 * q) < 4u * (uint32_t)e->n_cus) q = 1;
+  const uint32_t tiles = (e->n_active + kBlock * 8 * q - 1) / (kBlock * 8 * q);
+  const uint32_t pg = e->persist16 ? persist_grid(e, sweep16_pick(h, q, true, true, e->fsm_kernel), tiles) : tiles;
+  return 2 * pg > tiles;
+}
+
+static uint32_t fuse_group(kwk_engine* e, uint32_t left, uint32_t ev_every) {
+  if (e->fuse_steps < 2 || !e->loaded_table || ev_every == 1 || left < 2) return 1;
+  if (e->fmt.byte ? e->n_stages > 4 || e->fsm8_due_any : !fuse16_ok(e)) return 1;
   uint32_t m = e->fuse_steps;
   while (ev_every && m > 2 && m > ev_every) m >>= 1;
   while (m > left) m >>= 1;
@@ -5598,17 +5718,29 @@
   if (ev_a >= 0)
     if (kwk_status st = kwk_event_record(e, (uint32_t)ev_a + 1u)) return st;
   const uint32_t n_waves = e->last_blocks * kWavesPerBlock;
-  if (compact == KWK_COMPACT_PACKED16 && e->last_rec == kRecId8Half && n_waves) {
+  const bool multi16 = compact == KWK_COMPACT_PACKED16 && e->last_rec == kRecId8Half;
+  const bool multi_small = compact && e->fmt.half && !e->fmt.byte && n_waves <= e->compact_small;
+  if ((multi16 || multi_small) && n_waves) {
+    const HbFmt mode = multi16 ? HbFmt::Packed16 : hb_fmt_of_compact(compact) == HbFmt::Rec ? HbFmt::Rec : HbFmt::Packed;
     CompactArgs4 c4;
     for (uint32_t i = 0; i < m; ++i)
-      if (kwk_status st = hb_prepare(e, hb_next(e, i + 1), HbFmt::Packed16, e->stream)) return st;
+      if (kwk_status st = hb_prepare(e, hb_next(e, i + 1), mode, e->stream)) return st;
     for (uint32_t i = 0; i < m; ++i) {
       CompactArgs& a = c4.a[i];
       a.fired32 = reinterpret_cast<const uint32_t*>((i ? e->d_firedx[i - 1] : e->d_fired).get());
       a.counts = i ? e->d_countsx[i - 1] : e->d_wave_counts;
-      hb_args(e, hb_next(e, i + 1), HbFmt::Packed16, a);
-    }
-    if (kwk_status st = launch_compact16(e, e->stream, n_waves, c4, m)) return st;
+      hb_args(e, hb_next(e, i + 1), mode, a);
+    }
+    if (multi16) {
+      if (kwk_status st = launch_compact16(e, e->stream, n_waves, c4, m)) return st;
+    } else {
+      const dim3 grid((n_waves + kSegsPerBlock - 1) / kSegsPerBlock, m);
+      if (mode == HbFmt::Packed)
+        hipLaunchKernelGGL((compact_small_multi_kernel<kRecSlot, true>), grid, dim3(kBlock), 0, e->stream, c4);
+      else
+        hipLaunchKernelGGL((compact_small_multi_kernel<kRecSlot>), grid, dim3(kBlock), 0, e->stream, c4);
+      HIP_TRY(hipGetLastError());
+    }
     for (uint32_t i = 1; i < m; ++i) {
       std::swap(e->d_fired, e->d_firedx[i - 1]);
       std::swap(e->d_wave_counts, e->d_countsx[i - 1]);
@@ -5616,8 +5748,7 @@
     const uint32_t last = hb_next(e, m);
     for (uint32_t i = 0; i < m; ++i) {
       const uint32_t slot = hb_next(e, 1);
-      if (kwk_status st = hb_commit(e, slot, step + i, HbFmt::Packed16, n_waves, (int)last, e->stream, i + 1 == m))
-        return st;
+      if (kwk_status st = hb_commit(e, slot, step + i, mode, n_waves, (int)last, e->stream, i + 1 == m)) return st;
     }
     return KWK_OK;
   }
@@ -5689,8 +5820,16 @@
     } else if (kwk_status st = step_one(e, now, seed, step0 + k, compact, ev_of(ev_every, j))) {
       return st;
     }
-    for (uint32_t i = 0; i < m; ++i)
-      if (kwk_status st = step_one(other, now + (int64_t)i * dt_ns, seed, step0 + k + i, compact, -1)) return st;
+    for (uint32_t i = 0; i < m;) {
+      const uint32_t mo = fuse_group(other, m - i, 0);
+      const int64_t now_i = now + (int64_t)i * dt_ns;
+      if (mo > 1) {
+        if (kwk_status st = step_group(other, mo, now_i, dt_ns, seed, step0 + k + i, compact, -1)) return st;
+      } else if (kwk_status st = step_one(other, now_i, seed, step0 + k + i, compact, -1)) {
+        return st;
+      }
+      i += mo;
+    }
     k += m;
   }
   return KWK_OK;
```

Result: faster. 229.9 billion (median of 6 runs) (+3.6%).
